# pangenome/seqrush

Measured on AMD Instinct MI355X. Metric: aligned pairs/sec all-vs-all 64x5kb, higher is better.
Workload: dtype i16; 1 GPU; C2: 64 x 5 kb synthetic (5% SNP, seed 2001), all-vs-all incl. self = 4096 ordered pairs, -k 0 -S 0,5,8,2,24,1 --orientation-scores 0,1,1,1, biWFA (Ultralow); pairs_total=4096, pairs_per_gpu=4096, parallelism=pair-shard x1

## Files before the change

### include/seqrush_amd.h

```cpp
#ifndef SEQRUSH_AMD_H
#define SEQRUSH_AMD_H
#include <stddef.h>
#include <stdint.h>

#ifdef __cplusplus
extern "C" {
#endif

#define SR_ABI_VERSION 2

typedef enum {
    SR_OK = 0,
    SR_ERR_INVALID = -1,
    SR_ERR_NO_DEVICE = -2,
    SR_ERR_HIP = -3,
    SR_ERR_ALPHABET = -4,
    SR_ERR_EMPTY_SEQ = -5,
    SR_ERR_UNSUPPORTED = -6,
    SR_ERR_DEVICE_FAULT = -7,
    SR_ERR_IO = -8,
    SR_ERR_NOMEM = -9
} sr_status;

typedef struct {
    uint32_t n;
    const uint8_t *bases;
    const uint64_t *offsets;
    const char *const *names;
} sr_seqset;

#define SR_MEM_HIGH 0
#define SR_MEM_ULTRALOW 3

#define SR_SPARSE_NONE 0
#define SR_SPARSE_AUTO 1
#define SR_SPARSE_RANDOM 2
#define SR_SPARSE_CONNECTIVITY 3
#define SR_SPARSE_TREE 4

typedef struct {
    int32_t match_score;
    int32_t mismatch_penalty;
    int32_t gap_open1, gap_ext1;
    int32_t gap_open2, gap_ext2;
    int32_t ori_match, ori_mismatch, ori_gap_open, ori_gap_ext;
    uint64_t min_match_len;
    double max_divergence;
    int32_t exclude_self;
    int32_t memory_mode;
    int32_t sparsify_kind;
    double sparsify_factor;
    uint64_t sparsify_seed;
    int32_t canonical_labels;
    int32_t device;
    uint32_t shard_rank, shard_count;
    uint32_t tree_k_nearest, tree_k_farthest;
    double tree_rand_frac;
    uint32_t tree_kmer;
} sr_params;

void sr_default_params(sr_params *p);
int sr_parse_scores(const char *s, sr_params *p);
int sr_parse_orientation_scores(const char *s, sr_params *p);
int sr_parse_sparsification(const char *s, sr_params *p);

int sr_pair_list(uint32_t n, const sr_params *p, uint32_t **q_out, uint32_t **t_out,
                 uint64_t *count);

typedef struct {
    uint64_t n;
    uint32_t *query_idx, *target_idx;
    uint8_t *is_reverse;
    int32_t *score;
    uint64_t *query_start, *query_end, *target_start, *target_end;
    uint64_t *cigar_off;
    uint32_t *cigar_ops;
} sr_alignments;

int sr_align_all(const sr_seqset *seqs, const sr_params *p, sr_alignments **out);
void sr_alignments_free(sr_alignments *a);
size_t sr_alignment_cigar(const sr_alignments *a, uint64_t i, char *buf, size_t cap);

int sr_align_and_unite(const sr_seqset *seqs, const sr_params *p, uint64_t *parent_out);

uint64_t sr_uf_find(const uint64_t *nodes, uint64_t n, uint64_t x);
int sr_uf_same(const uint64_t *nodes, uint64_t n, uint64_t x, uint64_t y);
int sr_uf_init_host(uint64_t *nodes, uint64_t n, uint64_t total_len);
int sr_uf_unite_host(uint64_t *nodes, uint64_t n, uint64_t x, uint64_t y);
int sr_uf_merge_labels_host(uint64_t *nodes, uint64_t n, const uint64_t *labels, uint32_t count);
int sr_uf_canonical_labels_host(const uint64_t *nodes, uint64_t n, uint64_t *labels_out);

int sr_write_paf(const sr_alignments *a, const sr_seqset *seqs, const char *path);

typedef struct sr_ctx sr_ctx;
int sr_ctx_create(int device, sr_ctx **out);
void sr_ctx_destroy(sr_ctx *c);
int sr_ctx_set_stream(sr_ctx *c, void *hip_stream);
int sr_ctx_load(sr_ctx *c, const sr_seqset *seqs, const sr_params *p);
int sr_ctx_load_pairs(sr_ctx *c, const sr_seqset *seqs, const sr_params *p, const uint32_t *query_idx,
                      const uint32_t *target_idx, uint64_t count);
int sr_ctx_pairs(const sr_ctx *c, uint32_t **q_out, uint32_t **t_out, uint64_t *count);
uint32_t sr_ctx_num_batches(const sr_ctx *c);
const char *sr_ctx_workspace_report(const sr_ctx *c);
int sr_ctx_reset_uf(sr_ctx *c);
int sr_ctx_align(sr_ctx *c);
int sr_ctx_unite(sr_ctx *c);
int sr_ctx_run(sr_ctx *c);
int sr_ctx_align_all(sr_ctx *c, int unite, sr_alignments **out);
int sr_ctx_pair_results(sr_ctx *c, int32_t *score, uint8_t *is_reverse, uint32_t *cigar_ops);
int sr_ctx_sync(sr_ctx *c);
int sr_ctx_alignments(sr_ctx *c, sr_alignments **out);
int sr_ctx_download_uf(sr_ctx *c, uint64_t *parent_out);
uint64_t sr_ctx_uf_size(const sr_ctx *c);
uint64_t sr_ctx_num_pairs(const sr_ctx *c);
uint64_t sr_ctx_dp_cells(const sr_ctx *c);
int sr_ctx_labels_device(sr_ctx *c, uint64_t *dev_labels);
int sr_ctx_merge_labels(sr_ctx *c, const uint64_t *dev_labels, uint32_t count);
int sr_ctx_labels_device_u32(sr_ctx *c, uint32_t *dev_labels);
int sr_ctx_merge_labels_u32(sr_ctx *c, const uint32_t *dev_labels, uint32_t count);
int sr_ctx_download_labels(sr_ctx *c, uint64_t *labels_out);
int sr_ctx_merge_labels_host(sr_ctx *c, const uint64_t *labels, uint32_t count);
int sr_ctx_load_paf(sr_ctx *c, const sr_seqset *seqs, const sr_params *p, const char *paf_path);
int sr_unite_paf(const sr_seqset *seqs, const sr_params *p, const char *paf_path, uint64_t *parent_out);
int sr_ctx_build_gfa(sr_ctx *c, const sr_seqset *seqs, char **gfa, uint64_t *n_nodes, uint64_t *n_edges);
int sr_ctx_kernel_ms(sr_ctx *c, int which, float *ms);
const char *sr_ctx_align_kernel(const sr_ctx *c);
int sr_ctx_counters(sr_ctx *c, uint64_t out[16]);
int sr_ctx_counters_ext(sr_ctx *c, uint64_t out[32]);
int sr_ctx_counters_all(sr_ctx *c, uint64_t *out, uint32_t cap);
const char *sr_knobs_doc(void);
int sr_ctx_tail_deferred(sr_ctx *c, uint64_t *out);
int sr_ctx_tail_timeline(sr_ctx *c, uint64_t *out, uint32_t cap_wg);
int sr_tail_shape(int impl, int block_levels, int wave_build, int off16, int ring_u16, int symbol_bits, int two_piece,
                  int main_threads, uint32_t max_words, int forced);

typedef struct {
    uint64_t tree_entries;
    uint64_t random_entries;
    uint64_t random_processed;
    uint64_t random_aligned;
    uint64_t checks;
    uint64_t windows;
    uint64_t post_tree;
    uint64_t final_components;
    int32_t stabilized;
    int32_t tree_defaulted;
    uint32_t tree_k_nearest, tree_k_farthest;
    double tree_rand_frac;
    uint32_t tree_kmer;
    uint32_t reserved;
} sr_iter_stats;
int sr_ctx_load_iterative(sr_ctx *c, const sr_seqset *seqs, const sr_params *p, int keep_alignments);
int sr_ctx_run_iterative(sr_ctx *c);
int sr_ctx_iterative_stats(sr_ctx *c, sr_iter_stats *out, uint64_t *check_counts, uint64_t cap);
int sr_ctx_iterative_alignments(sr_ctx *c, sr_alignments **out);
int sr_uf_count_components_host(const uint64_t *nodes, uint64_t n, uint64_t total_len, uint64_t *count);
int sr_iterative_stop_host(const uint64_t *counts, uint64_t nchecks, uint64_t post_tree, uint64_t *stop_check);
int sr_iterative_pair_lists(uint32_t n, const uint8_t *sel, const sr_params *p, uint32_t **tree_i, uint32_t **tree_j,
                            uint64_t *tree_count, uint32_t **rand_i, uint32_t **rand_j, uint64_t *rand_count);
int sr_base_cone_reach(int e1, int e2, int two, int levels_left);
int sr_mirror_map(const uint32_t *query_idx, const uint32_t *target_idx, uint64_t count, const uint32_t *batch_first,
                  uint32_t nbatch, uint32_t workgroups, uint32_t *mirror_out, uint64_t *partners_out);
int sr_ctx_orientation_scores(sr_ctx *c, int32_t *fwd, int32_t *rev);
int sr_mirror_bt_pick(const int *off, int transposed);
int sr_mirror_bt_rank_transposed(int tag);
int sr_mirror_bt_tie_host(const int *off);
int sr_mirror_bp_pick_host(const int *val, const int *dist, const int *comp, const int *diag, int n, int value_bias,
                           int *pick_out, int *pick_t_out);
int sr_replay_record_ints(void);
void sr_replay_transpose_host(const int *rec, int *out);
int sr_replay_match_host(const int *recs, int nrec, const int *segs, int nseg, int level, int *match_out);

typedef struct {
    uint64_t min_size;
    int32_t keep_alignments;
    uint32_t join_below;
} sr_inv_params;
typedef struct {
    uint64_t scanned;
    uint64_t sites;
    uint64_t candidates;
    uint64_t accepted;
    uint64_t rejected_score;
    uint64_t rejected_divergence;
    uint64_t united_bases;
    uint64_t patch_batches;
    double scan_ms, patch_align_ms;
} sr_inv_stats;
typedef struct {
    uint64_t pair;
    uint32_t query_idx, target_idx;
    uint64_t query_start, query_end;
    uint64_t target_start, target_end;
    int32_t main_score, patch_score;
    uint8_t is_reverse;
    uint8_t accepted;
    uint8_t reserved[2];
    int32_t site_cost;
} sr_inv_job;
int sr_ctx_enable_inversions(sr_ctx *c, const sr_inv_params *p);
int sr_ctx_inversion_stats(sr_ctx *c, sr_inv_stats *out);
int sr_ctx_inversion_join_stats(sr_ctx *c, uint64_t out[4]);
int sr_ctx_inversion_jobs(sr_ctx *c, sr_inv_job **jobs, uint64_t *count);
int sr_ctx_inversion_alignments(sr_ctx *c, sr_alignments **out);
int sr_append_paf_tagged(const sr_alignments *a, const sr_seqset *seqs, const char *path, const char *tag);
#define SR_INV_SITE_DIVERGENT 1
#define SR_INV_SITE_QUERY_ONLY 2
#define SR_INV_SITE_TARGET_ONLY 3
typedef struct {
    uint64_t query_start, query_end, target_start, target_end;
    int32_t kind;
    int32_t candidate;
} sr_inv_site;
int sr_inversion_sites_host(const uint32_t *ops, uint64_t n_ops, uint64_t min_size, sr_inv_site **sites, uint64_t *count);
int sr_inversion_candidate(uint64_t qgap, uint64_t tgap, uint64_t min_size);
int sr_inversion_accept(int32_t patch_score, int32_t main_score);
int sr_inversion_sites_host_join(const uint32_t *ops, uint64_t n_ops, uint64_t min_size, uint32_t join_below, const sr_params *pen,
                                 sr_inv_site **sites, int32_t **cost, uint64_t *count);
int sr_inversion_accept_site(int32_t patch_score, int32_t site_cost);
int sr_inversion_scan_device(int device, const uint32_t *ops, const uint64_t *cigar_off, uint64_t n, uint64_t min_size,
                             sr_inv_site **sites, uint64_t **owner, uint64_t *count);
int sr_inversion_scan_device_join(int device, const uint32_t *ops, const uint64_t *cigar_off, uint64_t n, uint64_t min_size,
                                  uint32_t join_below, const sr_params *pen, const int32_t *score, const int32_t *max_score,
                                  sr_inv_site **sites, uint64_t **owner, int32_t **cost, uint64_t *count, uint64_t stats[4]);
int sr_sketch_device(int device, const sr_seqset *seqs, uint32_t kmer, uint64_t **sketch, uint32_t **sketch_n,
                     uint32_t **shared, uint32_t **denom);
int sr_knn_select_device(int device, const uint32_t *shared, const uint32_t *denom, uint32_t n, uint32_t k_nearest,
                         uint32_t k_farthest, uint8_t **sel);

int sr_build_gfa(const sr_seqset *seqs, const uint64_t *labels, char **gfa,
                 uint64_t *n_nodes, uint64_t *n_edges);
int sr_build_gfa_opts(const sr_seqset *seqs, const uint64_t *labels, int compact, char **gfa,
                      uint64_t *n_nodes, uint64_t *n_edges);
int sr_build_gfa_from_nodes(const sr_seqset *seqs, const uint64_t *nodes, int compact, char **gfa,
                            uint64_t *n_nodes, uint64_t *n_edges);
int sr_ctx_build_gfa_opts(sr_ctx *c, const sr_seqset *seqs, int compact, char **gfa, uint64_t *n_nodes, uint64_t *n_edges);

#define SR_SORT_DEVICE_HOST_TWIN (-1)
#define SR_SORT_DEVICE_SEQUENTIAL (-2)
typedef struct {
    uint64_t seed;
    uint64_t iter_max;
    double theta;
    double eps;
    double eta_max;
    double cooling_start;
    uint64_t space;
    uint64_t space_max;
    uint64_t space_quant;
    uint64_t min_term_updates;
    uint64_t terms_per_round;
    int32_t skip_sgd, skip_groom, skip_topo;
    int32_t device;
} sr_sort_params;
void sr_sort_params_default(sr_sort_params *p);
int sr_ctx_build_gfa_sorted(sr_ctx *c, const sr_seqset *seqs, int compact, const sr_sort_params *p, char **gfa,
                            uint64_t *n_nodes, uint64_t *n_edges);
int sr_sort_gfa(const char *gfa_in, const sr_sort_params *p, char **gfa_out, uint64_t *n_nodes, uint64_t *n_edges);
int sr_sgd_layout(const char *gfa_in, const sr_sort_params *p, double *pos_out, uint64_t n);
int sr_sgd_tables(const char *gfa_in, const sr_sort_params *p, sr_sort_params *resolved, uint64_t sizes[4], double *etas,
                  double *zetas, double *prefix_theta, double *prefix_cool);
int sr_sort_stats(double *out, uint32_t cap);

#define SR_COMPACT_DEVICE_HOST (-1)
#define SR_COMPACT_DEVICE_TABLES_HOST (-2)
int sr_compact_gfa(const char *gfa_in, int device, char **gfa_out, uint64_t *n_nodes, uint64_t *n_edges, uint64_t stats[8]);
int sr_compact_stats(uint64_t stats[8]);

#define SR_STATS_DEVICE_HOST (-1)
typedef struct {
    uint64_t length, nodes, edges, paths, steps;
    uint64_t rev_steps, depth_bp;
    uint64_t self_loops, tips, components;
    uint32_t *depth, *paths_on;
    uint64_t *bp_by_paths, *nodes_by_paths;
    uint64_t *shared;
    uint64_t *path_pairs, *path_abs, *path_len;
    uint64_t *path_sq;
    uint64_t total_pairs, total_abs, total_len, total_sq[3];
    uint64_t stats_us;
    uint64_t kernel_us[5];
} sr_graph_stats;
int sr_graph_stats_gfa(const char *gfa_in, int device, sr_graph_stats **out);
void sr_graph_stats_free(sr_graph_stats *s);
int sr_graph_stats_report(const sr_graph_stats *s, const char *const *names, char **text);
// ... 115 lines not shown
```

### seqrush_amd/_lib.py

```python
import ctypes as C
import os

_HERE = os.path.dirname(os.path.abspath(__file__))
LIB_PATH = os.environ.get("SEQRUSH_AMD_LIB") or os.path.join(_HERE, "libseqrush_amd.so")

EXPORTS = [
    "sr_default_params", "sr_parse_scores", "sr_parse_orientation_scores",
    "sr_parse_sparsification", "sr_align_all", "sr_alignments_free", "sr_alignment_cigar",
    "sr_align_and_unite", "sr_uf_find", "sr_uf_same", "sr_write_paf", "sr_ctx_create",
    "sr_ctx_destroy", "sr_ctx_set_stream", "sr_ctx_load", "sr_ctx_reset_uf", "sr_ctx_align",
    "sr_ctx_unite", "sr_ctx_sync", "sr_ctx_alignments", "sr_ctx_download_uf", "sr_ctx_uf_size",
    "sr_ctx_num_pairs", "sr_ctx_dp_cells", "sr_ctx_labels_device", "sr_ctx_merge_labels",
    "sr_ctx_download_labels", "sr_ctx_kernel_ms", "sr_ctx_counters", "sr_build_gfa", "sr_free",
    "sr_last_error", "sr_abi_version", "sr_device_count", "sr_pair_list", "sr_ctx_align_kernel",
    "sr_ctx_load_paf", "sr_unite_paf", "sr_ctx_build_gfa", "sr_ctx_load_pairs", "sr_ctx_pairs",
    "sr_ctx_num_batches", "sr_ctx_workspace_report", "sr_ctx_run", "sr_ctx_align_all", "sr_ctx_pair_results",
    "sr_ctx_labels_device_u32", "sr_ctx_merge_labels_u32", "sr_ctx_counters_ext",
    "sr_build_gfa_opts", "sr_ctx_build_gfa_opts", "sr_ctx_merge_labels_host",
    "sr_uf_init_host", "sr_uf_unite_host", "sr_uf_merge_labels_host", "sr_uf_canonical_labels_host",
    "sr_build_gfa_from_nodes", "sr_ctx_counters_all", "sr_knobs_doc",
    "sr_sort_params_default", "sr_ctx_build_gfa_sorted", "sr_sort_gfa", "sr_sgd_layout", "sr_sgd_tables", "sr_sort_stats",
    "sr_ctx_load_iterative", "sr_ctx_run_iterative", "sr_ctx_iterative_stats", "sr_ctx_iterative_alignments",
    "sr_uf_count_components_host", "sr_iterative_stop_host", "sr_iterative_pair_lists", "sr_base_cone_reach",
    "sr_ctx_enable_inversions", "sr_ctx_inversion_stats", "sr_ctx_inversion_jobs", "sr_ctx_inversion_alignments",
    "sr_append_paf_tagged", "sr_inversion_sites_host", "sr_inversion_candidate", "sr_inversion_accept",
    "sr_inversion_scan_device",
    "sr_ctx_inversion_join_stats", "sr_inversion_sites_host_join", "sr_inversion_accept_site", "sr_inversion_scan_device_join",
    "sr_compact_gfa", "sr_compact_stats",
    "sr_sketch_device", "sr_knn_select_device",
    "sr_graph_stats_gfa", "sr_graph_stats_free", "sr_graph_stats_report", "sr_stats_sq_sums_host",
    "sr_mirror_map", "sr_mirror_bt_pick", "sr_mirror_bt_rank_transposed", "sr_mirror_bt_tie_host", "sr_mirror_bp_pick_host",
    "sr_ctx_orientation_scores",
    "sr_layout_params_default", "sr_layout_gfa", "sr_layout_tsv", "sr_layout_svg", "sr_layout_quality", "sr_layout_stats",
    "sr_layout_resolve", "sr_layout_select_host",
    "sr_path_bins_gfa", "sr_path_bins_free", "sr_path_bins_tsv", "sr_viz_params_default", "sr_path_bins_rgb", "sr_path_bins_png",
    "sr_growth_params_default", "sr_growth_gfa", "sr_growth_free", "sr_growth_groups", "sr_growth_expected", "sr_growth_fit",
    "sr_growth_report",
    "sr_variant_params_default", "sr_variants_gfa", "sr_variants_free", "sr_variants_vcf",
    "sr_ctx_tail_deferred", "sr_ctx_tail_timeline", "sr_tail_shape",
    "sr_replay_record_ints", "sr_replay_transpose_host", "sr_replay_match_host",
]


class SeqSetC(C.Structure):
    _fields_ = [("n", C.c_uint32), ("bases", C.c_char_p), ("offsets", C.POINTER(C.c_uint64)),
                ("names", C.POINTER(C.c_char_p))]


class ParamsC(C.Structure):
    _fields_ = [
        ("match_score", C.c_int32), ("mismatch_penalty", C.c_int32),
        ("gap_open1", C.c_int32), ("gap_ext1", C.c_int32),
        ("gap_open2", C.c_int32), ("gap_ext2", C.c_int32),
        ("ori_match", C.c_int32), ("ori_mismatch", C.c_int32),
        ("ori_gap_open", C.c_int32), ("ori_gap_ext", C.c_int32),
        ("min_match_len", C.c_uint64), ("max_divergence", C.c_double),
        ("exclude_self", C.c_int32), ("memory_mode", C.c_int32),
        ("sparsify_kind", C.c_int32), ("sparsify_factor", C.c_double),
        ("sparsify_seed", C.c_uint64), ("canonical_labels", C.c_int32), ("device", C.c_int32),
        ("shard_rank", C.c_uint32), ("shard_count", C.c_uint32),
        ("tree_k_nearest", C.c_uint32), ("tree_k_farthest", C.c_uint32), ("tree_rand_frac", C.c_double),
        ("tree_kmer", C.c_uint32),
    ]


class SortParamsC(C.Structure):
    _fields_ = [
        ("seed", C.c_uint64), ("iter_max", C.c_uint64), ("theta", C.c_double), ("eps", C.c_double),
        ("eta_max", C.c_double), ("cooling_start", C.c_double), ("space", C.c_uint64), ("space_max", C.c_uint64),
        ("space_quant", C.c_uint64), ("min_term_updates", C.c_uint64), ("terms_per_round", C.c_uint64),
        ("skip_sgd", C.c_int32), ("skip_groom", C.c_int32), ("skip_topo", C.c_int32), ("device", C.c_int32),
    ]


class LayoutParamsC(C.Structure):
    _fields_ = [
        ("seed", C.c_uint64), ("iter_max", C.c_uint64), ("theta", C.c_double), ("eps", C.c_double),
        ("eta_max", C.c_double), ("cooling_start", C.c_double), ("space", C.c_uint64), ("space_max", C.c_uint64),
        ("space_quant", C.c_uint64), ("min_term_updates", C.c_uint64), ("terms_per_round", C.c_uint64),
        ("device", C.c_int32), ("reserved", C.c_int32),
    ]


class IterStatsC(C.Structure):
    _fields_ = [
        ("tree_entries", C.c_uint64), ("random_entries", C.c_uint64), ("random_processed", C.c_uint64),
        ("random_aligned", C.c_uint64), ("checks", C.c_uint64), ("windows", C.c_uint64), ("post_tree", C.c_uint64),
        ("final_components", C.c_uint64), ("stabilized", C.c_int32), ("tree_defaulted", C.c_int32),
        ("tree_k_nearest", C.c_uint32), ("tree_k_farthest", C.c_uint32), ("tree_rand_frac", C.c_double),
        ("tree_kmer", C.c_uint32), ("reserved", C.c_uint32),
    ]


class InvParamsC(C.Structure):
    _fields_ = [("min_size", C.c_uint64), ("keep_alignments", C.c_int32), ("join_below", C.c_uint32)]


class InvStatsC(C.Structure):
    _fields_ = [("scanned", C.c_uint64), ("sites", C.c_uint64), ("candidates", C.c_uint64), ("accepted", C.c_uint64),
                ("rejected_score", C.c_uint64), ("rejected_divergence", C.c_uint64), ("united_bases", C.c_uint64),
                ("patch_batches", C.c_uint64), ("scan_ms", C.c_double), ("patch_align_ms", C.c_double)]


class InvJobC(C.Structure):
    _fields_ = [("pair", C.c_uint64), ("query_idx", C.c_uint32), ("target_idx", C.c_uint32),
                ("query_start", C.c_uint64), ("query_end", C.c_uint64), ("target_start", C.c_uint64),
                ("target_end", C.c_uint64), ("main_score", C.c_int32), ("patch_score", C.c_int32),
                ("is_reverse", C.c_uint8), ("accepted", C.c_uint8), ("reserved", C.c_uint8 * 2), ("site_cost", C.c_int32)]


class InvSiteC(C.Structure):
    _fields_ = [("query_start", C.c_uint64), ("query_end", C.c_uint64), ("target_start", C.c_uint64),
                ("target_end", C.c_uint64), ("kind", C.c_int32), ("candidate", C.c_int32)]


class GraphStatsC(C.Structure):
    _fields_ = [("length", C.c_uint64), ("nodes", C.c_uint64), ("edges", C.c_uint64), ("paths", C.c_uint64), ("steps", C.c_uint64),
                ("rev_steps", C.c_uint64), ("depth_bp", C.c_uint64),
                ("self_loops", C.c_uint64), ("tips", C.c_uint64), ("components", C.c_uint64),
                ("depth", C.POINTER(C.c_uint32)), ("paths_on", C.POINTER(C.c_uint32)),
                ("bp_by_paths", C.POINTER(C.c_uint64)), ("nodes_by_paths", C.POINTER(C.c_uint64)),
                ("shared", C.POINTER(C.c_uint64)),
                ("path_pairs", C.POINTER(C.c_uint64)), ("path_abs", C.POINTER(C.c_uint64)), ("path_len", C.POINTER(C.c_uint64)),
                ("path_sq", C.POINTER(C.c_uint64)),
                ("total_pairs", C.c_uint64), ("total_abs", C.c_uint64), ("total_len", C.c_uint64), ("total_sq", C.c_uint64 * 3),
                ("stats_us", C.c_uint64), ("kernel_us", C.c_uint64 * 5)]


class BinParamsC(C.Structure):
    _fields_ = [("bin_width", C.c_uint64), ("bins", C.c_uint64)]


class PathBinsC(C.Structure):
    _fields_ = [("length", C.c_uint64), ("paths", C.c_uint64), ("bins", C.c_uint64), ("bin_width", C.c_uint64),
                ("cov", C.POINTER(C.c_uint64)), ("inv", C.POINTER(C.c_uint64)),
                ("bin_us", C.c_uint64), ("kernel_us", C.c_uint64 * 3)]


class VizParamsC(C.Structure):
    _fields_ = [("mode", C.c_int), ("path_height", C.c_uint32), ("path_gap", C.c_uint32), ("depth_max", C.c_uint32)]


class GrowthParamsC(C.Structure):
    _fields_ = [("seed", C.c_uint64), ("permutations", C.c_uint64)]


class GrowthC(C.Structure):
    _fields_ = [("length", C.c_uint64), ("paths", C.c_uint64), ("groups", C.c_uint64), ("permutations", C.c_uint64),
                ("exhaustive", C.c_int32), ("variant", C.c_int32),
                ("pan", C.POINTER(C.c_uint64)), ("core", C.POINTER(C.c_uint64)), ("perm", C.POINTER(C.c_uint32)),
                ("bp_by_groups", C.POINTER(C.c_uint64)), ("growth_us", C.c_uint64), ("kernel_us", C.c_uint64 * 4),
                ("seed", C.c_uint64)]


class VariantParamsC(C.Structure):
    _fields_ = [("ref_name", C.c_char_p), ("max_allele_len", C.c_uint64), ("hash_mask", C.c_uint64), ("reserved", C.c_uint64)]


class VariantsC(C.Structure):
    _fields_ = [("ref_path", C.c_uint64), ("ref_len", C.c_uint64), ("paths", C.c_uint64), ("anchors", C.c_uint64),
                ("traversals", C.c_uint64), ("sites", C.c_uint64), ("hash_collision_sites", C.c_uint64),
                ("breaks", C.POINTER(C.c_uint64)), ("skipped", C.POINTER(C.c_uint64)),
                ("site_start", C.POINTER(C.c_uint64)), ("site_end", C.POINTER(C.c_uint64)), ("site_alleles", C.POINTER(C.c_uint32)),
                ("allele_off", C.POINTER(C.c_uint64)), ("alleles", C.POINTER(C.c_char)), ("gt", C.POINTER(C.c_int32)),
                ("ref_seq", C.POINTER(C.c_char)), ("variant", C.c_int32), ("reserved", C.c_int32),
                ("variants_us", C.c_uint64), ("kernel_us", C.c_uint64 * 6)]


class AlignmentsC(C.Structure):
    _fields_ = [
        ("n", C.c_uint64), ("query_idx", C.POINTER(C.c_uint32)), ("target_idx", C.POINTER(C.c_uint32)),
        ("is_reverse", C.POINTER(C.c_uint8)), ("score", C.POINTER(C.c_int32)),
        ("query_start", C.POINTER(C.c_uint64)), ("query_end", C.POINTER(C.c_uint64)),
        ("target_start", C.POINTER(C.c_uint64)), ("target_end", C.POINTER(C.c_uint64)),
        ("cigar_off", C.POINTER(C.c_uint64)), ("cigar_ops", C.POINTER(C.c_uint32)),
    ]


class SeqRushError(RuntimeError):
    def __init__(self, code, msg):
        super().__init__(f"seqrush_amd error {code}: {msg}")
        self.code = code


_lib = None


def load():
    global _lib
    if _lib is not None:
        return _lib
    if not os.path.exists(LIB_PATH):
        raise ImportError(
            f"{LIB_PATH} not found: build it with `python -c 'import __graft_entry__ as g; g.build()'` "
            "(seqrush_amd has no CPU fallback)")
    L = C.CDLL(LIB_PATH)
    vp, u64, i32 = C.c_void_p, C.c_uint64, C.c_int
    PP, PS = C.POINTER(ParamsC), C.POINTER(SeqSetC)
    L.sr_default_params.argtypes = [PP]; L.sr_default_params.restype = None
    L.sr_parse_scores.argtypes = [C.c_char_p, PP]
    L.sr_parse_orientation_scores.argtypes = [C.c_char_p, PP]
    L.sr_parse_sparsification.argtypes = [C.c_char_p, PP]
    L.sr_align_all.argtypes = [PS, PP, C.POINTER(C.POINTER(AlignmentsC))]
    L.sr_alignments_free.argtypes = [C.POINTER(AlignmentsC)]; L.sr_alignments_free.restype = None
    L.sr_alignment_cigar.argtypes = [C.POINTER(AlignmentsC), u64, C.c_char_p, C.c_size_t]
    L.sr_alignment_cigar.restype = C.c_size_t
    L.sr_align_and_unite.argtypes = [PS, PP, C.POINTER(u64)]
    L.sr_uf_find.argtypes = [C.POINTER(u64), u64, u64]; L.sr_uf_find.restype = u64
    L.sr_uf_same.argtypes = [C.POINTER(u64), u64, u64, u64]
    L.sr_write_paf.argtypes = [C.POINTER(AlignmentsC), PS, C.c_char_p]
    L.sr_ctx_create.argtypes = [i32, C.POINTER(vp)]
    L.sr_ctx_destroy.argtypes = [vp]; L.sr_ctx_destroy.restype = None
    L.sr_ctx_set_stream.argtypes = [vp, vp]
    L.sr_ctx_load.argtypes = [vp, PS, PP]
    for f in ("sr_ctx_reset_uf", "sr_ctx_align", "sr_ctx_unite", "sr_ctx_sync"):
        getattr(L, f).argtypes = [vp]
    L.sr_ctx_alignments.argtypes = [vp, C.POINTER(C.POINTER(AlignmentsC))]
    L.sr_ctx_download_uf.argtypes = [vp, C.POINTER(u64)]
    for f in ("sr_ctx_uf_size", "sr_ctx_num_pairs", "sr_ctx_dp_cells"):
        getattr(L, f).argtypes = [vp]; getattr(L, f).restype = u64
    L.sr_ctx_labels_device.argtypes = [vp, vp]
    L.sr_ctx_merge_labels.argtypes = [vp, vp, C.c_uint32]
    L.sr_ctx_download_labels.argtypes = [vp, C.POINTER(u64)]
    L.sr_ctx_merge_labels_host.argtypes = [vp, C.POINTER(u64), C.c_uint32]
    L.sr_ctx_kernel_ms.argtypes = [vp, i32, C.POINTER(C.c_float)]
    L.sr_ctx_align_kernel.argtypes = [vp]; L.sr_ctx_align_kernel.restype = C.c_char_p
    L.sr_ctx_load_paf.argtypes = [vp, PS, PP, C.c_char_p]
    L.sr_unite_paf.argtypes = [PS, PP, C.c_char_p, C.POINTER(u64)]
    L.sr_ctx_build_gfa.argtypes = [vp, PS, C.POINTER(vp), C.POINTER(u64), C.POINTER(u64)]
    L.sr_ctx_counters.argtypes = [vp, C.POINTER(u64)]
    L.sr_ctx_counters_ext.argtypes = [vp, C.POINTER(u64)]
    L.sr_ctx_counters_all.argtypes = [vp, C.POINTER(u64), C.c_uint32]
    L.sr_knobs_doc.restype = C.c_char_p
    L.sr_ctx_tail_deferred.argtypes = [vp, C.POINTER(u64)]
    L.sr_ctx_tail_timeline.argtypes = [vp, C.POINTER(u64), C.c_uint32]
    L.sr_tail_shape.argtypes = [i32] * 8 + [C.c_uint32, i32]
    L.sr_ctx_load_pairs.argtypes = [vp, PS, PP, C.POINTER(C.c_uint32), C.POINTER(C.c_uint32), u64]
    L.sr_ctx_pairs.argtypes = [vp, C.POINTER(C.POINTER(C.c_uint32)), C.POINTER(C.POINTER(C.c_uint32)), C.POINTER(u64)]
    L.sr_ctx_num_batches.argtypes = [vp]; L.sr_ctx_num_batches.restype = C.c_uint32
    L.sr_ctx_workspace_report.argtypes = [vp]; L.sr_ctx_workspace_report.restype = C.c_char_p
    L.sr_ctx_run.argtypes = [vp]
    L.sr_ctx_align_all.argtypes = [vp, i32, C.POINTER(C.POINTER(AlignmentsC))]
    L.sr_ctx_pair_results.argtypes = [vp, C.POINTER(C.c_int32), C.POINTER(C.c_uint8), C.POINTER(C.c_uint32)]
    L.sr_ctx_labels_device_u32.argtypes = [vp, vp]
    L.sr_ctx_merge_labels_u32.argtypes = [vp, vp, C.c_uint32]
    L.sr_build_gfa.argtypes = [PS, C.POINTER(u64), C.POINTER(vp), C.POINTER(u64), C.POINTER(u64)]
    L.sr_build_gfa_opts.argtypes = [PS, C.POINTER(u64), i32, C.POINTER(vp), C.POINTER(u64), C.POINTER(u64)]
    L.sr_ctx_build_gfa_opts.argtypes = [vp, PS, i32, C.POINTER(vp), C.POINTER(u64), C.POINTER(u64)]
    L.sr_uf_init_host.argtypes = [C.POINTER(u64), u64, u64]
    L.sr_uf_unite_host.argtypes = [C.POINTER(u64), u64, u64, u64]
    L.sr_uf_merge_labels_host.argtypes = [C.POINTER(u64), u64, C.POINTER(u64), C.c_uint32]
    L.sr_uf_canonical_labels_host.argtypes = [C.POINTER(u64), u64, C.POINTER(u64)]
    L.sr_build_gfa_from_nodes.argtypes = [PS, C.POINTER(u64), i32, C.POINTER(vp), C.POINTER(u64), C.POINTER(u64)]
    SP, PD = C.POINTER(SortParamsC), C.POINTER(C.c_double)
    L.sr_sort_params_default.argtypes = [SP]; L.sr_sort_params_default.restype = None
    L.sr_ctx_build_gfa_sorted.argtypes = [vp, PS, i32, SP, C.POINTER(vp), C.POINTER(u64), C.POINTER(u64)]
    L.sr_sort_gfa.argtypes = [C.c_char_p, SP, C.POINTER(vp), C.POINTER(u64), C.POINTER(u64)]
    L.sr_sgd_layout.argtypes = [C.c_char_p, SP, PD, u64]
    L.sr_sgd_tables.argtypes = [C.c_char_p, SP, SP, C.POINTER(u64), PD, PD, PD, PD]
    L.sr_sort_stats.argtypes = [PD, C.c_uint32]
    L.sr_pair_list.argtypes = [C.c_uint32, PP, C.POINTER(C.POINTER(C.c_uint32)),
                               C.POINTER(C.POINTER(C.c_uint32)), C.POINTER(u64)]
    L.sr_ctx_load_iterative.argtypes = [vp, PS, PP, i32]
    L.sr_ctx_run_iterative.argtypes = [vp]
    L.sr_ctx_iterative_stats.argtypes = [vp, C.POINTER(IterStatsC), C.POINTER(u64), u64]
    L.sr_ctx_iterative_alignments.argtypes = [vp, C.POINTER(C.POINTER(AlignmentsC))]
    L.sr_uf_count_components_host.argtypes = [C.POINTER(u64), u64, u64, C.POINTER(u64)]
    L.sr_iterative_stop_host.argtypes = [C.POINTER(u64), u64, u64, C.POINTER(u64)]
    L.sr_base_cone_reach.argtypes = [C.c_int, C.c_int, C.c_int, C.c_int]
    PU32 = C.POINTER(C.POINTER(C.c_uint32))
    L.sr_iterative_pair_lists.argtypes = [C.c_uint32, C.POINTER(C.c_uint8), PP, PU32, PU32, C.POINTER(u64), PU32, PU32,
                                          C.POINTER(u64)]
    L.sr_ctx_enable_inversions.argtypes = [vp, C.POINTER(InvParamsC)]
    L.sr_ctx_inversion_stats.argtypes = [vp, C.POINTER(InvStatsC)]
    L.sr_ctx_inversion_jobs.argtypes = [vp, C.POINTER(C.POINTER(InvJobC)), C.POINTER(u64)]
    L.sr_ctx_inversion_alignments.argtypes = [vp, C.POINTER(C.POINTER(AlignmentsC))]
    L.sr_append_paf_tagged.argtypes = [C.POINTER(AlignmentsC), PS, C.c_char_p, C.c_char_p]
    L.sr_inversion_sites_host.argtypes = [C.POINTER(C.c_uint32), u64, u64, C.POINTER(C.POINTER(InvSiteC)), C.POINTER(u64)]
    L.sr_inversion_candidate.argtypes = [u64, u64, u64]
    L.sr_inversion_accept.argtypes = [C.c_int32, C.c_int32]
    L.sr_inversion_scan_device.argtypes = [i32, C.POINTER(C.c_uint32), C.POINTER(u64), u64, u64,
                                           C.POINTER(C.POINTER(InvSiteC)), C.POINTER(C.POINTER(u64)), C.POINTER(u64)]
    PI32 = C.POINTER(C.c_int32)
    L.sr_ctx_inversion_join_stats.argtypes = [vp, C.POINTER(u64)]
    L.sr_inversion_sites_host_join.argtypes = [C.POINTER(C.c_uint32), u64, u64, C.c_uint32, PP, C.POINTER(C.POINTER(InvSiteC)),
                                               C.POINTER(PI32), C.POINTER(u64)]
    L.sr_inversion_accept_site.argtypes = [C.c_int32, C.c_int32]
    L.sr_inversion_scan_device_join.argtypes = [i32, C.POINTER(C.c_uint32), C.POINTER(u64), u64, u64, C.c_uint32, PP, PI32, PI32,
                                                C.POINTER(C.POINTER(InvSiteC)), C.POINTER(C.POINTER(u64)), C.POINTER(PI32),
                                                C.POINTER(u64), C.POINTER(u64)]
    PU32P = C.POINTER(C.POINTER(C.c_uint32))
    L.sr_sketch_device.argtypes = [i32, PS, C.c_uint32, C.POINTER(C.POINTER(u64)), PU32P, PU32P, PU32P]
    L.sr_knn_select_device.argtypes = [i32, C.POINTER(C.c_uint32), C.POINTER(C.c_uint32), C.c_uint32, C.c_uint32, C.c_uint32,
                                       C.POINTER(C.POINTER(C.c_uint8))]
    L.sr_compact_gfa.argtypes = [C.c_char_p, i32, C.POINTER(vp), C.POINTER(u64), C.POINTER(u64), C.POINTER(u64)]
    L.sr_compact_stats.argtypes = [C.POINTER(u64)]
    PGS = C.POINTER(GraphStatsC)
    L.sr_graph_stats_gfa.argtypes = [C.c_char_p, i32, C.POINTER(PGS)]
    L.sr_graph_stats_free.argtypes = [PGS]; L.sr_graph_stats_free.restype = None
    L.sr_graph_stats_report.argtypes = [PGS, C.POINTER(C.c_char_p), C.POINTER(vp)]
    L.sr_stats_sq_sums_host.argtypes = [C.POINTER(u64), u64, C.POINTER(u64)]
    LP = C.POINTER(LayoutParamsC)
    L.sr_layout_params_default.argtypes = [LP]; L.sr_layout_params_default.restype = None
    L.sr_layout_gfa.argtypes = [C.c_char_p, LP, PD, u64]
    L.sr_layout_tsv.argtypes = [PD, u64, C.POINTER(vp)]
    L.sr_layout_svg.argtypes = [C.c_char_p, PD, u64, C.POINTER(vp)]
    L.sr_layout_quality.argtypes = [C.c_char_p, PD, u64, u64, u64, PD]
    L.sr_layout_stats.argtypes = [PD, C.c_uint32]
    L.sr_layout_resolve.argtypes = [C.c_char_p, LP, LP]
    L.sr_layout_select_host.argtypes = [C.c_char_p, LP, u64, u64, u64, i32, C.POINTER(C.c_uint32), C.POINTER(C.c_uint32), PD]
    PPB, PVP = C.POINTER(PathBinsC), C.POINTER(VizParamsC)
    L.sr_path_bins_gfa.argtypes = [C.c_char_p, C.POINTER(BinParamsC), i32, C.POINTER(PPB)]
    L.sr_path_bins_free.argtypes = [PPB]; L.sr_path_bins_free.restype = None
    L.sr_path_bins_tsv.argtypes = [PPB, C.POINTER(C.c_char_p), C.POINTER(vp)]
    L.sr_viz_params_default.argtypes = [PVP]; L.sr_viz_params_default.restype = None
    L.sr_path_bins_rgb.argtypes = [PPB, C.POINTER(C.c_char_p), PVP, C.POINTER(vp), C.POINTER(C.c_uint32), C.POINTER(C.c_uint32)]
    L.sr_path_bins_png.argtypes = [PPB, C.POINTER(C.c_char_p), PVP, C.POINTER(vp), C.POINTER(u64)]
    PG, PU32 = C.POINTER(GrowthC), C.POINTER(C.c_uint32)
    L.sr_growth_params_default.argtypes = [C.POINTER(GrowthParamsC)]; L.sr_growth_params_default.restype = None
    L.sr_growth_gfa.argtypes = [C.c_char_p, PU32, C.c_uint32, C.POINTER(GrowthParamsC), i32, C.POINTER(PG)]
    L.sr_growth_free.argtypes = [PG]; L.sr_growth_free.restype = None
    L.sr_growth_groups.argtypes = [C.POINTER(C.c_char_p), u64, i32, PU32, PU32, C.POINTER(C.POINTER(C.c_char_p))]
    L.sr_growth_expected.argtypes = [C.POINTER(u64), C.c_uint32, PD, PD]
    L.sr_growth_fit.argtypes = [PD, C.c_uint32, PD, PD, PU32]
    L.sr_growth_report.argtypes = [PG, C.POINTER(vp)]
    PV = C.POINTER(VariantsC)
    L.sr_variant_params_default.argtypes = [C.POINTER(VariantParamsC)]; L.sr_variant_params_default.restype = None
    L.sr_variants_gfa.argtypes = [C.c_char_p, C.POINTER(VariantParamsC), i32, C.POINTER(PV)]
    L.sr_variants_free.argtypes = [PV]; L.sr_variants_free.restype = None
    L.sr_variants_vcf.argtypes = [PV, C.POINTER(C.c_char_p), C.POINTER(vp)]
    PI = C.POINTER(C.c_int)
    L.sr_mirror_map.argtypes = [C.POINTER(C.c_uint32), C.POINTER(C.c_uint32), u64, C.POINTER(C.c_uint32), C.c_uint32, C.c_uint32,
                                C.POINTER(C.c_uint32), C.POINTER(u64)]
    L.sr_ctx_orientation_scores.argtypes = [vp, C.POINTER(C.c_int32), C.POINTER(C.c_int32)]
    L.sr_mirror_bt_pick.argtypes = [PI, i32]
    L.sr_mirror_bt_rank_transposed.argtypes = [i32]
    L.sr_mirror_bt_tie_host.argtypes = [PI]
    L.sr_mirror_bp_pick_host.argtypes = [PI, PI, PI, PI, i32, i32, PI, PI]
    L.sr_replay_record_ints.argtypes = []
    L.sr_replay_transpose_host.argtypes = [PI, PI]; L.sr_replay_transpose_host.restype = None
    L.sr_replay_match_host.argtypes = [PI, i32, PI, i32, i32, PI]
    L.sr_free.argtypes = [vp]; L.sr_free.restype = None
    L.sr_last_error.restype = C.c_char_p
    L.sr_abi_version.restype = i32
    L.sr_device_count.restype = i32
    _lib = L
    return L


def check(rc):
    if rc != 0:
        raise SeqRushError(rc, load().sr_last_error().decode(errors="replace"))
```

### seqrush_amd/csrc/sr_align_blk.inc

```
#include "sr_blk_rows.inc"
#include "sr_blk_tile.inc"
#include "sr_blk_pass.inc"
#include "sr_blk_phase2.inc"
#include "sr_blk_orient.inc"

#define K_SHIFT0 29
#define K_WIDTH0 64
struct KSeqs { int poff_f, poff_r, toff_f, toff_r, plen_all, tlen_all; };
__device__ __forceinline__ void kjob_set(int jid, int base, int pb, int pe, int tb, int te, int rev, int begin, int chk,
                                         int seg, const KSeqs &q) {
    bjob_set(jid, base, pb, pe, tb, te, 0, begin, chk, seg, rev ? q.poff_r : q.poff_f);
    BJob &b = b_sh.job[jid];
    b.shift = (pe - pb) + K_SHIFT0;
    b.pad0 = rev ? q.toff_r : q.toff_f;
    b.pad2 = 1;
    if (rev) { b.p0 = q.plen_all - pe; b.t0 = q.tlen_all - te; }
}
__device__ __forceinline__ int kjob_width(int plen, int tlen) { return (plen + tlen + K_WIDTH0) & ~3; }

#define SR_BLK_MIN_WAVES 4
template <typename OT, int NT, bool TWO, int B, int E1, int E2, bool PROF = false, int X = 0, int OE1 = 0, typename RT = OT>
__global__ void __launch_bounds__(NT, SR_BLK_MIN_WAVES) sr_align_blk_kernel(SrAlignArgs a) {
    const int tid = threadIdx.x;
    if (a.tail_mode == SR_TAIL_RUN && *a.tail_count == 0u) return;
    GP<RT> bring = (GP<RT>)(RT *)a.bring + (size_t)blockIdx.x * a.bring_wg_stride;
    GP<OT> bhist = (GP<OT>)(OT *)a.bhist + (size_t)blockIdx.x * a.bhist_wg_stride;
    GP<int> lists = (GP<int>)a.bseg + (size_t)blockIdx.x * 2 * SR_BFS_MAXSEG * SR_BFS_SEGREC;
    GP<uint32_t> btbuf = (GP<uint32_t>)a.bbt + (size_t)blockIdx.x * a.bbase_jobs * SR_BFS_BTCAP;
    GP<uint32_t> clist = (GP<uint32_t>)a.bcl + (size_t)blockIdx.x * a.bcl_wg_stride;
    GP<int> gmak = (GP<int>)a.bmak + (size_t)blockIdx.x * (BJ_MAX * BFS_MAK_SLOTS);
    unsigned long long t_ori = 0, t_bp = 0, t_base = 0, t_all = 0, tb_bt = 0, tb_emit = 0;
    unsigned long long tq_pass = 0, tq_bar = 0, tq_ctl = 0, tq_ph2 = 0, tq_tail = 0, tq_rec = 0;
    unsigned row_ld = 0, row_st = 0;
    unsigned long long tl_first = 0, tl_last = 0, tl_n = 0, tl_mir = 0;
    const int depth = a.kdepth;
    const int depth2 = a.kdepth2;
    const unsigned nrows = (unsigned)depth + 4u * (unsigned)depth2 + (unsigned)SR_NULL_ROWS + 2u;
    KRows<OT, RT> RR;
    KRows<OT, OT> RH;
    RR.base = bring; RR.cM = (unsigned)depth * 256u; RR.cst2 = (unsigned)depth2 * 256u; RR.sstr = 256u; RR.chs = nrows * 256u;
    RR.depth = depth; RR.depth2 = depth2; RR.perjob = false; RR.extent = (unsigned)a.bring_wg_stride;
    RR.nuloff = ((unsigned)depth + 4u * (unsigned)depth2) * 256u; RR.urow = RR.nuloff + (unsigned)SR_NULL_ROWS * 256u; RR.trash = RR.urow + 256u;
    const unsigned urow = RR.urow;
    const unsigned hw = a.hist_nul_w;
    RH.base = bhist; RH.cM = 0; RH.cst2 = 0; RH.sstr = 0; RH.chs = 256u; RH.depth = 0x3fff; RH.depth2 = 0x3fff; RH.urow = 0; RH.perjob = true; RH.extent = (unsigned)a.bhist_wg_stride;
    RH.nuloff = (unsigned)a.hist_cap; RH.trash = RH.nuloff + hw;
    if (tid < 64) k_sh.cells_l[tid] = 0ull;
    if (tid < 64) k_sh.row_w[tid >> 4][tid & 15] = 0ull;
    {
        for (int r = 0; r < SR_NULL_ROWS; r++)
            for (int i = tid; i < a.brow; i += NT) rput(RR, RR.nuloff + (unsigned)r * 256u, (unsigned)i, NULLV);
        for (int i = tid; i < (int)hw; i += NT) RH.base[RH.nuloff + (unsigned)i] = (OT)NULLV;
        if (tid == 0) {
            b_sh.pen[0] = a.pen; b_sh.pen[1] = a.ori; b_sh.cells = 0; k_sh.t_setup = 0; k_sh.t_p2a = k_sh.t_p2f = k_sh.t_p2e = k_sh.t_p2w = 0; k_sh.t_c1 = k_sh.t_c2 = 0;
            k_sh.dg_f = k_sh.dg_c = k_sh.dg_e = k_sh.dg_r = 0; k_sh.dg_redo = 0;
#ifdef SR_BOUNDS
            k_sh.bnd_flag = 0; k_sh.bnd_off = k_sh.bnd_ext = k_sh.bnd_what = 0; k_sh.lds_seq_bytes = 16u * a.max_words + 16u;
#endif
            k_sh.dg_steps = k_sh.dg_nbase = k_sh.dg_nbp = k_sh.dg_npass = 0; k_sh.base_tiles = k_sh.base_cells = 0;
            k_sh.mir_next = -1; k_sh.mir_pairs = k_sh.mir_ties = 0;
            k_sh.rp_record = k_sh.rp_on = k_sh.rp_ready = 0; k_sh.rp_nrec = 0;
            k_sh.rp_replays = k_sh.rp_cached = k_sh.rp_tie_top = k_sh.rp_tie_base = 0;
            b_sh.geom.brow = a.brow; b_sh.geom.ring_scope = a.ring_scope; b_sh.geom.ring_hot = a.ring_hot;
            b_sh.geom.bbase_jobs = a.bbase_jobs; b_sh.geom.hist_w = a.hist_w; b_sh.geom.hist_levels = a.hist_levels;
            b_sh.geom.urow = urow;
        }
        __syncthreads();
    }
    const SrPen pen = a.pen;
    const SrPen ori = a.ori;
    constexpr bool KTIGHT = KTIGHT_OF(OT, RT, B, X);
    const int scope = pen.scope;
    const int gap_opening = TWO ? max(pen.o1, pen.o2) : pen.o1;
    for (;;) {
        if (tid < 64) {
            unsigned long long cl = k_sh.cells_l[tid];
            k_sh.cells_l[tid] = 0ull;
            for (int o = 32; o > 0; o >>= 1) cl += __shfl_xor(cl, o, 64);
            if (tid == 0) b_sh.cells += cl;
        }
        if (tid == 0) {
            int pr = k_sh.mir_next;
            k_sh.mir_next = -1;
            const bool from_mir = pr >= 0;
            if (a.tail_mode == SR_TAIL_RUN) {
                const uint32_t i = atomicAdd(a.tail_head, 1u);
                pr = i < *a.tail_count ? (int)a.tail_list[i] : (int)a.npairs;
            } else while (pr < 0) {
                pr = (int)atomicAdd(a.queue_head, 1u);
                if (pr >= (int)a.npairs) { pr = (int)a.npairs; break; }
                if (a.order) pr = (int)a.order[pr];
                if (a.mirror && a.mirror[pr] != SR_MIRROR_NONE && (a.mirror[pr] & SR_MIRROR_SECONDARY)) pr = -1;
            }
            if (PROF) {
                const unsigned long long now = KTICK();
                if (tl_n == 0) tl_first = now;
                if (pr < (int)a.npairs) { tl_last = now; tl_n++; tl_mir = from_mir ? 1ull : 0ull; }
            }
            k_sh.rp_on = (from_mir && k_sh.rp_ready) ? 1 : 0;
            k_sh.rp_ready = 0; k_sh.rp_record = 0;
            if (a.brec && !from_mir && a.tail_mode != SR_TAIL_RUN && a.mirror && pr < (int)a.npairs) {
                const uint32_t m = a.mirror[pr];
                if (m != SR_MIRROR_NONE && !(m & SR_MIRROR_SECONDARY)) { k_sh.rp_record = 1; k_sh.rp_nrec = 0; }
            }
            k_sh.rp_level = 0; k_sh.rp_rd = 0; k_sh.rp_top_tie = 0; k_sh.rp_seg_tie = 0;
            b_sh.pair = pr;
            b_sh.err = 0; b_sh.cig_cnt = 0; b_sh.score_acc = 0; k_sh.pend_op = -1; k_sh.pend_len = 0;
            k_sh.mir_tie = 0;
            k_sh.mir_snap[0] = b_sh.cells; k_sh.mir_snap[1] = k_sh.dg_steps; k_sh.mir_snap[2] = k_sh.dg_nbase; k_sh.mir_snap[3] = k_sh.dg_nbp;
        }
        __syncthreads();
        const int pair = RFL(b_sh.pair);
        if (pair >= (int)a.npairs) break;
        const uint32_t q = a.pair_q[pair], t = a.pair_t[pair];
        const int plen = (int)a.seqlen[q], tlen = (int)a.seqlen[t];
        const int pw = SR_SEQ_WORDS(plen), tw = SR_SEQ_WORDS(tlen);
        load_seq_lds<NT>(lds_seq, (GP<const uint32_t>)a.seqwords + a.word_off_fwd[q] - 1, pw);
        load_seq_lds<NT>(lds_seq + a.max_words, (GP<const uint32_t>)a.seqwords + a.word_off_rc[q] - 1, pw);
        load_seq_lds<NT>(lds_seq + 2 * (size_t)a.max_words, (GP<const uint32_t>)a.seqwords + a.word_off_fwd[t] - 1, tw);
        load_seq_lds<NT>(lds_seq + 3 * (size_t)a.max_words, (GP<const uint32_t>)a.seqwords + a.word_off_rev[t] - 1, tw);
        const int oPf = 1, oPr = (int)a.max_words + 1, oTf = 2 * (int)a.max_words + 1, oTr = 3 * (int)a.max_words + 1;
        GP<uint32_t> ops = (GP<uint32_t>)a.cigar_ops + a.cigar_base[pair];
        const uint32_t cap = (uint32_t)(a.cigar_base[pair + 1] - a.cigar_base[pair]);
        const unsigned long long tk0 = KTICK();
        int fwd = -1, rev = INT_MAX, is_rev = 0;
        if (a.pre_oriented) {
            is_rev = a.is_reverse[pair] != 0; fwd = a.ori_fwd[pair]; rev = a.ori_rev[pair];
        } else {
        if (tid == 0) {
            const int w = kjob_width(plen, tlen);
            const KSeqs k0 = {oPf, oPr, oTf, oTr, plen, tlen}, k1 = {oPr, oPf, oTf, oTr, plen, tlen};
            kjob_set(0, 0, 0, plen, 0, tlen, 0, SR_C_M, SR_C_M, 0, k0);
            kjob_set(1, w, 0, plen, 0, tlen, 0, SR_C_M, SR_C_M, 0, k1);
            b_sh.njobs = 2;
        }
        __syncthreads();
        const long long smax = (long long)ori.o1 * 2 + (long long)ori.e1 * (plen + tlen) + 64;
        if (!ori.two && ori.x == 1 && ori.o1 == 1 && ori.e1 == 1 && !a.ori_levels) {
            if (tid == 0) {
                b_sh.job[0].shift = plen + 24; b_sh.job[1].shift = plen + 24;
                b_sh.job[1].base = (plen + tlen + 64) & ~3;
            }
            __syncthreads();
            for (int s0 = 0;; s0 += ORI_B) {
                ori_pass8<OT, NT>(RR, s0, ori, row_ld, row_st);
                __syncthreads();
                int hit = -1, who = 0;
#pragma unroll
                for (int j = ORI_B - 1; j >= 0; j--) {
                    const bool rf = RFL(k_sh.jreach[j][0]) != 0, rr = RFL(k_sh.jreach[j][1]) != 0;
                    if (rf || rr) { hit = j; who = rf ? 0 : 1; }
                }
                __syncthreads();
                const int used = hit >= 0 ? hit + 1 : ORI_B;
                if (tid == 0) k_sh.dg_steps += 2ull * (unsigned long long)used;
                if (hit >= 0) {
                    if (tid == 0) {
                        long long sur = 0;
                        for (int l = s0 + hit + 1; l < s0 + ORI_B; l++) {
                            const int Rw = reach(ori, l, SR_C_M);
                            sur += 2LL * (long long)(min(tlen, Rw) - max(-plen, -Rw) + 1);
                        }
                        b_sh.cells -= (unsigned long long)sur;
                    }
                    if (who == 0) fwd = s0 + hit; else { rev = s0 + hit; is_rev = 1; }
                    break;
                }
                if (s0 + ORI_B - 1 > smax) { if (tid == 0) b_sh.err |= SR_DEV_ERR_SCORE_BOUND; break; }
            }
        } else {
            for (int s = 0;; s++) {
                blk_pass<OT, false, NT, 1, 1, 1, PROF>(RR, s, ori, 2, row_ld, row_st);
                __syncthreads();
                if (tid == 0) k_sh.dg_steps += 2ull;
                const bool rf = RFL(k_sh.jreach[0][0]) != 0, rr = RFL(k_sh.jreach[0][1]) != 0;
                __syncthreads();
                if (rf) { fwd = s; break; }
                if (rr) { rev = s; is_rev = 1; break; }
                if (s > smax) { if (tid == 0) b_sh.err |= SR_DEV_ERR_SCORE_BOUND; break; }
            }
        }
        }
        if (a.word_off_rev != a.word_off_rc) {
            __syncthreads();
            load_seq_lds<NT>(lds_seq + (is_rev ? 0 : (size_t)a.max_words),
                             (GP<const uint32_t>)a.seqwords + (is_rev ? a.word_off_cmp[q] : a.word_off_rev[q]) - 1, pw);
            __syncthreads();
        }
        const KSeqs ks = {is_rev ? oPr : oPf, is_rev ? oPf : oPr, oTf, oTr, plen, tlen};
        const unsigned long long tk1 = KTICK();
        t_ori += tk1 - tk0;
        GP<int> cur = lists, nxt = lists + (size_t)SR_BFS_MAXSEG * SR_BFS_SEGREC;
        if (tid == 0) {
            cur[SL_PB] = 0; cur[SL_PE] = plen; cur[SL_TB] = 0; cur[SL_TE] = tlen; cur[SL_CB] = SR_C_M; cur[SL_CE] = SR_C_M;
            const int rem = (a.mem_mode == 3) ? INT_MAX : -1;
            cur[SL_REM] = rem; cur[SL_KIND] = seg_kind(plen, tlen, rem);
            b_sh.list_n = 1;
            if (is_rev) k_sh.rp_on = 0;
            if (k_sh.rp_on) k_sh.rp_replays += 1ull;
        }
        __syncthreads();
        for (;;) {
            const int n_cur = RFL(b_sh.list_n);
            bool any_bp = false;
            int pos = 0;
            if (RFL(k_sh.rp_on) != 0 && tid == 0) {
                GP<int> recs = (GP<int>)a.brec + (size_t)blockIdx.x * (SR_BPREC_MAX * SR_BPREC_INTS);
                const int nrec = min(k_sh.rp_nrec, SR_BPREC_MAX), lvl = k_sh.rp_level;
                int rd = k_sh.rp_rd;
                unsigned long long cells = 0ull, cached = 0ull;
                while (rd < nrec && recs[rd * SR_BPREC_INTS + SR_BR_LEVEL] < lvl) rd++;
                for (int p = 0; p < n_cur; p++) {
                    GP<int> e = cur + (size_t)p * SR_BFS_SEGREC;
                    if (e[SL_KIND] != SK_BP) continue;
                    int solved = 0;
                    while (rd < nrec) {
                        GP<int> r = recs + rd * SR_BPREC_INTS;
                        if (r[SR_BR_LEVEL] != lvl) break;
                        const int c = sr_replay_cmp(r, e);
                        if (c > 0) break;
                        rd++;
                        if (c < 0) continue;
                        if (r[SR_BR_TIE] == 0 && sr_replay_same(r, e)) {
                            e[SL_BV] = sr_bprec_t(r, SR_BR_BV); e[SL_BH] = sr_bprec_t(r, SR_BR_BH); e[SL_BCOMP] = sr_bprec_t(r, SR_BR_BCOMP);
                            e[SL_BSF] = r[SR_BR_BSF]; e[SL_BSR] = r[SR_BR_BSR]; e[SL_PASSES] = r[SR_BR_PASSES];
                            cells += ((unsigned long long)(unsigned)r[SR_BR_CELLS_HI] << 32) | (unsigned long long)(unsigned)r[SR_BR_CELLS_LO];
                            cached += 1ull; solved = 1;
                        }
                        break;
                    }
                    e[SL_SOLVED] = solved;
                }
                k_sh.rp_rd = rd; b_sh.cells += cells; k_sh.rp_cached += cached;
            }
            while (pos < n_cur && RFL(b_sh.err) == 0) {
                __syncthreads();
                if (tid == 0) {
                    int na = 0, p = pos, base = 0, ntot = 0, maxp = 0;
                    const bool rp_on = k_sh.rp_on != 0, rp_rec = k_sh.rp_record != 0;
                    for (; p < n_cur && ntot < SR_BFS_MAXACT; p++) {
                        GP<int> e = cur + (size_t)p * SR_BFS_SEGREC;
                        if (e[SL_KIND] != SK_BP) continue;
                        ntot++;
                        if (rp_on && e[SL_SOLVED] != 0) { maxp = max(maxp, e[SL_PASSES]); continue; }
                        k_sh.sg_tie[na] = 0; k_sh.sg_sur[na] = 0; k_sh.sg_done[na] = 0;
                        if (rp_rec) {
                            b_sh.cells += k_sh.cells_l[2 * na] + k_sh.cells_l[2 * na + 1];
                            k_sh.cells_l[2 * na] = 0ull; k_sh.cells_l[2 * na + 1] = 0ull;
                        }
// ... 296 lines not shown
                            if (st == 0) EMIT(SR_OP_D, sp);
                            else EMIT(SR_OP_I, st);
                        } else if (kind == SK_BASE) {
                            GP<uint32_t> b = btbuf + (size_t)bj * SR_BFS_BTCAP;
                            const int nbt = RFL(b_sh.bt_n[bj]);
                            for (int i = nbt - 1; i >= 0; i -= 64) {
                                const uint32_t v = (i - lane >= 0) ? b[i - lane] : 0u;
                                const int m = min(64, i + 1);
                                for (int u = 0; u < m; u++) {
                                    const uint32_t x = (uint32_t)__builtin_amdgcn_readlane((int)v, u);
                                    EMIT((int)(x & 15u), (int)(x >> 4));
                                }
                            }
                            bj++;
                        } else err |= SR_DEV_ERR_BACKTRACE;
                    }
#undef EMIT
                    if (lane == 0) {
                        b_sh.cig_cnt = cnt; b_sh.emit_pos = pos; k_sh.pend_op = pop; k_sh.pend_len = plen_;
                        if (err) b_sh.err |= err;
                    }
                    KPRIO_LO();
                }
                __syncthreads();
                tb_emit += KTICK() - tem0;
            }
            if (tid == 0 && b_sh.err == 0 && k_sh.pend_op >= 0) {
                uint32_t cnt = b_sh.cig_cnt;
                if (cnt >= cap) b_sh.err |= SR_DEV_ERR_CIGAR_OVERFLOW;
                else { ops[cnt++] = ((uint32_t)k_sh.pend_len << 4) | (uint32_t)k_sh.pend_op; b_sh.cig_cnt = cnt; }
            }
            __syncthreads();
        }
        t_base += KTICK() - tc0;
        __syncthreads();
        const uint32_t cnt = RFL(b_sh.cig_cnt);
        int part = 0;
        for (uint32_t i = tid; i < cnt; i += NT) {
            const uint32_t op = ops[i] & 15u; const int len = (int)(ops[i] >> 4);
            if (op == SR_OP_X) part += len * pen.x;
            else if (op == SR_OP_I || op == SR_OP_D) {
                int g = pen.o1 + pen.e1 * len;
                if (TWO) g = min(g, pen.o2 + pen.e2 * len);
                part += g;
            }
        }
        if (part) atomicAdd(&b_sh.score_acc, part);
        __syncthreads();
        const int p_err = RFL(b_sh.err), p_score = RFL(b_sh.score_acc), p_tie = RFL(k_sh.mir_tie);
        if (tid == 0) {
            a.is_reverse[pair] = is_rev ? 1 : 0;
            a.score[pair] = b_sh.err ? -1 : b_sh.score_acc;
            a.ori_fwd[pair] = fwd; a.ori_rev[pair] = rev;
            a.cigar_cnt[pair] = b_sh.err ? 0u : cnt;
            if (b_sh.err) atomicOr(a.error_flag, b_sh.err);
#ifdef SR_BOUNDS
            if (k_sh.bnd_flag == 1) {
                k_sh.bnd_flag = 2;
                if (atomicCAS(&a.counters[40], 0ull, (unsigned long long)pair + 1ull) == 0ull) {
                    a.counters[41] = k_sh.bnd_what; a.counters[42] = k_sh.bnd_off; a.counters[43] = k_sh.bnd_ext;
                }
            }
#endif
        }
        __syncthreads();
        const uint32_t mir = a.mirror ? a.mirror[pair] : SR_MIRROR_NONE;
        bool mir_emit = false;
        if (mir != SR_MIRROR_NONE && !(mir & SR_MIRROR_SECONDARY)) {
            mir_emit = p_err == 0 && !is_rev && p_tie == 0 && !(a.pre_oriented && a.is_reverse[mir] != 0);
            if (mir_emit) {
                GP<uint32_t> ops2 = (GP<uint32_t>)a.cigar_ops + a.cigar_base[mir];
                for (uint32_t i = tid; i < cnt; i += NT) { const uint32_t v = ops[i]; ops2[i] = v ^ ((v & 2u) >> 1); }
                if (tid < 64) {
                    unsigned long long cl = k_sh.cells_l[tid];
                    k_sh.cells_l[tid] = 0ull;
                    for (int o = 32; o > 0; o >>= 1) cl += __shfl_xor(cl, o, 64);
                    if (tid == 0) {
                        b_sh.cells += cl;
                        b_sh.cells += b_sh.cells - k_sh.mir_snap[0]; k_sh.dg_steps += k_sh.dg_steps - k_sh.mir_snap[1];
                        k_sh.dg_nbase += k_sh.dg_nbase - k_sh.mir_snap[2]; k_sh.dg_nbp += k_sh.dg_nbp - k_sh.mir_snap[3];
                        k_sh.mir_pairs += 1ull;
                        a.score[mir] = p_score; a.cigar_cnt[mir] = cnt;
                        if (!a.pre_oriented) { a.is_reverse[mir] = 0; a.ori_fwd[mir] = fwd; a.ori_rev[mir] = rev; }
                    }
                }
            } else if (tid == 0) {
                k_sh.mir_ties += 1ull;
                if (p_tie != 0) {
                    if (k_sh.rp_top_tie != 0) k_sh.rp_tie_top += 1ull;
                    else if (k_sh.rp_seg_tie == 0) k_sh.rp_tie_base += 1ull;
                }
                const bool replay = k_sh.rp_record != 0 && p_err == 0 && !is_rev && k_sh.rp_top_tie == 0 &&
                                    !(a.pre_oriented && a.is_reverse[mir] != 0) && a.tail_mode != SR_TAIL_DEFER_ALL;
                bool defer = false;
                if (!replay && a.tail_list && a.tail_mode != SR_TAIL_RUN)
                    defer = a.tail_mode == SR_TAIL_DEFER_ALL ||
                            __hip_atomic_load(a.queue_head, __ATOMIC_RELAXED, __HIP_MEMORY_SCOPE_AGENT) >= a.npairs;
                if (defer) { a.tail_list[atomicAdd(a.tail_count, 1u)] = mir; atomicAdd(a.tail_deferred, 1u); }
                else { k_sh.mir_next = (int)mir; k_sh.rp_ready = replay ? 1 : 0; }
            }
        }
        if (a.fuse_unite) {
            const int sc = p_err ? -1 : p_score;
            if (sc >= 0 && sc <= a.max_score[pair]) {
                unsigned long long united = 0, runs = 0;
                int uerr = 0;
                uf_unite_cigar<NT>((const uint32_t *)a.cigar_ops + a.cigar_base[pair], cnt, a.seq_goff[q], a.seq_goff[t],
                                   (unsigned long long)plen, is_rev != 0, 0ull, 0ull, a.min_match_len, a.uf_nodes, united, runs, uerr);
                for (int o = 32; o > 0; o >>= 1) { united += __shfl_xor(united, o, 64); runs += __shfl_xor(runs, o, 64); }
                if ((tid & 63) == 0) {
                    if (united) atomicAdd(&a.counters[4], mir_emit ? 2ull * united : united);
                    if (runs) atomicAdd(&a.counters[5], mir_emit ? 2ull * runs : runs);
                }
                if (uerr) atomicOr(a.error_flag, uerr);
            }
        }
        t_all += KTICK() - tk0;
        if ((tid & 63) == 0) {
            k_sh.row_w[0][(tid >> 6) & 15] += row_ld; k_sh.row_w[1][(tid >> 6) & 15] += row_st;
            k_sh.row_w[2][(tid >> 6) & 15] += row_ld; k_sh.row_w[3][(tid >> 6) & 15] += row_st;
        }
        row_ld = 0; row_st = 0;
    }
    if (tid < 64 && k_sh.cells_l[tid]) atomicAdd(&a.counters[0], k_sh.cells_l[tid]);
    if ((tid & 63) == 0) {
        const unsigned long long lane_bytes = 8ull;
        const unsigned long long row_ld_acc = k_sh.row_w[0][(tid >> 6) & 15], row_st_acc = k_sh.row_w[1][(tid >> 6) & 15];
        if (row_ld_acc) atomicAdd(&a.counters[16], row_ld_acc * lane_bytes);
        if (row_st_acc) atomicAdd(&a.counters[17], row_st_acc * lane_bytes);
        const unsigned long long hist_ld_acc = k_sh.row_w[2][(tid >> 6) & 15], hist_st_acc = k_sh.row_w[3][(tid >> 6) & 15];
        if (hist_ld_acc) atomicAdd(&a.counters[44], hist_ld_acc * lane_bytes);
        if (hist_st_acc) atomicAdd(&a.counters[45], hist_st_acc * lane_bytes);
    }
    if (tid == 0) {
        atomicAdd(&a.counters[0], b_sh.cells);
        atomicAdd(&a.counters[1], k_sh.dg_steps);
        atomicAdd(&a.counters[2], k_sh.dg_nbase);
        atomicAdd(&a.counters[3], k_sh.dg_nbp);
        atomicAdd(&a.counters[9], k_sh.dg_npass);
        atomicAdd(&a.counters[19], k_sh.dg_f); atomicAdd(&a.counters[20], k_sh.dg_c);
        atomicAdd(&a.counters[21], k_sh.dg_e); atomicAdd(&a.counters[22], k_sh.dg_r);
        if (k_sh.dg_redo) atomicAdd(&a.counters[37], k_sh.dg_redo);
        if (k_sh.mir_pairs) atomicAdd(&a.counters[38], k_sh.mir_pairs);
        if (k_sh.mir_ties) atomicAdd(&a.counters[39], k_sh.mir_ties);
        if (k_sh.rp_tie_top) atomicAdd(&a.counters[48], k_sh.rp_tie_top);
        if (k_sh.rp_tie_base) atomicAdd(&a.counters[49], k_sh.rp_tie_base);
        if (k_sh.rp_replays) atomicAdd(&a.counters[50], k_sh.rp_replays);
        if (k_sh.rp_cached) atomicAdd(&a.counters[51], k_sh.rp_cached);
        atomicAdd(&a.counters[46], k_sh.base_tiles); atomicAdd(&a.counters[47], k_sh.base_cells);
        if (PROF && a.timeline) {
            unsigned long long *tl = a.timeline + 4ull * blockIdx.x;
            tl[0] = tl_first; tl[1] = tl_last; tl[2] = KTICK(); tl[3] = tl_n | (tl_mir << 32);
        }
        if (PROF) {
            if (!a.pre_oriented) atomicAdd(&a.counters[6], t_ori);
            atomicAdd(&a.counters[7], t_bp);
            atomicAdd(&a.counters[8], t_base);
            atomicAdd(&a.counters[10], t_all);
            atomicAdd(&a.counters[11], tq_pass);
            atomicAdd(&a.counters[12], tq_bar);
            atomicAdd(&a.counters[13], k_sh.t_setup);
            atomicAdd(&a.counters[25], tq_ctl); atomicAdd(&a.counters[26], k_sh.t_c1); atomicAdd(&a.counters[27], k_sh.t_c2);
            atomicAdd(&a.counters[28], k_sh.t_p2a); atomicAdd(&a.counters[29], k_sh.t_p2f); atomicAdd(&a.counters[30], k_sh.t_p2e); atomicAdd(&a.counters[31], k_sh.t_p2w);
            atomicAdd(&a.counters[14], tq_ph2);
            atomicAdd(&a.counters[18], tq_rec);
            atomicAdd(&a.counters[23], tb_bt); atomicAdd(&a.counters[24], tb_emit);
            atomicAdd(&a.counters[15], tq_tail);
        }
    }
#undef KTICK
}
```

### seqrush_amd/csrc/sr_blk_pass.inc

```
#include "sr_base_cone.h"
template <bool TWO, int E1, int E2>
__device__ __forceinline__ int kreach(const SrPen &p, int s, int begin) {
    int r;
    if (begin == SR_C_M) {
        r = (s >= p.o1 + E1) ? (s - p.o1) / E1 : 0;
        if (TWO && s >= p.o2 + E2) r = max(r, (s - p.o2) / E2);
    } else {
        r = s / E1;
        if (TWO) r = max(r, s / E2);
    }
    return r;
}

template <bool TWO, int B, int E1, int E2, bool TIGHT>
__device__ __forceinline__ void kwindow(const SrPen &pen, const BJob &b, int s0, int &glo, int &ghi) {
    const int Rw = kreach<TWO, E1, E2>(pen, s0 + B - 1, b.begin);
    const int mg = TIGHT ? 1 : pen.scope + 1;
    const int wlo = max(-b.plen - 1, -Rw - mg), whi = min(b.tlen + 1, Rw + mg);
    glo = (wlo + b.shift) >> 2; ghi = (whi + b.shift) >> 2;
}

#define KTICK() (PROF ? __builtin_amdgcn_s_memrealtime() : 0ull)
#define KPRIO_HI() __builtin_amdgcn_s_setprio(3)
#define KPRIO_LO() __builtin_amdgcn_s_setprio(0)
#ifndef SR_BASE_CONE
#define SR_BASE_CONE 1
#endif
template <bool TWO, int NT, int B, int E1, int E2, bool TIGHT = false, bool BASE = false>
__device__ __forceinline__ void blk_setup(int s0, const SrPen &pen, int njobs) {
    const int tid = threadIdx.x;
    constexpr bool CONE = BASE && SR_BASE_CONE;
    int nt = 0, glo = 0, ghi = -1, cells = 0, ccells = 0;
    const bool act = tid < njobs && b_sh.job[tid].active;
    const int pglo = (tid < BJ_MAX) ? k_sh.jglo[tid] : 0, pghi = (tid < BJ_MAX) ? k_sh.jghi[tid] : -1;
    if (act) {
        const BJob &b = b_sh.job[tid];
        int Rw = 0, clo0 = 0, chi0 = 0;
#pragma unroll
        for (int j = 0; j < B; j++) {
            Rw = kreach<TWO, E1, E2>(pen, s0 + j, b.begin);
            int klo = max(-b.plen, -Rw), khi = min(b.tlen, Rw);
            cells += (khi >= klo) ? khi - klo + 1 : 0;
            if (CONE) {
                const int rb = sr_cone_reach(E1, E2, TWO, b.pad1 - 1 - (s0 + j));
                klo = max(klo, b.kend - rb); khi = min(khi, b.kend + rb);
                if (j == 0) { clo0 = b.kend - rb; chi0 = b.kend + rb; }
            }
            k_sh.jklo[j][tid] = klo; k_sh.jkhi[j][tid] = khi;
            ccells += (khi >= klo) ? khi - klo + 1 : 0;
        }
        (void)Rw;
        kwindow<TWO, B, E1, E2, TIGHT>(pen, b, s0, glo, ghi);
        if (CONE) {
            const int mg = TIGHT ? 1 : pen.scope + 1;
            const int wlo = max(max(-b.plen - 1, -Rw - mg), clo0 - 1), whi = min(min(b.tlen + 1, Rw + mg), chi0 + 1);
            glo = (wlo + b.shift) >> 2; ghi = (whi >= wlo) ? (whi + b.shift) >> 2 : glo - 1;
        }
        nt = max(0, (ghi - glo + KGeo<B>::OWN) / KGeo<B>::OWN);
        if (BASE && ccells) atomicAdd(&k_sh.base_cells, (unsigned long long)ccells);
    }
    int incl = nt, hincl = 0;
#pragma unroll
    for (int o = 1; o < 64; o <<= 1) {
        const int v = __shfl_up(incl, o, 64), h = __shfl_up(hincl, o, 64);
        if (tid >= o) { incl += v; hincl += h; }
    }
    if (tid < BJ_MAX) {
        k_sh.jglo[tid] = glo; k_sh.jghi[tid] = ghi;
        k_sh.jgplo[tid] = pglo; k_sh.jgphi[tid] = pghi;
        k_sh.jtstart[tid + 1] = incl;
        k_sh.jmerge[tid] = 0;
        k_sh.jband[tid] = INT_MAX / 2;
#pragma unroll
        for (int j = 0; j < B; j++) { k_sh.jak[j][tid] = 0; k_sh.jreach[j][tid] = 0; }
    }
    if (tid == 0) k_sh.jtstart[0] = 0;
    if (tid == 63) { k_sh.nband = hincl; k_sh.total_tiles = incl + hincl; k_sh.next_tile = NT / 64; if (BASE) k_sh.base_tiles += (unsigned long long)incl; }
    k_sh.cells_l[tid] += (unsigned long long)cells;
}

template <typename OT, bool TWO, int NT, int B, int E1, int E2, bool PROF, int X = 0, int OE1 = 0, typename ST = OT, bool RING = false, bool BASE = false>
__device__ __forceinline__ void blk_pass(const KRows<OT, ST> &R, int s0, const SrPen &pen, int njobs,
                                         unsigned &row_ld, unsigned &row_st, const bool setup = true) {
    const int tid = threadIdx.x;
    if (setup) {
        const unsigned long long tsu0 = KTICK();
        if (tid < 64) blk_setup<TWO, NT, B, E1, E2, RING && KTIGHT_OF(OT, ST, B, X), BASE>(s0, pen, njobs);
        __syncthreads();
        if (PROF && threadIdx.x == 0) k_sh.t_setup += KTICK() - tsu0;
    }
    const int total = RFL(k_sh.total_tiles);
    const int slot0 = kslots(R, s0);
    const int nband = RFL(k_sh.nband);
    for (int t = (tid >> 6); t < total;) {
        int lo, ti;
        if (t < nband) { lo = RFL(k_sh.jbandown[t]); ti = RFL(k_sh.jband[lo]); }
        else {
            const int r = t - nband;
            int hi = njobs; lo = 0;
            while (hi - lo > 1) { const int mid = (lo + hi) >> 1; if (RFL(k_sh.jtstart[mid]) <= r) lo = mid; else hi = mid; }
            ti = r - RFL(k_sh.jtstart[lo]);
            ti += (ti >= RFL(k_sh.jband[lo])) ? 1 : 0;
        }
        blk_tile_any<OT, TWO, B, E1, E2, false, X, OE1, ST, RING>(R, s0, slot0, pen, lo, ti, lo, row_ld, row_st);
        int nx = 0;
        if ((tid & 63) == 0) nx = atomicAdd(&k_sh.next_tile, 1);
        t = RFL(nx);
    }
}

template <typename OT, bool TWO, int NT, int B, int E1, int E2, int X = 0, int OE1 = 0, typename ST = OT>
__device__ __forceinline__ void blk_recompute(const KRows<OT, ST> &R, const SrPen &pen, int sa, int entry_level, int s0_now,
                                              unsigned &row_ld, unsigned &row_st) {
    const int tid = threadIdx.x;
    const int wlo = max(0, entry_level - pen.scope);
    for (int blk = (wlo / B) * B; blk <= s0_now; blk += B) {
        __syncthreads();
        if (tid < 2) {
            const BJob &b = b_sh.job[2 * sa + tid];
            int Rw = 0;
#pragma unroll
            for (int j = 0; j < B; j++) {
                Rw = kreach<TWO, E1, E2>(pen, blk + j, b.begin);
                k_sh.jklo[j][BJ_MAX + tid] = max(-b.plen, -Rw); k_sh.jkhi[j][BJ_MAX + tid] = min(b.tlen, Rw);
            }
            (void)Rw;
            int glo, ghi;
            kwindow<TWO, B, E1, E2, KTIGHT_OF(OT, ST, B, X)>(pen, b, blk, glo, ghi);
            const bool first = blk == (wlo / B) * B;
            k_sh.jgplo[BJ_MAX + tid] = first ? 1 : k_sh.jglo[BJ_MAX + tid];
            k_sh.jgphi[BJ_MAX + tid] = first ? 0 : k_sh.jghi[BJ_MAX + tid];
            k_sh.jglo[BJ_MAX + tid] = glo; k_sh.jghi[BJ_MAX + tid] = ghi;
            const int nt = (ghi - glo + KGeo<B>::OWN) / KGeo<B>::OWN;
            const int n0 = __shfl(nt, 0, 64), n1 = __shfl(nt, 1, 64);
            if (tid == 0) { k_sh.rt_n0 = n0; k_sh.rt_total = n0 + n1; }
        }
        __syncthreads();
        const int n0 = RFL(k_sh.rt_n0), total = RFL(k_sh.rt_total);
        const int slot0 = kslots(R, blk);
        for (int t = (tid >> 6); t < total; t += NT / 64) {
            const int side = (t >= n0) ? 1 : 0;
            blk_tile_any<OT, TWO, B, E1, E2, true, X, OE1, ST, true>(R, blk, slot0, pen, 2 * sa + side, t - (side ? n0 : 0), BJ_MAX + side, row_ld, row_st);
        }
    }
    __syncthreads();
    if (tid < 2) b_sh.job[2 * sa + tid].pad2 = 1;
}

__device__ __forceinline__ long long blk_surplus(const SrPen &pen, int jid, int l0, int l1) {
    const BJob &b = b_sh.job[jid];
    long long c = 0;
    for (int l = l0 + 1; l <= l1; l++) {
        const int Rw = reach(pen, l, b.begin);
        const int klo = max(-b.plen, -Rw), khi = min(b.tlen, Rw);
        c += (khi >= klo) ? khi - klo + 1 : 0;
    }
    return c;
}
```

### seqrush_amd/csrc/sr_blk_rows.inc

```
#define SR_ORI_B 16
#define SR_KB_MAX 10
#define KB_LV (SR_ORI_B > SR_KB_MAX ? SR_ORI_B : SR_KB_MAX)
#define KB_MAX SR_KB_MAX
#define KPK_U16_OF(OT, ST, B, X) (sizeof(OT) == 4 && sizeof(ST) == 2 && (X) > 0 && (B) % 10 == 0)
#define KTIGHT_OF(OT, ST, B, X) ((X) > 0 && (B) % 10 == 0 && (sizeof(OT) == 2 || KPK_U16_OF(OT, ST, B, X)))

struct KShared {
    int jklo[KB_LV][BJ_MAX + 2], jkhi[KB_LV][BJ_MAX + 2];
    int jak[KB_MAX][BJ_MAX], jreach[KB_LV][BJ_MAX];
    int jtstart[BJ_MAX + 1], jglo[BJ_MAX + 2], jghi[BJ_MAX + 2];
    int jmerge[BJ_MAX];
    int jband[BJ_MAX], jbandown[BJ_MAX], nband;
    unsigned newmask;
    int rt_n0, rt_total;
    int jgplo[BJ_MAX + 2], jgphi[BJ_MAX + 2];
    int total_tiles;
    int next_tile;
    int p2n, p2seg[K_P2];
    unsigned p2mask_lo, p2mask_hi;
    int pc_n[K_P2], pc_s1[K_P2][2 * KB_MAX];
    unsigned char pc_side[K_P2][2 * KB_MAX];
    signed char pc_idx[K_P2][2][KB_MAX];
    unsigned long long pc_best[K_P2][2 * KB_MAX];
    unsigned long long pc_best_t[K_P2][2 * KB_MAX];
    int pu_start[2 * K_P2 + 1], pu_glo[2 * K_P2];
    int pu_kmin[2 * K_P2], pu_kmax[2 * K_P2];
    int cl_n;
#ifdef SR_BOUNDS
    unsigned lds_seq_bytes;
    int bnd_flag; unsigned bnd_off, bnd_ext, bnd_what;
#endif
    int mir_tie, mir_next;
    unsigned long long mir_snap[4];
    unsigned long long mir_pairs, mir_ties;
    int sg_tie[SR_BFS_MAXACT], sg_sur[SR_BFS_MAXACT], sg_done[SR_BFS_MAXACT];
    int rp_record, rp_on, rp_ready;
    int rp_level, rp_nrec, rp_rd;
    int rp_top_tie, rp_seg_tie;
    int rp_ntot, rp_maxp;
    unsigned long long rp_npass0;
    unsigned long long rp_replays, rp_cached, rp_tie_top, rp_tie_base;
    int redo_from;
    int pend_op, pend_len;
    unsigned long long row_w[4][16];
    unsigned long long base_tiles, base_cells;
    unsigned long long cells_l[64];
    unsigned long long t_c1, t_c2;
    unsigned long long t_setup, t_p2a, t_p2f, t_p2e, t_p2w;
    unsigned long long dg_steps, dg_nbase, dg_nbp, dg_npass;
    unsigned long long dg_f, dg_c, dg_e, dg_r;
    unsigned long long dg_redo;
};
__shared__ KShared k_sh;

template <typename OT, typename ST = OT>
struct KRows {
    GP<ST> base;
    unsigned cM, cst2, sstr, chs;
    unsigned urow, nuloff, trash;
    int depth, depth2;
    bool perjob;
    unsigned extent;
};
#ifdef SR_BOUNDS
__device__ __forceinline__ void kbnd_fail(unsigned what, unsigned off, unsigned ext) {
    atomicOr(&b_sh.err, SR_DEV_ERR_ADDRESS);
    if (atomicCAS(&k_sh.bnd_flag, 0, 1) == 0) { k_sh.bnd_off = off; k_sh.bnd_ext = ext; k_sh.bnd_what = what; }
}
#define SR_BND_OK(R, CELL, WHAT) (((CELL) + 3u < (R).extent) ? true : (kbnd_fail((WHAT), (CELL), (R).extent), false))
#else
#define SR_BND_OK(R, CELL, WHAT) true
#endif
struct KAdr { unsigned hb, cM, cst2, sst; int slotM, slotD, depth, depth2; };
template <typename OT, typename ST>
__device__ __forceinline__ KAdr kadr(const KRows<OT, ST> &R, const BJob &jb, int slots) {
    KAdr A;
    if (R.perjob) { const unsigned hw = RFL(jb.hw); A.hb = RFL(jb.hbase); A.cM = hw; A.cst2 = hw; A.sst = 5u * hw; }
    else { A.hb = 0u; A.cM = R.cM; A.cst2 = R.cst2; A.sst = R.sstr; }
    A.slotM = slots & 0xffff; A.slotD = (int)((unsigned)slots >> 16); A.depth = R.depth; A.depth2 = R.depth2;
    return A;
}
template <typename OT, typename ST>
__device__ __forceinline__ int kslots(const KRows<OT, ST> &R, int s) { return (s % R.depth) | ((s % R.depth2) << 16); }
#define SR_RING_BIAS 24576
typedef short __attribute__((ext_vector_type(4))) S4;
template <typename OT, typename ST> __device__ __forceinline__ V4<OT> kcvt_in(V4<ST> v) {
    if constexpr (sizeof(ST) == sizeof(OT)) return v;
    else { const V4<OT> b = {SR_RING_BIAS, SR_RING_BIAS, SR_RING_BIAS, SR_RING_BIAS}; return __builtin_convertvector((S4)v, V4<OT>) + b; }
}
template <typename OT, typename ST> __device__ __forceinline__ V4<ST> kcvt_out(V4<OT> v) {
    if constexpr (sizeof(ST) == sizeof(OT)) return v;
    else { const V4<OT> b = {SR_RING_BIAS, SR_RING_BIAS, SR_RING_BIAS, SR_RING_BIAS}; return (V4<ST>)__builtin_convertvector(v - b, S4); }
}

__device__ __forceinline__ unsigned kslot(int slot0, int d, int depth) {
    int t = slot0 + d;
    t += (t < 0) ? depth : 0;
    t -= (t >= depth) ? depth : 0;
    return (unsigned)t;
}
template <typename OT, typename ST>
__device__ __forceinline__ unsigned klane(const KRows<OT, ST> &R, unsigned idx) { return (idx >> 8) * R.chs + (idx & 255u); }
template <typename OT, typename ST>
__device__ __forceinline__ unsigned krow_rel(const KRows<OT, ST> &R, const KAdr &A, int s0, int lvl, int c) {
    if (lvl < 0) return R.nuloff;
    if (c == SR_C_M) return A.hb + kslot(A.slotM, lvl - s0, A.depth) * A.sst;
    return A.hb + A.cM + (unsigned)(c - 1) * A.cst2 + kslot(A.slotD, lvl - s0, A.depth2) * A.sst;
}
template <typename OT, typename ST>
__device__ __forceinline__ unsigned krow_abs(const KRows<OT, ST> &R, int lvl, int c) {
    if (c == SR_C_M) return (unsigned)(lvl % R.depth) * R.sstr;
    return R.cM + (unsigned)(c - 1) * R.cst2 + (unsigned)(lvl % R.depth2) * R.sstr;
}
template <typename OT, typename ST>
__device__ __forceinline__ unsigned krow_fix(const KRows<OT, ST> &R, int c, int slot) {
    return (c == SR_C_M ? 0u : R.cM + (unsigned)(c - 1) * R.cst2) + (unsigned)slot * R.sstr;
}
#define SR_ROWPTR(R, OFF, LI) ((V4<ST> __attribute__((address_space(1))) *)((char __attribute__((address_space(1))) *)(R).base + (((OFF) + (LI)) * (unsigned)sizeof(ST))))
#define SR_BND_WHAT(R) ((R).perjob ? 2u : 1u)
template <typename OT> __device__ __forceinline__ V4<OT> knull4() { const V4<OT> n = {(OT)NULLV, (OT)NULLV, (OT)NULLV, (OT)NULLV}; return n; }
template <typename OT, typename ST> __device__ __forceinline__ V4<OT> rld(const KRows<OT, ST> &R, unsigned off, unsigned li) {
    if (!SR_BND_OK(R, off + li, SR_BND_WHAT(R))) return knull4<OT>();
    return kcvt_in<OT, ST>(*SR_ROWPTR(R, off, li));
}
template <typename OT, typename ST> __device__ __forceinline__ V4<OT> rld_nt(const KRows<OT, ST> &R, unsigned off, unsigned li) {
    if (!SR_BND_OK(R, off + li, SR_BND_WHAT(R))) return knull4<OT>();
    return kcvt_in<OT, ST>(__builtin_nontemporal_load(SR_ROWPTR(R, off, li)));
}
template <typename OT, typename ST> __device__ __forceinline__ void rst(const KRows<OT, ST> &R, unsigned off, unsigned li, V4<OT> v) {
    if (!SR_BND_OK(R, off + li, SR_BND_WHAT(R))) return;
    *SR_ROWPTR(R, off, li) = kcvt_out<OT, ST>(v);
}
template <typename OT, typename ST> __device__ __forceinline__ void rst_nt(const KRows<OT, ST> &R, unsigned off, unsigned li, V4<OT> v) {
    if (!SR_BND_OK(R, off + li, SR_BND_WHAT(R))) return;
    __builtin_nontemporal_store(kcvt_out<OT, ST>(v), SR_ROWPTR(R, off, li));
}
template <typename OT, typename ST> __device__ __forceinline__ int rcell(const KRows<OT, ST> &R, unsigned off, int idx) {
    if (!SR_BND_OK(R, off + klane(R, (unsigned)idx), SR_BND_WHAT(R))) return NULLV;
    const int v = (int)R.base[off + klane(R, (unsigned)idx)];
    return sizeof(ST) == sizeof(OT) ? v : (int)(short)v + SR_RING_BIAS;
}
template <typename OT, typename ST> __device__ __forceinline__ void rput(const KRows<OT, ST> &R, unsigned off, unsigned idx, int val) {
    if (!SR_BND_OK(R, off + klane(R, idx), SR_BND_WHAT(R))) return;
    R.base[off + klane(R, idx)] = (ST)(sizeof(ST) == sizeof(OT) ? val : val - SR_RING_BIAS);
}

typedef char __attribute__((address_space(1))) *GPB;
#define KBLK_C 4
template <typename OT, typename ST>
__device__ __forceinline__ GPB kbase(const KRows<OT, ST> &R, unsigned off_cells) { return (GPB)R.base + (size_t)off_cells * sizeof(ST); }
#define SR_IMMPTR(B, LANE_B, IMM) ((V4<ST> __attribute__((address_space(1))) *)((B) + (LANE_B) + (IMM) * (256 * (int)sizeof(ST))))
__device__ __forceinline__ unsigned kopaque_v(unsigned l) { asm volatile("" : "+v"(l)); return l; }
__device__ __forceinline__ int kopaque_s(int x) { asm volatile("" : "+s"(x)); return x; }
#define SR_IMMCELL(R, B, LANE_B, IMM) ((unsigned)(((B) - (GPB)(R).base) / (long)sizeof(ST)) + (LANE_B) / (unsigned)sizeof(ST) + (unsigned)((IMM) * 256))
template <typename OT, typename ST, typename KR> __device__ __forceinline__ V4<OT> ild(const KR &R, GPB b, unsigned lane_b, int imm) {
    if (!SR_BND_OK(R, SR_IMMCELL(R, b, lane_b, imm), 1u)) return knull4<OT>();
    return kcvt_in<OT, ST>(*SR_IMMPTR(b, lane_b, imm));
}
template <typename OT, typename ST, typename KR> __device__ __forceinline__ V4<OT> ild_nt(const KR &R, GPB b, unsigned lane_b, int imm) {
    if (!SR_BND_OK(R, SR_IMMCELL(R, b, lane_b, imm), 1u)) return knull4<OT>();
    return kcvt_in<OT, ST>(__builtin_nontemporal_load(SR_IMMPTR(b, lane_b, imm)));
}
template <typename OT, typename ST, typename KR> __device__ __forceinline__ void ist(const KR &R, GPB b, unsigned lane_b, int imm, V4<OT> v) {
    if (!SR_BND_OK(R, SR_IMMCELL(R, b, lane_b, imm), 1u)) return;
    *SR_IMMPTR(b, lane_b, imm) = kcvt_out<OT, ST>(v);
}
template <typename OT, typename ST, typename KR> __device__ __forceinline__ void ist_nt(const KR &R, GPB b, unsigned lane_b, int imm, V4<OT> v) {
    if (!SR_BND_OK(R, SR_IMMCELL(R, b, lane_b, imm), 1u)) return;
    __builtin_nontemporal_store(kcvt_out<OT, ST>(v), SR_IMMPTR(b, lane_b, imm));
}
// ... 34 lines not shown
```

### seqrush_amd/csrc/sr_host.cpp

```cpp
#include <hip/hip_runtime_api.h>
#include <algorithm>
#include <chrono>
#include <climits>
#include <functional>
#include <queue>
#include <cmath>
#include <cstdio>
#include <cstdlib>
#include <cstring>
#include <string>
#include <unordered_map>
#include <unordered_set>
#include <vector>
#include "../../include/seqrush_amd.h"
#include "sr_internal.h"
#include "sr_graph.h"
#include "sr_sort.h"
#include "sr_compact.h"
#include "sr_iter_rule.h"
#include "sr_inv_rule.h"
#include "sr_base_cone.h"
#include "sr_mirror_rule.h"

static thread_local std::string g_err;
static int fail(int code, const std::string &msg) { g_err = msg; return code; }
int sr_fail(int code, const std::string &msg) { return fail(code, msg); }
extern "C" const char *sr_last_error(void) { return g_err.c_str(); }

struct SrKnob { const char *name, *unset, *doc; };
static const SrKnob SR_KNOBS[] = {
    {"SR_ALIGN_IMPL", "2 when the penalties have a blocked instance", "1 = level-per-pass kernel (sr_align_bfs_kernel), 2 = score-blocked kernel"},
    {"SR_BLK_LEVELS", "10 for x=5, o1+e1=10", "5 = generic 5-level blocked instance instead of the exact 10-level one"},
    {"SR_ALIGN_THREADS", "by pairs per CU", "threads per workgroup: 64 | 128 | 256 | 512 | 1024"},
    {"SR_WG_PER_CU", "4", "workgroups per CU the launch is sized for"},
    {"SR_NWG", "CUs x workgroups per CU", "cap on workgroups (several pairs per workgroup on small inputs)"},
    {"SR_RING_U16", "1 below 57 k", "0 = 32-bit searches keep 32-bit ring rows"},
    {"SR_LAZY_ID", "1", "0 = searches store their I/D rows from the first level (no recompute pass)"},
    {"SR_HIST_JOBS", "4", "worst-case base cases the per-workgroup history holds (1..16)"},
    {"SR_BFS_BASE_JOBS", "16 (lean builds 4 / 8)", "base cases per batch"},
    {"SR_CIGAR_ARENA_OPS", "25 % of free memory", "CIGAR arena in ops (tests: force batches)"},
    {"SR_POISON_ROWS", "off", "fill the row workspaces with this offset before the run (stale-row tests)"},
    {"SR_PREORIENT", "by pairs per CU and LDS", "1 / 0 = orientation as its own kernel / inside the alignment kernel"},
    {"SR_NO_REORDER", "off", "keep list order instead of the cost-sorted dequeue order"},
    {"SR_ORIENT_LEVELS", "off", "orientation level by level even for the default penalties"},
    {"SR_NO_KBITS", "off", "no q-gram bound in the orientation kernel"},
    {"SR_NO_MIRROR", "off", "1 = no pair has a mirror partner: (q, t) and (t, q) are both aligned (A/B runs, tests)"},
    {"SR_MIRROR_REPLAY", "on", "0 = a tied secondary is aligned in full: its primary keeps no breakpoint records and none is matched (A/B runs, tests)"},
    {"SR_NO_FUSED_UNITE", "off", "sr_ctx_run launches sr_unite_kernel per batch instead of uniting inside the blocked alignment kernel"},
    {"SR_PROFILE_TICKS", "0", "1 = launch the instrumented instance (100 MHz tick counters, per-workgroup timeline)"},
    {"SR_TAIL", "on", "0 = no tail launch: a tied secondary is always aligned by its primary's workgroup (A/B runs); all = every such secondary is deferred to the tail launch (tests)"},
    {"SR_TAIL_THREADS", "widest instance wider than the main launch", "threads per workgroup of the tail launch among the existing instances: 256 | 512 | 1024 (tests)"},
    {"SR_TAIL_ROUNDS", "8", "a batch defers only when its alignments are at most this many times the launch's workgroups"},
    {"SR_FORCE_INT32", "off", "tests: 32-bit offsets (and the 16-bit ring of 32-bit searches) whatever the sequence length"},
    {"SR_TEST_BASE_LEVELS", "off", "tests: cap on the levels a base case is given at first (forces the re-queue path)"},
    {"SR_BOUNDS_DETAIL", "off", "1 = (bounds-checked build) keep the first offending access in counters[40..43]"},
};
static const char *knob(const char *name) {
    for (const SrKnob &k : SR_KNOBS)
        if (!strcmp(k.name, name)) return getenv(name);
    fprintf(stderr, "seqrush_amd: internal error: environment knob %s is not in SR_KNOBS\n", name);
    abort();
}
static std::string knobs_json() {
    std::string out = "{";
    for (const SrKnob &k : SR_KNOBS)
        if (const char *v = getenv(k.name)) {
            if (out.size() > 1) out += ", ";
            out += std::string("\"") + k.name + "\": \"";
            for (const char *q = v; *q; q++) if (*q != '"' && *q != '\\' && (unsigned char)*q >= 32) out += *q;
            out += "\"";
        }
    return out + "}";
}
extern "C" const char *sr_knobs_doc(void) {
    static std::string doc;
    if (doc.empty())
        for (const SrKnob &k : SR_KNOBS) doc += std::string(k.name) + "\t" + k.unset + "\t" + k.doc + "\n";
    return doc.c_str();
}
extern "C" int sr_abi_version(void) { return SR_ABI_VERSION; }
extern "C" void sr_free(void *p) { free(p); }
extern "C" int sr_device_count(void) {
    int n = 0;
    if (hipGetDeviceCount(&n) != hipSuccess) return 0;
    return n;
}

#define HIPCHK(expr)                                                                     \
    do {                                                                                 \
        hipError_t _e = (expr);                                                          \
        if (_e != hipSuccess)                                                            \
            return fail(SR_ERR_HIP, std::string(#expr) + ": " + hipGetErrorString(_e));  \
    } while (0)

extern "C" void sr_default_params(sr_params *p) {
    memset(p, 0, sizeof(*p));
    p->match_score = 0; p->mismatch_penalty = 5; p->gap_open1 = 8; p->gap_ext1 = 2;
    p->gap_open2 = 24; p->gap_ext2 = 1;
    p->ori_match = 0; p->ori_mismatch = 1; p->ori_gap_open = 1; p->ori_gap_ext = 1;
    p->min_match_len = 0; p->max_divergence = -1.0; p->exclude_self = 0;
    p->memory_mode = SR_MEM_ULTRALOW; p->sparsify_kind = SR_SPARSE_NONE; p->sparsify_factor = 1.0;
    p->sparsify_seed = 42; p->canonical_labels = 0; p->device = 0;
    p->shard_rank = 0; p->shard_count = 1;
    p->tree_k_nearest = 0; p->tree_k_farthest = 0; p->tree_rand_frac = 0.0; p->tree_kmer = 16;
}

static bool parse_i32(const std::string &s, int32_t *out) {
    if (s.empty() || s.size() > 15) return false;
    size_t i = (s[0] == '+' || s[0] == '-') ? 1 : 0;
    if (i == s.size()) return false;
    for (size_t j = i; j < s.size(); j++) if (s[j] < '0' || s[j] > '9') return false;
    long long v = atoll(s.c_str());
    if (v > INT32_MAX || v < INT32_MIN) return false;
    *out = (int32_t)v;
    return true;
}
static std::vector<std::string> split(const std::string &s, char c) {
    std::vector<std::string> out;
    size_t st = 0;
    for (;;) {
        size_t p = s.find(c, st);
        if (p == std::string::npos) { out.push_back(s.substr(st)); break; }
        out.push_back(s.substr(st, p - st));
        st = p + 1;
    }
    return out;
}

extern "C" int sr_parse_scores(const char *s, sr_params *p) {
    auto parts = split(s, ',');
    if (parts.size() < 4)
        return fail(SR_ERR_INVALID, "Scores must have at least 4 values: match,mismatch,gap1_open,gap1_extend");
    if (parts.size() > 6) return fail(SR_ERR_INVALID, "Too many score values provided (max 6)");
    int32_t v[6] = {0, 0, 0, 0, -1, -1};
    static const char *nm[6] = {"match score", "mismatch penalty", "gap1_open penalty",
                                "gap1_extend penalty", "gap2_open penalty", "gap2_extend penalty"};
    for (int i = 0; i < 4; i++)
        if (!parse_i32(parts[i], &v[i])) return fail(SR_ERR_INVALID, std::string("Invalid ") + nm[i] + ": " + parts[i]);
    if (parts.size() >= 6)
        for (int i = 4; i < 6; i++)
            if (!parse_i32(parts[i], &v[i])) return fail(SR_ERR_INVALID, std::string("Invalid ") + nm[i] + ": " + parts[i]);
    p->match_score = v[0]; p->mismatch_penalty = v[1]; p->gap_open1 = v[2]; p->gap_ext1 = v[3];
    p->gap_open2 = v[4]; p->gap_ext2 = v[5];
    return SR_OK;
}

extern "C" int sr_parse_orientation_scores(const char *s, sr_params *p) {
    auto parts = split(s, ',');
    if (parts.size() != 4)
        return fail(SR_ERR_INVALID, "Orientation scores must have exactly 4 values: match,mismatch,gap_open,gap_extend");
    int32_t v[4];
    for (int i = 0; i < 4; i++)
        if (!parse_i32(parts[i], &v[i])) return fail(SR_ERR_INVALID, "Invalid orientation score: " + parts[i]);
    p->ori_match = v[0]; p->ori_mismatch = v[1]; p->ori_gap_open = v[2]; p->ori_gap_ext = v[3];
    return SR_OK;
}

static bool parse_f64(const std::string &s, double *out) {
    if (s.empty() || isspace((unsigned char)s[0])) return false;
    for (char ch : s) if (ch == 'x' || ch == 'X') return false;
    char *end;
    double v = strtod(s.c_str(), &end);
    if (*end != 0) return false;
    *out = v;
    return true;
}

extern "C" int sr_parse_sparsification(const char *cs, sr_params *p) {
    std::string s(cs);
    if (s == "none" || s == "1.0") { p->sparsify_kind = SR_SPARSE_NONE; return SR_OK; }
    if (s == "auto") { p->sparsify_kind = SR_SPARSE_AUTO; return SR_OK; }
    double f;
    if (s.rfind("random:", 0) == 0) {
        if (!parse_f64(s.substr(7), &f)) return fail(SR_ERR_INVALID, "Invalid random factor: " + s);
        if (f > 0.0 && f <= 1.0) { p->sparsify_kind = SR_SPARSE_RANDOM; p->sparsify_factor = f; return SR_OK; }
        return fail(SR_ERR_INVALID, "Random factor must be in (0.0, 1.0]");
    }
    if (s.rfind("connectivity:", 0) == 0) {
        if (!parse_f64(s.substr(13), &f)) return fail(SR_ERR_INVALID, "Invalid connectivity probability: " + s);
        if (f > 0.0 && f <= 1.0) { p->sparsify_kind = SR_SPARSE_CONNECTIVITY; p->sparsify_factor = f; return SR_OK; }
        return fail(SR_ERR_INVALID, "Connectivity probability must be in (0.0, 1.0]");
    }
    if (s.rfind("tree:", 0) == 0) {
        auto parts = split(s.substr(5), ',');
        if (parts.empty() || parts.size() > 4)
            return fail(SR_ERR_INVALID, "Tree sampling requires 1-4 values: tree:neighbor[,stranger[,random[,k-mer]]], got " + s);
        auto parse_usize = [](const std::string &t, uint64_t *v) {
            size_t i = (!t.empty() && t[0] == '+') ? 1 : 0;
            if (i >= t.size()) return false;
            *v = 0;
            for (; i < t.size(); i++) {
                if (t[i] < '0' || t[i] > '9') return false;
                const uint64_t dgt = (uint64_t)(t[i] - '0');
                if (*v > (0xffffffffffffffffULL - dgt) / 10) return false;
                *v = *v * 10 + dgt;
            }
            return true;
        };
        uint64_t kn = 0, kf = 0, km = 16;
        double rf = 0.0;
        if (!parse_usize(parts[0], &kn)) return fail(SR_ERR_INVALID, "Invalid neighbor count: " + parts[0]);
        if (parts.size() >= 2 && !parse_usize(parts[1], &kf)) return fail(SR_ERR_INVALID, "Invalid stranger count: " + parts[1]);
        if (parts.size() >= 3) {
            if (!parse_f64(parts[2], &rf)) return fail(SR_ERR_INVALID, "Invalid random fraction: " + parts[2]);
            if (rf < 0.0 || rf > 1.0) return fail(SR_ERR_INVALID, "Random fraction must be in [0.0, 1.0], got " + parts[2]);
        }
        if (parts.size() >= 4) {
            if (!parse_usize(parts[3], &km)) return fail(SR_ERR_INVALID, "Invalid k-mer size: " + parts[3]);
            if (km == 0) return fail(SR_ERR_INVALID, "K-mer size must be > 0");
        }
        p->sparsify_kind = SR_SPARSE_TREE;
        p->tree_k_nearest = (uint32_t)std::min<uint64_t>(kn, 0xffffffffULL);
        p->tree_k_farthest = (uint32_t)std::min<uint64_t>(kf, 0xffffffffULL);
        p->tree_rand_frac = rf; p->tree_kmer = (uint32_t)std::min<uint64_t>(km, 0xffffffffULL);
        return SR_OK;
    }
    if (parse_f64(s, &f) && f > 0.0 && f <= 1.0) { p->sparsify_kind = SR_SPARSE_RANDOM; p->sparsify_factor = f; return SR_OK; }
    return fail(SR_ERR_INVALID, "Invalid sparsification: '" + s + "'");
}

static int32_t max_score_for_divergence(const sr_params &p, uint64_t seq_len, double d) {
    int32_t max_mismatches = (int32_t)std::ceil((double)seq_len * d);
    int32_t max_gaps = (int32_t)std::ceil((double)seq_len * d * 0.5);
    int32_t mismatch_score = max_mismatches * p.mismatch_penalty;
    int32_t gap_score = max_gaps > 0 ? p.gap_open1 + (max_gaps - 1) * p.gap_ext1 : 0;
    return std::max(mismatch_score + gap_score, p.mismatch_penalty * 2);
}

#define SR_TAIL_ROUNDS_DEFAULT 8

struct sr_ctx {
    int device = 0;
    hipStream_t stream = nullptr;
    bool own_stream = false;
    sr_params prm;
    uint32_t n = 0;
    std::vector<uint32_t> len;
    std::vector<uint64_t> goff;
    uint64_t total_len = 0, uf_size = 0;
    std::vector<uint32_t> pair_q, pair_t;
    std::vector<uint64_t> cigar_base;
    std::vector<uint32_t> batch_first;
    uint64_t total_pairs_all_ranks = 0;
    uint64_t dp_cells = 0;
    int off16 = 1, nwg = 0, nthreads = 256, symbits = 2;
    size_t lds_bytes = 0;
    SrAlignArgs aa{};
    SrUniteArgs ua{};
    std::vector<void *> dev_allocs;
    unsigned long long *d_nodes = nullptr, *d_minarr = nullptr, *d_labels = nullptr;
    unsigned long long *d_counters = nullptr;
    int *d_error = nullptr;
    uint32_t *d_queue = nullptr, *d_oqueue = nullptr, *d_order = nullptr;
    uint64_t *d_okeys = nullptr, *d_okeys2 = nullptr;
    uint32_t *d_ovals = nullptr; void *d_otemp = nullptr; size_t otemp_bytes = 0;
    uint64_t *d_cbase = nullptr;
    uint8_t *d_bases = nullptr;
    int onwg = 0;
    size_t olds_bytes = 0;
    int32_t *d_max_score = nullptr;
    uint32_t *d_mirror = nullptr;
    uint64_t mirror_partners = 0;
    int tail_threads = 0, tail_wg_per_cu = 1, tail_rounds = SR_TAIL_ROUNDS_DEFAULT, tail_cus = 0;
    bool tail_all = false;
    std::vector<uint32_t> batch_partners;
    uint32_t *d_tail_list = nullptr, *d_tail_deferred = nullptr;
    unsigned long long *d_timeline = nullptr;
    std::vector<std::pair<hipEvent_t, hipEvent_t>> ev[5];
    int ev_used[5] = {0, 0, 0, 0, 0};
    bool loaded = false;
    bool fuse_unite = false;
    bool from_paf = false;
    bool aligned_batch_valid = false;
    std::string workspace_report;
    bool iter_loaded = false, iter_keep = false, iter_ran = false;
    uint64_t iter_tree_pairs = 0;
    uint32_t iter_tree_batches = 0, iter_max_chunks = 0;
    sr_iter_stats iter_stats{};
    std::vector<uint64_t> iter_counts;
    SrIterState *d_iter_state = nullptr;
    unsigned long long *d_iter_counts = nullptr;
    sr_alignments *iter_al = nullptr;
    bool inv_on = false, inv_keep = false;
    uint64_t inv_m = 0;
    uint32_t *d_inv_count = nullptr, *d_inv_off = nullptr;
    unsigned long long *d_inv_stats = nullptr;
    SrInvJob *d_inv_jobs = nullptr;
    uint64_t inv_job_cap = 0;
    std::vector<SrInvJob> inv_raw;
    std::vector<sr_inv_job> inv_jobs;
    sr_inv_stats inv_stats{};
    sr_alignments *inv_al = nullptr;
    std::vector<std::pair<hipEvent_t, hipEvent_t>> inv_ev;
    uint32_t inv_join = 0;
    SrInvJobJ *d_inv_jobs_j = nullptr;
    uint64_t inv_job_cap_j = 0;
    std::vector<SrInvJobJ> inv_raw_j;
    uint64_t inv_join_stats[4] = {0, 0, 0, 0};
    std::chrono::steady_clock::time_point t_first_kernel;
    int inv_ev_used = 0;
};

static int dev_alloc(sr_ctx *c, void **p, size_t bytes) {
    hipError_t e = hipMalloc(p, bytes ? bytes : 16);
    if (e != hipSuccess) {
        char buf[160];
        snprintf(buf, sizeof(buf), "hipMalloc of %zu bytes failed: %s", bytes, hipGetErrorString(e));
        return fail(e == hipErrorOutOfMemory ? SR_ERR_NOMEM : SR_ERR_HIP, buf);
    }
    c->dev_allocs.push_back(*p);
    return SR_OK;
}
static void free_dev(sr_ctx *c) {
    for (void *p : c->dev_allocs) (void)hipFree(p);
    c->dev_allocs.clear();
    c->d_nodes = c->d_minarr = c->d_labels = c->d_counters = nullptr;
    c->d_error = nullptr; c->d_queue = nullptr; c->d_oqueue = nullptr; c->d_order = nullptr; c->d_cbase = nullptr;
    c->d_bases = nullptr; c->d_max_score = nullptr; c->d_mirror = nullptr; c->mirror_partners = 0; c->onwg = 0;
    c->tail_threads = 0; c->tail_all = false; c->batch_partners.clear(); c->d_tail_list = c->d_tail_deferred = nullptr; c->d_timeline = nullptr;
    c->d_okeys = c->d_okeys2 = nullptr; c->d_ovals = nullptr; c->d_otemp = nullptr; c->otemp_bytes = 0;
    c->loaded = false; c->from_paf = false; c->aligned_batch_valid = false;
    for (int k = 0; k < 5; k++) c->ev_used[k] = 0;
    c->iter_loaded = c->iter_keep = c->iter_ran = false; c->iter_tree_pairs = 0; c->iter_tree_batches = c->iter_max_chunks = 0;
    c->iter_counts.clear(); c->d_iter_state = nullptr; c->d_iter_counts = nullptr; c->iter_stats = sr_iter_stats{};
    if (c->iter_al) { sr_alignments_free(c->iter_al); c->iter_al = nullptr; }
    c->inv_on = c->inv_keep = false; c->inv_m = 0; c->d_inv_count = c->d_inv_off = nullptr; c->d_inv_stats = nullptr;
    c->d_inv_jobs = nullptr; c->inv_job_cap = 0; c->inv_raw.clear(); c->inv_jobs.clear(); c->inv_stats = sr_inv_stats{};
    c->inv_join = 0; c->d_inv_jobs_j = nullptr; c->inv_job_cap_j = 0; c->inv_raw_j.clear();
    for (uint64_t &v : c->inv_join_stats) v = 0;
    c->inv_ev_used = 0;
    if (c->inv_al) { sr_alignments_free(c->inv_al); c->inv_al = nullptr; }
}

static int ev_get(sr_ctx *c, int kind, int idx, hipEvent_t **a, hipEvent_t **b) {
    while ((int)c->ev[kind].size() <= idx) {
        hipEvent_t x = nullptr, y = nullptr;
        HIPCHK(hipEventCreate(&x)); HIPCHK(hipEventCreate(&y));
        c->ev[kind].push_back({x, y});
    }
    *a = &c->ev[kind][idx].first; *b = &c->ev[kind][idx].second;
    return SR_OK;
}

extern "C" int sr_ctx_create(int device, sr_ctx **out) {
    int n = 0;
    if (hipGetDeviceCount(&n) != hipSuccess || n == 0)
        return fail(SR_ERR_NO_DEVICE, "no HIP device available (seqrush_amd has no CPU fallback)");
    if (device < 0 || device >= n) return fail(SR_ERR_INVALID, "device ordinal out of range");
    HIPCHK(hipSetDevice(device));
    sr_ctx *c = new sr_ctx();
    c->device = device;
    if (hipStreamCreate(&c->stream) != hipSuccess) { delete c; return fail(SR_ERR_HIP, "hipStreamCreate failed"); }
    c->own_stream = true;
    *out = c;
    return SR_OK;
}

extern "C" void sr_ctx_destroy(sr_ctx *c) {
    if (!c) return;
    (void)hipSetDevice(c->device);
    (void)hipStreamSynchronize(c->stream);
    free_dev(c);
    for (int k = 0; k < 5; k++)
        for (auto &e : c->ev[k]) { (void)hipEventDestroy(e.first); (void)hipEventDestroy(e.second); }
    for (auto &e : c->inv_ev) { (void)hipEventDestroy(e.first); (void)hipEventDestroy(e.second); }
    if (c->own_stream && c->stream) (void)hipStreamDestroy(c->stream);
    delete c;
}

extern "C" int sr_ctx_set_stream(sr_ctx *c, void *hip_stream) {
    if (!c) return fail(SR_ERR_INVALID, "null ctx");
    if (c->own_stream && c->stream) { (void)hipStreamSynchronize(c->stream); (void)hipStreamDestroy(c->stream); }
    c->stream = (hipStream_t)hip_stream;
    c->own_stream = false;
    return SR_OK;
}

static inline uint8_t comp_base(uint8_t b) {
    switch (b) {
    case 'A': case 'a': return 'T'; case 'T': case 't': return 'A';
    case 'C': case 'c': return 'G'; case 'G': case 'g': return 'C';
    default: return b;
    }
}

static uint64_t splitmix64(uint64_t x) {
    x += 0x9e3779b97f4a7c15ULL;
    x = (x ^ (x >> 30)) * 0xbf58476d1ce4e5b9ULL;
    x = (x ^ (x >> 27)) * 0x94d049bb133111ebULL;
    return x ^ (x >> 31);
}
static inline double unit53(uint64_t h) { return (double)(h >> 11) * (1.0 / 9007199254740992.0); }

static double connectivity_fraction(uint32_t n, double P) {
    if (n <= 2 || P >= 1.0) return 1.0;
    const double c = -std::log(-std::log(P));
    const double f = (std::log((double)n) + c) / (double)n;
    return f >= 1.0 ? 1.0 : (f <= 0.0 ? 0.0 : f);
}

static void enumerate_pairs(uint32_t n, const sr_params &p, const uint8_t *sel, std::vector<uint32_t> &pq, std::vector<uint32_t> &pt) {
    pq.clear(); pt.clear();
    int kind = p.sparsify_kind;
    double frac = p.sparsify_factor;
    if (kind == SR_SPARSE_AUTO) { if (n < 10) kind = SR_SPARSE_NONE; else { kind = SR_SPARSE_CONNECTIVITY; frac = 0.99; } }
    const double conn_f = (kind == SR_SPARSE_CONNECTIVITY) ? connectivity_fraction(n, frac) : 1.0;
    for (uint32_t q = 0; q < n; q++)
        for (uint32_t t = 0; t < n; t++) {
            if (q == t) { if (p.exclude_self) continue; pq.push_back(q); pt.push_back(t); continue; }
            const uint32_t i = std::min(q, t), j = std::max(q, t);
            bool keep = true;
            if (kind == SR_SPARSE_RANDOM)
                keep = unit53(splitmix64(p.sparsify_seed ^ ((uint64_t)q * n + t))) < frac;
            else if (kind == SR_SPARSE_CONNECTIVITY)
                keep = unit53(splitmix64(p.sparsify_seed ^ ((uint64_t)i * n + j))) < conn_f;
            else if (kind == SR_SPARSE_TREE)
                keep = (sel && (sel[(uint64_t)i * n + j] || sel[(uint64_t)j * n + i])) ||
                       unit53(splitmix64(p.sparsify_seed ^ ((uint64_t)i * n + j))) < p.tree_rand_frac;
            if (keep) { pq.push_back(q); pt.push_back(t); }
        }
}

static void iterative_lists(uint32_t n, const uint8_t *sel, uint64_t seed, double rf, std::vector<uint32_t> &ti,
                            std::vector<uint32_t> &tj, std::vector<uint32_t> &ri, std::vector<uint32_t> &rj) {
    ti.clear(); tj.clear(); ri.clear(); rj.clear();
    struct R { uint64_t h; uint32_t i, j; };
    std::vector<R> rnd;
    for (uint32_t i = 0; i < n; i++)
        for (uint32_t j = i + 1; j < n; j++) {
            if (sel && (sel[(uint64_t)i * n + j] || sel[(uint64_t)j * n + i])) { ti.push_back(i); tj.push_back(j); continue; }
            const uint64_t h = splitmix64(seed ^ ((uint64_t)i * n + j));
            if (unit53(h) < rf) rnd.push_back({h, i, j});
        }
    std::sort(rnd.begin(), rnd.end(), [](const R &a, const R &b) {
        return a.h != b.h ? a.h < b.h : (a.i != b.i ? a.i < b.i : a.j < b.j); });
    for (const R &e : rnd) { ri.push_back(e.i); rj.push_back(e.j); }
}

static uint32_t *copy_out_u32(const std::vector<uint32_t> &v) {
    uint32_t *o = (uint32_t *)malloc((v.empty() ? 1 : v.size()) * 4);
    if (o) memcpy(o, v.data(), v.size() * 4);
    return o;
}

extern "C" int sr_iterative_pair_lists(uint32_t n, const uint8_t *sel, const sr_params *p, uint32_t **tree_i, uint32_t **tree_j,
                                       uint64_t *tree_count, uint32_t **rand_i, uint32_t **rand_j, uint64_t *rand_count) {
    if (!p || !tree_i || !tree_j || !tree_count || !rand_i || !rand_j || !rand_count) return fail(SR_ERR_INVALID, "null argument");
    std::vector<uint32_t> ti, tj, ri, rj;
    iterative_lists(n, sel, p->sparsify_seed, p->tree_rand_frac, ti, tj, ri, rj);
    *tree_i = copy_out_u32(ti); *tree_j = copy_out_u32(tj); *rand_i = copy_out_u32(ri); *rand_j = copy_out_u32(rj);
    *tree_count = ti.size(); *rand_count = ri.size();
    return SR_OK;
}

static void shard_pairs(const std::vector<uint32_t> &len, uint32_t rank, uint32_t count, std::vector<uint32_t> &pq,
                        std::vector<uint32_t> &pt) {
    if (count <= 1) return;
    const size_t m = pq.size();
    std::vector<uint64_t> cost(m);
    for (size_t i = 0; i < m; i++)
        cost[i] = pq[i] == pt[i] ? (uint64_t)len[pq[i]] : (uint64_t)len[pq[i]] * (uint64_t)len[pt[i]];
    std::vector<uint32_t> idx(m);
    for (size_t i = 0; i < m; i++) idx[i] = (uint32_t)i;
    std::stable_sort(idx.begin(), idx.end(), [&](uint32_t a, uint32_t b) { return cost[a] > cost[b]; });
    typedef std::pair<uint64_t, uint32_t> LR;
    std::priority_queue<LR, std::vector<LR>, std::greater<LR>> heap;
    for (uint32_t r = 0; r < count; r++) heap.push({0, r});
    std::vector<uint8_t> mine(m, 0);
    for (uint32_t i : idx) {
        LR top = heap.top(); heap.pop();
        if (top.second == rank) mine[i] = 1;
        top.first += cost[i] ? cost[i] : 1;
// ... 454 lines not shown
    pl.hist_w = (2 * (rmax + pen.scope + 2) + 1 + 8 + 64 + 7) & ~7;
    pl.brow = (int)((4 * maxlen + 32 * 72 + 64 + 512 + 7) & ~7ULL);
    pl.kdepth = std::max(pen.scope + std::max(kblock, 1), ori.scope + 1) + 1;
    const char *lz = knob("SR_LAZY_ID");
    pl.lazy_id = (impl == 2 && !(lz && atoi(lz) == 0) && 2 * pen.scope + 2 * kblock + 2 <= SR_BLK_MAK_SLOTS) ? 1 : 0;
    pl.kdepth2 = pl.kdepth;
    if (pl.lazy_id) {
        pl.kdepth2 = std::max(pl.kdepth, pen.scope + 2 * kblock + 2);
        pl.kdepth = std::max(pl.kdepth, 2 * pen.scope + 2 * kblock + 2);
    }
    if (impl == 2 && kblock == 10) {
        pl.kdepth = (pl.kdepth + 9) / 10 * 10; pl.kdepth2 = (pl.kdepth2 + 9) / 10 * 10;
    }
    pl.bring_wg = ((uint64_t)(pl.ring_scope + 1) + 4ULL * pl.ring_hot + 4ULL * (pl.ring_scope + 1) + 2ULL) * (uint64_t)pl.brow;
    if (impl == 2) pl.bring_wg = ((uint64_t)pl.brow / 256 + 2ULL) * ((uint64_t)pl.kdepth + 4ULL * pl.kdepth2 + (uint64_t)SR_NULL_ROWS + 2ULL) * 256ULL + 1024;
    if (impl == 2 && pl.bring_wg * pl.rsz >= (1ULL << 32)) return fail(SR_ERR_UNSUPPORTED, "sequences too long for the device row workspace (4 GB per workgroup)");
    const uint64_t hist_worst = (uint64_t)pl.hist_levels * 5 * (uint64_t)pl.hist_w;
    pl.hist_cap = hist_worst * 4;
    if (const char *e = knob("SR_HIST_JOBS")) pl.hist_cap = hist_worst * (uint64_t)std::max(1, std::min(16, atoi(e)));
    pl.hist_nul_w = impl == 2 ? (uint64_t)pl.hist_w + 256 : (uint64_t)pl.bbase_jobs * (uint64_t)pl.hist_w;
    pl.bhist_wg = impl == 2 ? ((pl.hist_cap + pl.hist_nul_w + 256 + 1024 + 7) & ~7ULL)
                            : ((uint64_t)pl.hist_levels * 5 + 1) * pl.hist_nul_w + 1024;
    pl.bseg_wg = 2ULL * SR_BFS_MAXSEG * SR_BFS_SEGREC * 4;
    pl.bbt_wg = (uint64_t)pl.bbase_jobs * SR_BFS_BTCAP * 4;
    pl.brec_wg = impl == 2 ? (uint64_t)SR_BPREC_MAX * SR_BPREC_INTS * 4 : 0;
    pl.bcl_wg = 0;
    pl.per_wg_bytes = pl.bring_wg * pl.rsz + pl.bhist_wg * pl.osz + pl.bseg_wg + pl.bbt_wg + pl.bcl_wg * 4 + (impl == 2 ? 32 * SR_BLK_MAK_SLOTS * 4 : 0) +
                      pl.brec_wg;
    (void)c;
    return SR_OK;
}

static int plan_memory(sr_ctx *c, uint32_t np, Plan &pl, bool iterative = false) {
    size_t total_b = 0;
    HIPCHK(hipMemGetInfo(&pl.free_b, &total_b));
    const uint64_t fixed = 3ULL * c->uf_size * 8 + (uint64_t)np * 40 + (1ULL << 20);
    if (fixed + (64ULL << 20) > pl.free_b) return fail(SR_ERR_NOMEM, "not enough device memory for the union-find arrays");
    const uint64_t avail = pl.free_b - fixed;
    pl.arena_ops = c->cigar_base[np] + 1;
    {
        uint64_t cap = std::max<uint64_t>((uint64_t)(avail * 0.25) / 4, pl.max_reserve + 1);
        if (const char *e = knob("SR_CIGAR_ARENA_OPS")) cap = std::max<uint64_t>((uint64_t)atoll(e), pl.max_reserve + 1);
        if (iterative)
            for (uint64_t f = c->iter_tree_pairs; f < np; f += 4 * SR_ITER_CHECK_INTERVAL)
                cap = std::max<uint64_t>(cap, c->cigar_base[std::min<uint64_t>(np, f + 4 * SR_ITER_CHECK_INTERVAL)] - c->cigar_base[f] + 1);
        pl.arena_ops = std::min(pl.arena_ops, cap);
    }
    if (pl.arena_ops * 4 > avail / 2) return fail(SR_ERR_NOMEM, "not enough device memory for one pair's CIGAR");
    c->batch_first.assign(1, 0);
    const uint32_t tp = iterative ? (uint32_t)c->iter_tree_pairs : np;
    for (uint32_t i = 0; i < tp; i++)
        if (c->cigar_base[i + 1] - c->cigar_base[c->batch_first.back()] + 1 > pl.arena_ops) c->batch_first.push_back(i);
    if (iterative) {
        if (tp > 0 && tp < np) c->batch_first.push_back(tp);
        c->iter_tree_batches = tp == 0 ? 0 : (tp < np ? (uint32_t)c->batch_first.size() - 1 : (uint32_t)c->batch_first.size());
        const uint32_t CH = 4 * SR_ITER_CHECK_INTERVAL;
        uint64_t target = SR_ITER_STABILITY_THRESHOLD;
        c->iter_max_chunks = 0;
        for (uint32_t f = tp; f < np;) {
            uint32_t l = f, chunks = 0;
            while (l < np && (chunks == 0 || chunks < target)) {
                const uint32_t e = std::min(np, l + CH);
                if (chunks > 0 && c->cigar_base[e] - c->cigar_base[f] + 1 > pl.arena_ops) break;
                l = e; chunks++;
            }
            c->iter_max_chunks = std::max(c->iter_max_chunks, chunks);
            if (l < np) c->batch_first.push_back(l);
            f = l;
            target = std::min<uint64_t>(2 * target, 1ULL << 32);
        }
    } else {
        c->iter_tree_batches = 0;
    }
    c->batch_first.push_back(np);
    pl.nbatch = (uint32_t)c->batch_first.size() - 1;
    pl.max_batch_pairs = 0;
    for (uint32_t b = 0; b < pl.nbatch; b++) pl.max_batch_pairs = std::max(pl.max_batch_pairs, c->batch_first[b + 1] - c->batch_first[b]);
    pl.left = avail - pl.arena_ops * 4;
    const uint64_t budget = (uint64_t)(pl.left * 0.7);
    int nwg = pl.cus * pl.wg_per_cu;
    if (const char *e = knob("SR_NWG")) nwg = std::max(1, std::min(nwg, atoi(e)));
    if ((uint64_t)nwg > pl.max_batch_pairs) nwg = (int)pl.max_batch_pairs;
    if (nwg < 1) nwg = 1;
    while (nwg > 1 && (uint64_t)nwg * pl.per_wg_bytes > budget) nwg--;
    if ((uint64_t)nwg * pl.per_wg_bytes > budget) return fail(SR_ERR_NOMEM, "not enough device memory for one workgroup's wavefront ring");
    pl.nwg = c->nwg = nwg;
    return SR_OK;
}

static int alloc_workspace(sr_ctx *c, const sr_params *p, const PackedSeqs &pk, const SeqDev &sd, const SrPen &pen, const SrPen &ori,
                           uint64_t maxlen, const std::vector<int32_t> &max_score, Plan &pl, bool forced_strand = false) {
    int r;
    void *d;
    const uint32_t np = (uint32_t)c->pair_q.size(), nbatch = pl.nbatch;
    const int impl = pl.impl, nwg = pl.nwg;
    const size_t osz = pl.osz, rsz = pl.rsz;
    SrAlignArgs &a = c->aa;
    memset(&a, 0, sizeof(a));
    uint32_t *d_pq, *d_pt;
    std::vector<uint32_t> pq = c->pair_q, pt = c->pair_t;
    if (pq.empty()) { pq.push_back(0); pt.push_back(0); }
    DEV_UPLOAD(d_pq, uint32_t, pq);
    DEV_UPLOAD(d_pt, uint32_t, pt);
    std::vector<uint64_t> cb((size_t)np + nbatch, 0);
    for (uint32_t b = 0; b < nbatch; b++) {
        const uint32_t f = c->batch_first[b], l = c->batch_first[b + 1];
        for (uint32_t i = f; i <= l; i++) cb[(size_t)i + b] = c->cigar_base[i] - c->cigar_base[f];
    }
    DEV_UPLOAD(c->d_cbase, uint64_t, cb);
    std::vector<uint32_t> order(std::max<uint32_t>(np, 1), 0);
    for (uint32_t b = 0; b < nbatch; b++) {
        const uint32_t f = c->batch_first[b], l = c->batch_first[b + 1];
        std::vector<uint32_t> idx(l - f);
        for (uint32_t i = 0; i < l - f; i++) idx[i] = i;
        auto cost = [&](uint32_t i) { const uint32_t q = c->pair_q[f + i], t = c->pair_t[f + i];
                                      return q == t ? (uint64_t)c->len[q] : (uint64_t)c->len[q] * c->len[t]; };
        std::stable_sort(idx.begin(), idx.end(), [&](uint32_t x, uint32_t y) { return cost(x) > cost(y); });
        for (uint32_t i = 0; i < l - f; i++) order[f + i] = idx[i];
    }
    DEV_UPLOAD(c->d_order, uint32_t, order);
    DEV_UPLOAD(c->d_max_score, int32_t, max_score);
    std::vector<uint32_t> mirror;
    c->mirror_partners = 0;
    if (impl == 2 && pk.sm.bits == 2 && !forced_strand && np > 0) {
        mirror.assign(np, SR_MIRROR_NONE);
        if (!knob("SR_NO_MIRROR")) c->mirror_partners = mirror_map(c->pair_q.data(), c->pair_t.data(), c->batch_first.data(), nbatch, (uint32_t)nwg, mirror.data());
        DEV_UPLOAD(c->d_mirror, uint32_t, mirror);
    }
    c->batch_partners.assign(nbatch, 0);
    uint32_t max_partners = 0;
    for (uint32_t b = 0; b < nbatch && !mirror.empty(); b++) {
        for (uint32_t i = c->batch_first[b]; i < c->batch_first[b + 1]; i++)
            if (mirror[i] != SR_MIRROR_NONE && !(mirror[i] & SR_MIRROR_SECONDARY)) c->batch_partners[b]++;
        max_partners = std::max(max_partners, c->batch_partners[b]);
    }
    HIPCHK(hipStreamSynchronize(c->stream));
    if ((r = dev_alloc(c, &d, 4 * sizeof(uint32_t)))) return r; c->d_queue = (uint32_t *)d;
    c->tail_threads = c->mirror_partners > 0 ? pl.tail_threads : 0;
    pl.tail_threads = c->tail_threads;
    if (c->tail_threads) {
        c->tail_wg_per_cu = (int)std::max<size_t>(1, std::min<size_t>((size_t)1024 / c->tail_threads,
                                                                      (160 * 1024) / (c->lds_bytes + align_static_lds(false, 2, c->tail_threads))));
        const char *tl = knob("SR_TAIL"), *tr = knob("SR_TAIL_ROUNDS");
        c->tail_all = tl && !strcmp(tl, "all");
        c->tail_rounds = tr ? std::max(0, atoi(tr)) : SR_TAIL_ROUNDS_DEFAULT;
        c->tail_cus = pl.cus;
        if ((r = dev_alloc(c, &d, (size_t)max_partners * 4))) return r; c->d_tail_list = (uint32_t *)d;
        if ((r = dev_alloc(c, &d, sizeof(uint32_t)))) return r; c->d_tail_deferred = (uint32_t *)d;
        HIPCHK(hipMemsetAsync(c->d_tail_deferred, 0, sizeof(uint32_t), c->stream));
    }
    if (impl == 2 && knob("SR_PROFILE_TICKS") && atoi(knob("SR_PROFILE_TICKS")) != 0) {
        if ((r = dev_alloc(c, &d, (size_t)nwg * 4 * 8))) return r; c->d_timeline = (unsigned long long *)d;
        HIPCHK(hipMemsetAsync(c->d_timeline, 0, (size_t)nwg * 4 * 8, c->stream));
    }
    if ((r = dev_alloc(c, &d, (uint64_t)nwg * pl.bring_wg * rsz))) return r; a.bring = d;
    if ((r = dev_alloc(c, &d, (uint64_t)nwg * pl.bhist_wg * osz))) return r; a.bhist = d;
    if (const char *e = knob("SR_POISON_ROWS")) {
        const int v = atoi(e);
        if (rsz == 2) HIPCHK(hipMemsetD16Async((hipDeviceptr_t)a.bring, (unsigned short)(pl.ring_u16 ? v - 24576 : v), (size_t)nwg * pl.bring_wg, c->stream));
        else HIPCHK(hipMemsetD32Async((hipDeviceptr_t)a.bring, v, (size_t)nwg * pl.bring_wg, c->stream));
        if (osz == 2) HIPCHK(hipMemsetD16Async((hipDeviceptr_t)a.bhist, (unsigned short)v, (size_t)nwg * pl.bhist_wg, c->stream));
        else HIPCHK(hipMemsetD32Async((hipDeviceptr_t)a.bhist, v, (size_t)nwg * pl.bhist_wg, c->stream));
    }
    if ((r = dev_alloc(c, &d, (uint64_t)nwg * pl.bseg_wg))) return r; a.bseg = (int *)d;
    if ((r = dev_alloc(c, &d, (uint64_t)nwg * pl.bbt_wg))) return r; a.bbt = (uint32_t *)d;
    {
        const char *rpk = knob("SR_MIRROR_REPLAY");
        pl.brec_bytes = 0;
        if (impl == 2 && c->mirror_partners > 0 && pl.brec_wg && !(rpk && atoi(rpk) == 0)) {
            pl.brec_bytes = (uint64_t)nwg * pl.brec_wg;
            if ((r = dev_alloc(c, &d, pl.brec_bytes))) return r; a.brec = (int *)d;
        }
    }
    if (pl.bcl_wg) { if ((r = dev_alloc(c, &d, (uint64_t)nwg * pl.bcl_wg * 4))) return r; a.bcl = (uint32_t *)d; a.bcl_wg_stride = pl.bcl_wg; }
    if (impl == 2) { if ((r = dev_alloc(c, &d, (uint64_t)nwg * 32 * SR_BLK_MAK_SLOTS * 4))) return r; a.bmak = (int *)d; }
    const char *po = knob("SR_PREORIENT");
    const bool pre_auto = (uint64_t)np >= 4ULL * (uint64_t)pl.cus && (size_t)pl.max_words * 12 <= 20 * 1024;
    if (!forced_strand && impl == 2 && (po ? atoi(po) != 0 : pre_auto) && (size_t)pl.max_words * 12 <= 60 * 1024) {
        const int orow = (int)((2 * ((2 * maxlen + 32) & ~3ULL) + 512 + 7) & ~7ULL);
        const uint64_t oring_wg = ((uint64_t)(ori.scope + 1) * 3 + 1) * (uint64_t)orow + 256;
        int onwg = (int)std::min<uint64_t>(pl.max_batch_pairs, (uint64_t)pl.cus * 16);
        while (onwg > 1 && (uint64_t)onwg * oring_wg * osz > (uint64_t)(pl.left * 0.2)) onwg--;
        if (onwg >= 1 && np > 0) {
            pl.oring_bytes = (uint64_t)onwg * oring_wg * osz;
            if ((r = dev_alloc(c, &d, pl.oring_bytes))) return r; a.oring = d;
            if ((r = dev_alloc(c, &d, sizeof(uint32_t)))) return r; c->d_oqueue = (uint32_t *)d;
            a.oring_wg_stride = oring_wg; a.orow = orow; a.oqueue = c->d_oqueue; a.pre_oriented = 1;
            if (!knob("SR_NO_REORDER")) {
                c->otemp_bytes = srk_order_temp_bytes(pl.max_batch_pairs);
                if ((r = dev_alloc(c, &d, (uint64_t)pl.max_batch_pairs * 8))) return r; c->d_okeys = (uint64_t *)d;
                if ((r = dev_alloc(c, &d, (uint64_t)pl.max_batch_pairs * 8))) return r; c->d_okeys2 = (uint64_t *)d;
                if ((r = dev_alloc(c, &d, (uint64_t)pl.max_batch_pairs * 4))) return r; c->d_ovals = (uint32_t *)d;
                if ((r = dev_alloc(c, &d, std::max<size_t>(c->otemp_bytes, 16)))) return r; c->d_otemp = d;
            }
            c->onwg = onwg; c->olds_bytes = (size_t)pl.max_words * 3 * 4;
        }
    }
    if ((r = dev_alloc(c, &d, (size_t)np + 1))) return r; a.is_reverse = (uint8_t *)d;
    if ((r = dev_alloc(c, &d, ((size_t)np + 1) * 4))) return r; a.score = (int32_t *)d;
    if ((r = dev_alloc(c, &d, ((size_t)np + 1) * 4))) return r; a.ori_fwd = (int32_t *)d;
    if ((r = dev_alloc(c, &d, ((size_t)np + 1) * 4))) return r; a.ori_rev = (int32_t *)d;
    if ((r = dev_alloc(c, &d, ((size_t)np + 1) * 4))) return r; a.cigar_cnt = (uint32_t *)d;
    if ((r = dev_alloc(c, &d, (pl.arena_ops + 1) * 4))) return r; a.cigar_ops = (uint32_t *)d;
    if ((r = dev_alloc(c, &d, SR_NCOUNTERS * sizeof(unsigned long long)))) return r; c->d_counters = (unsigned long long *)d;
    if ((r = dev_alloc(c, &d, sizeof(int)))) return r; c->d_error = (int *)d;
    if ((r = dev_alloc(c, &d, c->uf_size * 8))) return r; c->d_nodes = (unsigned long long *)d;
    if ((r = dev_alloc(c, &d, c->uf_size * 8))) return r; c->d_minarr = (unsigned long long *)d;
    if ((r = dev_alloc(c, &d, c->uf_size * 8))) return r; c->d_labels = (unsigned long long *)d;
    HIPCHK(hipMemsetAsync(c->d_counters, 0, SR_NCOUNTERS * sizeof(unsigned long long), c->stream));
    HIPCHK(hipMemsetAsync(c->d_error, 0, sizeof(int), c->stream));
    HIPCHK(hipMemsetAsync(a.cigar_cnt, 0, ((size_t)np + 1) * 4, c->stream));
    HIPCHK(hipMemsetAsync(a.score, 0xff, ((size_t)np + 1) * 4, c->stream));
    if (forced_strand) {
        HIPCHK(hipMemsetAsync(a.is_reverse, 0, (size_t)np + 1, c->stream));
        HIPCHK(hipMemsetAsync(a.ori_fwd, 0, ((size_t)np + 1) * 4, c->stream));
        HIPCHK(hipMemsetAsync(a.ori_rev, 0, ((size_t)np + 1) * 4, c->stream));
    }
    a.seqwords = sd.words; a.word_off_fwd = sd.woff[0]; a.word_off_rc = sd.woff[1]; a.word_off_rev = sd.woff[2]; a.word_off_cmp = sd.woff[3];
    if (forced_strand) { if (impl == 2) a.pre_oriented = 1; else a.word_off_rc = a.word_off_fwd; }
    a.symbits = pk.sm.bits; a.order = c->d_order; a.seqlen = sd.len;
    a.max_words = pl.max_words; a.pair_q = d_pq; a.pair_t = d_pt; a.npairs = np;
    a.queue_head = c->d_queue; a.pen = pen; a.ori = ori; a.mem_mode = p->memory_mode;
    a.ring_scope = pl.ring_scope; a.ring_hot = pl.ring_hot;
    a.hist_w = pl.hist_w; a.hist_levels = pl.hist_levels;
    { const char *pt_ = knob("SR_PROFILE_TICKS"); a.profile_ticks = (pt_ && atoi(pt_) != 0) ? 1 : 0; }
    a.impl = impl; a.kdepth = pl.kdepth; a.kdepth2 = pl.kdepth2; a.kblock = pl.kblock; a.lazy_id = pl.lazy_id; a.ring_u16 = pl.ring_u16;
    a.ori_levels = knob("SR_ORIENT_LEVELS") ? 1 : 0;
    { const char *tb = knob("SR_TEST_BASE_LEVELS"); a.test_base_levels = tb ? std::max(0, atoi(tb)) : 0; }
    a.bring_wg_stride = pl.bring_wg; a.brow = pl.brow; a.bhist_wg_stride = pl.bhist_wg; a.bbase_jobs = pl.bbase_jobs;
    a.hist_cap = pl.hist_cap; a.hist_nul_w = (uint32_t)pl.hist_nul_w; a.hist_stride = (uint32_t)((uint64_t)pl.bbase_jobs * (uint64_t)pl.hist_w);
    a.cigar_base = c->d_cbase; a.counters = c->d_counters; a.error_flag = c->d_error;
    if (a.pre_oriented && pk.sm.bits == 2 && !ori.two && ori.x == 1 && ori.o1 == 1 && ori.e1 == 1 && !knob("SR_NO_KBITS") && !knob("SR_ORIENT_LEVELS")) {
        const uint64_t kb = (uint64_t)c->len.size() * 8192ull;
        if (kb > 0 && kb <= (256ull << 20) && kb <= (uint64_t)(pl.left * 0.05)) {
            if ((r = dev_alloc(c, &d, kb))) return r;
            if ((r = srk_kmer_bits(&a, (uint32_t)c->len.size(), (uint32_t *)d, c->stream))) return fail(SR_ERR_DEVICE_FAULT, "k-mer set kernel failed to launch");
            a.kbits = (const uint32_t *)d;
        }
    }
    SrUniteArgs &u = c->ua;
    memset(&u, 0, sizeof(u));
    u.pair_q = d_pq; u.pair_t = d_pt; u.npairs = np; u.seqlen = sd.len; u.seq_goff = sd.goff;
    a.fuse_unite = 0; a.uf_nodes = c->d_nodes; a.seq_goff = sd.goff; a.max_score = c->d_max_score; a.min_match_len = p->min_match_len;
    a.mirror = c->d_mirror;
    a.tail_count = c->d_queue + 1; a.tail_head = c->d_queue + 2; a.tail_deferred = c->d_tail_deferred; a.timeline = c->d_timeline;
    c->fuse_unite = impl == 2 && !knob("SR_NO_FUSED_UNITE");
    u.is_reverse = a.is_reverse; u.score = a.score; u.max_score = c->d_max_score;
    u.cigar_ops = a.cigar_ops; u.cigar_base = c->d_cbase; u.cigar_cnt = a.cigar_cnt;
    u.min_match_len = p->min_match_len; u.nodes = c->d_nodes; u.uf_size = c->uf_size;
    u.counters = c->d_counters; u.error_flag = c->d_error;
    return SR_OK;
}

static void write_report(sr_ctx *c, const PackedSeqs &pk, const SrPen &pen, const Plan &pl) {
    const uint32_t np = (uint32_t)c->pair_q.size();
    char buf[2048];
    const SrPen &ori = c->aa.ori;
    const char *oroute = c->onwg == 0 ? "in-kernel"
                         : (!ori.two && ori.x == 1 && ori.o1 == 1 && ori.e1 == 1 && !knob("SR_ORIENT_LEVELS")) ? "orient-blk" : "orient-levels";
    snprintf(buf, sizeof(buf),
             "{\"pairs\": %u, \"batches\": %u, \"symbol_bits\": %d, \"offset_bytes\": %zu, \"ring_cell_bytes\": %zu, \"kernel_impl\": %d, "
             "\"block_levels\": %d, \"two_piece\": %d, \"lazy_id_rows\": %d, \"workgroups\": %d, "
             "\"threads_per_workgroup\": %d, \"workgroups_per_cu\": %d, \"lds_dynamic_bytes\": %zu, \"ring_bytes_per_workgroup\": %llu, "
             "\"base_history_bytes_per_workgroup\": %llu, \"workspace_bytes\": %llu, \"cigar_arena_bytes\": %llu, "
             "\"orientation_ring_bytes\": %llu, \"union_find_bytes\": %llu, \"device_free_bytes_at_load\": %zu, \"kernel_build\": \"%s\", "
             "\"ring_depth_m\": %d, \"ring_depth_id\": %d, \"fused_unite\": %d, \"wave_build\": %d, \"level_kernel_wide\": %d, "
             "\"profile_ticks\": %d, \"orientation_route\": \"%s\", \"source_digest\": \"%s\", \"mirror_partners\": %llu, \"tail_threads\": %d, \"mirror_replay\": %d, \"replay_record_bytes\": %llu, \"knobs\": ",
             np, pl.nbatch, pk.sm.bits, pl.osz, pl.impl == 2 ? pl.rsz : pl.osz, pl.impl, pl.impl == 2 ? pl.kblock : 1, pen.two ? 1 : 0, pl.lazy_id,
             pl.nwg, c->nthreads, pl.wg_per_cu, c->lds_bytes,
             (unsigned long long)(pl.bring_wg * pl.rsz), (unsigned long long)(pl.bhist_wg * pl.osz),
             (unsigned long long)((uint64_t)pl.nwg * pl.per_wg_bytes), (unsigned long long)(pl.arena_ops * 4), (unsigned long long)pl.oring_bytes,
             (unsigned long long)(3ULL * c->uf_size * 8), pl.free_b, srk_align_blk_build_tag(), pl.kdepth, pl.kdepth2, c->fuse_unite ? 1 : 0,
             pl.wave_wg ? 1 : 0, (pl.impl == 1 && pl.ring_scope + 1 > 32) ? 1 : 0, c->aa.profile_ticks, oroute, srk_source_digest(),
             (unsigned long long)c->mirror_partners, c->tail_threads, pl.brec_bytes ? 1 : 0, (unsigned long long)pl.brec_bytes);
    c->workspace_report = std::string(buf) + knobs_json() + "}";
}

static int load_impl(sr_ctx *c, const sr_seqset *seqs, const sr_params *p, const uint32_t *eq, const uint32_t *et,
                     uint64_t ecount, bool explicit_pairs, bool iterative = false, bool forced_strand = false) {
    if (!c || !seqs || !p) return fail(SR_ERR_INVALID, "null argument");
    if (seqs->n == 0) return fail(SR_ERR_INVALID, "no sequences");
    HIPCHK(hipSetDevice(c->device));
    HIPCHK(hipStreamSynchronize(c->stream));
    free_dev(c);
    int r;
    SrPen pen, ori;
    uint64_t maxlen = 0;
    if ((r = load_index(c, seqs, p, explicit_pairs, &pen, &ori, &maxlen))) return r;
    PackedSeqs pk;
    pack_sequences(c, seqs, pk);
    c->symbits = pk.sm.bits;
    SeqDev sd;
    if ((r = upload_sequences(c, seqs, pk, sd))) return r;
    Plan pl;
    std::vector<int32_t> max_score;
    if ((r = build_pair_list(c, p, sd, eq, et, ecount, explicit_pairs, max_score, &pl.max_reserve, iterative))) return r;
    const uint32_t np = (uint32_t)c->pair_q.size();
    if ((r = plan_kernel(c, pk, pen, ori, maxlen, np, pl))) return r;
    if ((r = plan_workspace(c, pen, ori, maxlen, pl))) return r;
    if ((r = plan_memory(c, np, pl, iterative))) return r;
    if ((r = alloc_workspace(c, p, pk, sd, pen, ori, maxlen, max_score, pl, forced_strand))) return r;
    write_report(c, pk, pen, pl);
    c->t_first_kernel = std::chrono::steady_clock::now();
    if (srk_uf_init(c->d_nodes, c->total_len, c->uf_size, c->stream)) return fail(SR_ERR_HIP, "uf init launch failed");
    HIPCHK(hipStreamSynchronize(c->stream));
    c->loaded = true;
    return SR_OK;
}
#undef DEV_UPLOAD

extern "C" int sr_ctx_load(sr_ctx *c, const sr_seqset *seqs, const sr_params *p) {
    return load_impl(c, seqs, p, nullptr, nullptr, 0, false);
}
extern "C" int sr_ctx_load_pairs(sr_ctx *c, const sr_seqset *seqs, const sr_params *p, const uint32_t *query_idx,
                                 const uint32_t *target_idx, uint64_t count) {
    if (count && (!query_idx || !target_idx)) return fail(SR_ERR_INVALID, "null pair list");
    return load_impl(c, seqs, p, query_idx, target_idx, count, true);
}

extern "C" int sr_ctx_pairs(const sr_ctx *c, uint32_t **q_out, uint32_t **t_out, uint64_t *count) {
    if (!c || !c->loaded || !q_out || !t_out || !count) return fail(SR_ERR_INVALID, "context not loaded");
    const size_t m = c->pair_q.size();
    *count = m;
    *q_out = (uint32_t *)malloc((m ? m : 1) * 4);
    *t_out = (uint32_t *)malloc((m ? m : 1) * 4);
    memcpy(*q_out, c->pair_q.data(), m * 4);
    memcpy(*t_out, c->pair_t.data(), m * 4);
    return SR_OK;
}
extern "C" int sr_ctx_orientation_scores(sr_ctx *c, int32_t *fwd, int32_t *rev) {
    if (!c || !c->loaded || c->from_paf || !c->aa.ori_fwd) return fail(SR_ERR_INVALID, "context has no alignment stage");
    const size_t np = c->pair_q.size();
    HIPCHK(hipSetDevice(c->device));
    HIPCHK(hipStreamSynchronize(c->stream));
    if (fwd && np) HIPCHK(hipMemcpy(fwd, c->aa.ori_fwd, np * 4, hipMemcpyDeviceToHost));
    if (rev && np) HIPCHK(hipMemcpy(rev, c->aa.ori_rev, np * 4, hipMemcpyDeviceToHost));
    return SR_OK;
}
extern "C" uint32_t sr_ctx_num_batches(const sr_ctx *c) { return (c && c->loaded) ? (uint32_t)c->batch_first.size() - 1 : 0; }
extern "C" const char *sr_ctx_workspace_report(const sr_ctx *c) { return c ? c->workspace_report.c_str() : ""; }

extern "C" int sr_ctx_reset_uf(sr_ctx *c) {
    if (!c || !c->loaded) return fail(SR_ERR_INVALID, "context not loaded");
    HIPCHK(hipSetDevice(c->device));
    if (srk_uf_init(c->d_nodes, c->total_len, c->uf_size, c->stream)) return fail(SR_ERR_HIP, "uf init launch failed");
    return SR_OK;
}

static void batch_args(const sr_ctx *c, uint32_t b, SrAlignArgs *a, SrUniteArgs *u) {
    const uint32_t f = c->batch_first[b], cnt = c->batch_first[b + 1] - f;
    if (a) {
        *a = c->aa;
        a->pair_q += f; a->pair_t += f; a->npairs = cnt; if (a->order) a->order += f;
        a->is_reverse += f; a->score += f; a->ori_fwd += f; a->ori_rev += f; a->cigar_cnt += f;
        if (a->max_score) a->max_score += f;
        if (a->mirror) a->mirror += f;
        a->cigar_base = c->d_cbase + f + b;
    }
    if (u) {
        *u = c->ua;
        u->pair_q += f; u->pair_t += f; u->npairs = cnt; u->is_reverse += f; u->score += f; u->max_score += f;
        u->cigar_cnt += f; u->cigar_base = c->d_cbase + f + b;
        if (u->q_start) { u->q_start += f; u->t_start += f; }
    }
}

static int enqueue_align_batch(sr_ctx *c, uint32_t b, bool fuse_unite = false) {
    SrAlignArgs a;
    batch_args(c, b, &a, nullptr);
    a.fuse_unite = fuse_unite ? 1 : 0;
    const int main_wg = std::min<int>(c->nwg, (int)a.npairs);
    const uint32_t partners = c->tail_threads && b < c->batch_partners.size() ? c->batch_partners[b] : 0;
    const bool defer = partners > 0 && (c->tail_all || (uint64_t)(a.npairs - partners) <= (uint64_t)c->tail_rounds * (uint64_t)main_wg);
    a.tail_list = defer ? c->d_tail_list : nullptr;
    a.tail_mode = defer && c->tail_all ? SR_TAIL_DEFER_ALL : SR_TAIL_MAIN;
    HIPCHK(hipMemsetAsync(c->d_queue, 0, (c->tail_threads ? 3 : 1) * sizeof(uint32_t), c->stream));
    hipEvent_t *e0, *e1;
    int r;
    if (c->onwg > 0 && a.npairs > 0) {
        HIPCHK(hipMemsetAsync(c->d_oqueue, 0, sizeof(uint32_t), c->stream));
        if ((r = ev_get(c, 4, c->ev_used[4], &e0, &e1))) return r;
        HIPCHK(hipEventRecord(*e0, c->stream));
        r = srk_orient(&a, std::min<int>(c->onwg, (int)a.npairs), c->olds_bytes, c->off16, c->stream);
        if (r) return fail(SR_ERR_HIP, std::string("orientation kernel launch failed: ") + hipGetErrorString((hipError_t)r));
        if (c->d_okeys && a.order) {
            r = srk_order(&a, c->d_okeys, c->d_okeys2, c->d_ovals, c->d_otemp, c->otemp_bytes, (uint32_t *)a.order, c->stream);
            if (r) return fail(SR_ERR_HIP, std::string("dequeue-order sort failed: ") + hipGetErrorString((hipError_t)r));
        }
        HIPCHK(hipEventRecord(*e1, c->stream));
        c->ev_used[4]++;
    }
    if ((r = ev_get(c, 0, c->ev_used[0], &e0, &e1))) return r;
    HIPCHK(hipEventRecord(*e0, c->stream));
    if (a.npairs > 0) {
        r = srk_align(&a, main_wg, c->lds_bytes, c->off16, c->nthreads, c->stream);
        if (r) return fail(SR_ERR_HIP, std::string("align kernel launch failed: ") + hipGetErrorString((hipError_t)r));
        if (defer) {
            const int grid = (int)std::min<uint64_t>({(uint64_t)c->tail_cus * (uint64_t)c->tail_wg_per_cu, (uint64_t)c->nwg, (uint64_t)partners});
            a.tail_mode = SR_TAIL_RUN; a.timeline = nullptr;
            r = srk_align(&a, grid, c->lds_bytes, c->off16, c->tail_threads, c->stream);
            if (r) return fail(SR_ERR_HIP, std::string("align kernel tail launch failed: ") + hipGetErrorString((hipError_t)r));
        }
    }
    HIPCHK(hipEventRecord(*e1, c->stream));
    c->ev_used[0]++;
    return SR_OK;
}

static int enqueue_unite_batch(sr_ctx *c, uint32_t b, bool fused = false) {
    SrUniteArgs u;
    batch_args(c, b, nullptr, &u);
    hipEvent_t *e0, *e1;
    int r;
    if ((r = ev_get(c, 1, c->ev_used[1], &e0, &e1))) return r;
    HIPCHK(hipEventRecord(*e0, c->stream));
    if (u.npairs > 0 && !fused) {
        int nwg = (int)std::min<uint64_t>(u.npairs, 4096);
        r = srk_unite(&u, nwg, c->stream);
        if (r) return fail(SR_ERR_HIP, std::string("unite kernel launch failed: ") + hipGetErrorString((hipError_t)r));
    }
    HIPCHK(hipEventRecord(*e1, c->stream));
    c->ev_used[1]++;
    return SR_OK;
}

static int begin_pass(sr_ctx *c, bool reset_counters) {
    HIPCHK(hipSetDevice(c->device));
    if (reset_counters) {
        HIPCHK(hipMemsetAsync(c->d_counters, 0, SR_NCOUNTERS * sizeof(unsigned long long), c->stream));
        if (c->d_tail_deferred) HIPCHK(hipMemsetAsync(c->d_tail_deferred, 0, sizeof(uint32_t), c->stream));
        c->ev_used[0] = c->ev_used[4] = 0;
    }
    return SR_OK;
}

extern "C" int sr_ctx_align(sr_ctx *c) {
    if (!c || !c->loaded) return fail(SR_ERR_INVALID, "context not loaded");
    if (c->from_paf) return fail(SR_ERR_INVALID, "context was loaded from a PAF file: there is no alignment stage");
    if (c->batch_first.size() > 2)
        return fail(SR_ERR_UNSUPPORTED, "the pair list runs in several batches that share one CIGAR arena: use sr_ctx_run "
                                        "(align + unite per batch) or sr_align_all");
    int r = begin_pass(c, true);
    if (r) return r;
    if ((r = enqueue_align_batch(c, 0))) return r;
    c->aligned_batch_valid = true;
    return SR_OK;
}

extern "C" int sr_ctx_unite(sr_ctx *c) {
    if (!c || !c->loaded) return fail(SR_ERR_INVALID, "context not loaded");
    if (c->batch_first.size() > 2) return fail(SR_ERR_UNSUPPORTED, "several batches: use sr_ctx_run");
    HIPCHK(hipSetDevice(c->device));
    c->ev_used[1] = 0;
    return enqueue_unite_batch(c, 0);
}

static int inv_begin_run(sr_ctx *c);
static int inv_scan_batch(sr_ctx *c, uint32_t b);
static int inv_patch_pass(sr_ctx *c);

extern "C" int sr_ctx_run(sr_ctx *c) {
    if (!c || !c->loaded) return fail(SR_ERR_INVALID, "context not loaded");
    int r = begin_pass(c, !c->from_paf);
    if (r) return r;
    c->ev_used[1] = 0;
    const uint32_t nbatch = (uint32_t)c->batch_first.size() - 1;
    const bool fuse = c->fuse_unite && !c->from_paf;
    if (c->inv_on && (r = inv_begin_run(c))) return r;
    for (uint32_t b = 0; b < nbatch; b++) {
        if (!c->from_paf && (r = enqueue_align_batch(c, b, fuse))) return r;
        if ((r = enqueue_unite_batch(c, b, fuse))) return r;
        if (c->inv_on && (r = inv_scan_batch(c, b))) return r;
    }
    c->aligned_batch_valid = nbatch == 1 && !c->from_paf;
    if (c->inv_on && (r = inv_patch_pass(c))) return r;
    return SR_OK;
}

extern "C" int sr_ctx_sync(sr_ctx *c) {
    if (!c) return fail(SR_ERR_INVALID, "null ctx");
    HIPCHK(hipSetDevice(c->device));
    HIPCHK(hipStreamSynchronize(c->stream));
    if (c->loaded) {
        int err = 0;
        HIPCHK(hipMemcpy(&err, c->d_error, sizeof(int), hipMemcpyDeviceToHost));
        if (err) {
            static const char *names[9] = {"score bound exceeded", "base-case history overflow", "backtrace found no predecessor",
                                           "recursion stack / segment list overflow", "CIGAR buffer overflow", "union-find retry bound",
                                           "breakpoint outside its segment", "graph induction",
                                           "row / LDS address outside the workgroup's extent (bounds-checked build)"};
            std::string msg = "device reported internal fault bits";
            char buf[32];
            snprintf(buf, sizeof(buf), " 0x%x:", err);
            msg += buf;
            for (int b = 0; b < 9; b++) if (err & (1 << b)) { msg += " ["; msg += names[b]; msg += "]"; }
            if (err & SR_DEV_ERR_ADDRESS) {
                uint64_t d[4] = {0, 0, 0, 0};
                if (hipMemcpy(d, c->d_counters + 40, sizeof(d), hipMemcpyDeviceToHost) == hipSuccess && d[0]) {
                    char b2[160];
                    snprintf(b2, sizeof(b2), " first: pair #%llu, %s, offset %llu, extent %llu", (unsigned long long)(d[0] - 1),
                             d[1] == 1 ? "ring row" : d[1] == 2 ? "history row" : "LDS window", (unsigned long long)d[2], (unsigned long long)d[3]);
                    msg += b2;
                }
            }
            if (!c->from_paf && c->aa.score) {
                const size_t np = c->pair_q.size();
                std::vector<int32_t> sc(np);
                if (np && hipMemcpy(sc.data(), c->aa.score, np * 4, hipMemcpyDeviceToHost) == hipSuccess) {
                    int shown = 0;
                    for (size_t i = 0; i < np && shown < 4; i++)
                        if (sc[i] < 0) { snprintf(buf, sizeof(buf), " pair(%u,%u)", c->pair_q[i], c->pair_t[i]); msg += buf; shown++; }
                }
            }
            return fail(SR_ERR_DEVICE_FAULT, msg);
        }
    }
    return SR_OK;
}

extern "C" uint64_t sr_ctx_uf_size(const sr_ctx *c) { return c ? c->uf_size : 0; }
extern "C" uint64_t sr_ctx_num_pairs(const sr_ctx *c) { return c ? c->pair_q.size() : 0; }
extern "C" uint64_t sr_ctx_dp_cells(const sr_ctx *c) { return c ? c->dp_cells : 0; }

extern "C" const char *sr_ctx_align_kernel(const sr_ctx *c) {
    if (!c || !c->loaded || c->from_paf) return nullptr;
    return c->aa.impl == 2 ? "sr_align_blk_kernel" : "sr_align_bfs_kernel";
}

extern "C" int sr_ctx_kernel_ms(sr_ctx *c, int which, float *ms) {
    if (!c || which < 0 || which > 4 || c->ev_used[which] == 0) return fail(SR_ERR_INVALID, "no timing recorded");
    float tot = 0;
    for (int i = 0; i < c->ev_used[which]; i++) {
        float t = 0;
        HIPCHK(hipEventSynchronize(c->ev[which][i].second));
        HIPCHK(hipEventElapsedTime(&t, c->ev[which][i].first, c->ev[which][i].second));
        tot += t;
    }
    *ms = tot;
    return SR_OK;
}

extern "C" int sr_ctx_counters(sr_ctx *c, uint64_t out[16]) {
    if (!c || !c->loaded) return fail(SR_ERR_INVALID, "context not loaded");
    HIPCHK(hipSetDevice(c->device));
    HIPCHK(hipStreamSynchronize(c->stream));
    HIPCHK(hipMemcpy(out, c->d_counters, 16 * sizeof(uint64_t), hipMemcpyDeviceToHost));
    return SR_OK;
}

extern "C" int sr_ctx_counters_ext(sr_ctx *c, uint64_t out[32]) {
    if (!c || !c->loaded) return fail(SR_ERR_INVALID, "context not loaded");
    HIPCHK(hipSetDevice(c->device));
    HIPCHK(hipStreamSynchronize(c->stream));
    HIPCHK(hipMemcpy(out, c->d_counters, 32 * sizeof(uint64_t), hipMemcpyDeviceToHost));
    return SR_OK;
}
extern "C" int sr_ctx_counters_all(sr_ctx *c, uint64_t *out, uint32_t cap) {
    if (!c || !c->loaded || !out) return fail(SR_ERR_INVALID, "context not loaded");
    HIPCHK(hipSetDevice(c->device));
    HIPCHK(hipStreamSynchronize(c->stream));
    const uint32_t n = std::min<uint32_t>(cap, SR_NCOUNTERS);
    HIPCHK(hipMemcpy(out, c->d_counters, n * sizeof(uint64_t), hipMemcpyDeviceToHost));
    return (int)n;
}

extern "C" int sr_ctx_tail_deferred(sr_ctx *c, uint64_t *out) {
    if (!c || !c->loaded || !out) return fail(SR_ERR_INVALID, "context not loaded");
    *out = 0;
    if (!c->d_tail_deferred) return SR_OK;
    HIPCHK(hipSetDevice(c->device));
    HIPCHK(hipStreamSynchronize(c->stream));
    uint32_t v = 0;
    HIPCHK(hipMemcpy(&v, c->d_tail_deferred, sizeof(v), hipMemcpyDeviceToHost));
    *out = v;
    return SR_OK;
}
extern "C" int sr_ctx_tail_timeline(sr_ctx *c, uint64_t *out, uint32_t cap_wg) {
    if (!c || !c->loaded || !out) return fail(SR_ERR_INVALID, "context not loaded");
    if (!c->d_timeline) return 0;
    HIPCHK(hipSetDevice(c->device));
    HIPCHK(hipStreamSynchronize(c->stream));
    const uint32_t n = std::min<uint32_t>(cap_wg, (uint32_t)c->nwg);
    HIPCHK(hipMemcpy(out, c->d_timeline, (size_t)n * 4 * sizeof(uint64_t), hipMemcpyDeviceToHost));
    return (int)n;
}

extern "C" int sr_ctx_download_uf(sr_ctx *c, uint64_t *parent_out) {
    if (!c || !c->loaded) return fail(SR_ERR_INVALID, "context not loaded");
    HIPCHK(hipSetDevice(c->device));
    HIPCHK(hipStreamSynchronize(c->stream));
    HIPCHK(hipMemcpy(parent_out, c->d_nodes, c->uf_size * 8, hipMemcpyDeviceToHost));
    return SR_OK;
}

static int labels_timed(sr_ctx *c, uint64_t *dev_labels64, uint32_t *dev_labels32) {
    hipEvent_t *e0, *e1;
    int r;
    if ((r = ev_get(c, 2, 0, &e0, &e1))) return r;
    HIPCHK(hipEventRecord(*e0, c->stream));
    if (dev_labels64) {
        if (srk_labels(c->d_nodes, c->uf_size, c->d_minarr, (unsigned long long *)dev_labels64, c->d_error, c->stream))
            return fail(SR_ERR_HIP, "label kernel launch failed");
    } else {
        if (srk_labels32(c->d_nodes, c->uf_size, c->d_minarr, dev_labels32, c->d_error, c->stream))
            return fail(SR_ERR_HIP, "label kernel launch failed");
    }
    HIPCHK(hipEventRecord(*e1, c->stream));
    c->ev_used[2] = 1;
    return SR_OK;
}

extern "C" int sr_ctx_labels_device(sr_ctx *c, uint64_t *dev_labels) {
    if (!c || !c->loaded) return fail(SR_ERR_INVALID, "context not loaded");
    HIPCHK(hipSetDevice(c->device));
    return labels_timed(c, dev_labels, nullptr);
}
extern "C" int sr_ctx_labels_device_u32(sr_ctx *c, uint32_t *dev_labels) {
    if (!c || !c->loaded) return fail(SR_ERR_INVALID, "context not loaded");
    if (c->uf_size > 0xffffffffULL) return fail(SR_ERR_UNSUPPORTED, "2N+2 >= 2^32: use the 64-bit label exchange");
    HIPCHK(hipSetDevice(c->device));
    return labels_timed(c, nullptr, dev_labels);
}

extern "C" int sr_ctx_merge_labels(sr_ctx *c, const uint64_t *dev_labels, uint32_t count) {
    if (!c || !c->loaded) return fail(SR_ERR_INVALID, "context not loaded");
    HIPCHK(hipSetDevice(c->device));
    if (srk_merge(c->d_nodes, c->uf_size, (const unsigned long long *)dev_labels, count, c->d_error, c->stream))
        return fail(SR_ERR_HIP, "merge kernel launch failed");
    return SR_OK;
}
extern "C" int sr_ctx_merge_labels_u32(sr_ctx *c, const uint32_t *dev_labels, uint32_t count) {
    if (!c || !c->loaded) return fail(SR_ERR_INVALID, "context not loaded");
    if (c->uf_size > 0xffffffffULL) return fail(SR_ERR_UNSUPPORTED, "2N+2 >= 2^32: use the 64-bit label exchange");
    HIPCHK(hipSetDevice(c->device));
    if (srk_merge32(c->d_nodes, c->uf_size, dev_labels, count, c->d_error, c->stream))
        return fail(SR_ERR_HIP, "merge kernel launch failed");
    return SR_OK;
}

extern "C" int sr_ctx_merge_labels_host(sr_ctx *c, const uint64_t *labels, uint32_t count) {
    if (!c || !c->loaded || !labels) return fail(SR_ERR_INVALID, "context not loaded");
    HIPCHK(hipSetDevice(c->device));
    for (uint32_t i = 0; i < count; i++) {
        HIPCHK(hipMemcpyAsync(c->d_labels, labels + (uint64_t)i * c->uf_size, c->uf_size * 8, hipMemcpyHostToDevice, c->stream));
        if (srk_merge(c->d_nodes, c->uf_size, c->d_labels, 1, c->d_error, c->stream)) return fail(SR_ERR_HIP, "merge kernel launch failed");
    }
    return SR_OK;
}

extern "C" int sr_ctx_download_labels(sr_ctx *c, uint64_t *labels_out) {
    int r = sr_ctx_labels_device(c, (uint64_t *)c->d_labels);
    if (r) return r;
    HIPCHK(hipStreamSynchronize(c->stream));
    HIPCHK(hipMemcpy(labels_out, c->d_labels, c->uf_size * 8, hipMemcpyDeviceToHost));
    return SR_OK;
}

extern "C" void sr_alignments_free(sr_alignments *a) {
    if (!a) return;
    free(a->query_idx); free(a->target_idx); free(a->is_reverse); free(a->score);
    free(a->query_start); free(a->query_end); free(a->target_start); free(a->target_end);
    free(a->cigar_off); free(a->cigar_ops);
    free(a);
}

struct AlnAcc { std::vector<uint32_t> cnt, ops; std::vector<int32_t> score; std::vector<uint8_t> isrev; };
static int collect_batch(sr_ctx *c, uint32_t b, AlnAcc &acc) {
    const uint32_t f = c->batch_first[b], l = c->batch_first[b + 1], cntp = l - f;
    if (cntp == 0) return SR_OK;
    std::vector<uint32_t> cnt(cntp);
    HIPCHK(hipMemcpy(cnt.data(), c->aa.cigar_cnt + f, (size_t)cntp * 4, hipMemcpyDeviceToHost));
    HIPCHK(hipMemcpy(acc.score.data() + f, c->aa.score + f, (size_t)cntp * 4, hipMemcpyDeviceToHost));
    HIPCHK(hipMemcpy(acc.isrev.data() + f, c->aa.is_reverse + f, (size_t)cntp, hipMemcpyDeviceToHost));
    const uint64_t arena_used = c->cigar_base[l] - c->cigar_base[f];
    std::vector<uint32_t> raw(arena_used + 1);
    HIPCHK(hipMemcpy(raw.data(), c->aa.cigar_ops, (arena_used + 1) * 4, hipMemcpyDeviceToHost));
    for (uint32_t i = 0; i < cntp; i++) {
        acc.cnt[f + i] = cnt[i];
        const uint32_t *src = raw.data() + (c->cigar_base[f + i] - c->cigar_base[f]);
        for (uint32_t j = 0; j < cnt[i]; j++) {
            const uint32_t op = src[j] & 15u, len = src[j] >> 4;
            const uint32_t o2 = op == SR_OP_M ? 0u : op == SR_OP_X ? 1u : op == SR_OP_I ? 3u : 2u;
            acc.ops.push_back((len << 4) | o2);
        }
    }
    return SR_OK;
}

static sr_alignments *make_alignments_of(const std::vector<uint32_t> &pair_q, const std::vector<uint32_t> &pair_t,
                                         const std::vector<uint32_t> &len, const AlnAcc &acc, size_t count = SIZE_MAX);
static sr_alignments *make_alignments(const sr_ctx *c, const AlnAcc &acc, size_t count = SIZE_MAX) {
    return make_alignments_of(c->pair_q, c->pair_t, c->len, acc, count);
}
static sr_alignments *make_alignments_of(const std::vector<uint32_t> &pair_q, const std::vector<uint32_t> &pair_t,
                                         const std::vector<uint32_t> &len, const AlnAcc &acc, size_t count) {
    const size_t np = std::min(count, pair_q.size());
    sr_alignments *a = (sr_alignments *)calloc(1, sizeof(sr_alignments));
    a->n = np;
    const size_t m = np ? np : 1;
    a->query_idx = (uint32_t *)malloc(m * 4); a->target_idx = (uint32_t *)malloc(m * 4);
    a->is_reverse = (uint8_t *)malloc(m); a->score = (int32_t *)malloc(m * 4);
    a->query_start = (uint64_t *)malloc(m * 8); a->query_end = (uint64_t *)malloc(m * 8);
    a->target_start = (uint64_t *)malloc(m * 8); a->target_end = (uint64_t *)malloc(m * 8);
    a->cigar_off = (uint64_t *)malloc((np + 1) * 8);
    a->cigar_ops = (uint32_t *)malloc((acc.ops.size() ? acc.ops.size() : 1) * 4);
    memcpy(a->cigar_ops, acc.ops.data(), acc.ops.size() * 4);
    uint64_t w = 0;
    for (size_t i = 0; i < np; i++) {
        a->query_idx[i] = pair_q[i]; a->target_idx[i] = pair_t[i];
        a->is_reverse[i] = acc.isrev[i]; a->score[i] = acc.score[i];
        a->query_start[i] = 0; a->query_end[i] = len[pair_q[i]];
        a->target_start[i] = 0; a->target_end[i] = len[pair_t[i]];
        a->cigar_off[i] = w;
        w += acc.cnt[i];
    }
    a->cigar_off[np] = w;
    return a;
}

extern "C" int sr_ctx_alignments(sr_ctx *c, sr_alignments **out) {
    if (!c || !c->loaded) return fail(SR_ERR_INVALID, "context not loaded");
    if (c->from_paf) return fail(SR_ERR_INVALID, "context was loaded from a PAF file: it holds no device alignments");
    if (c->batch_first.size() > 2 || !c->aligned_batch_valid)
        return fail(SR_ERR_UNSUPPORTED, "the CIGARs of this context are not resident (several batches, or no alignment pass yet): use sr_align_all");
    int r = sr_ctx_sync(c);
    if (r) return r;
    const size_t np = c->pair_q.size();
    AlnAcc acc;
    acc.cnt.assign(np + 1, 0); acc.score.assign(np + 1, 0); acc.isrev.assign(np + 1, 0);
    if ((r = collect_batch(c, 0, acc))) return r;
    *out = make_alignments(c, acc);
    return SR_OK;
}

extern "C" int sr_ctx_pair_results(sr_ctx *c, int32_t *score, uint8_t *is_reverse, uint32_t *cigar_ops) {
    if (!c || !c->loaded || c->from_paf) return fail(SR_ERR_INVALID, "context holds no device alignments");
    int r = sr_ctx_sync(c);
    if (r) return r;
// ... 1206 lines not shown
```

### seqrush_amd/csrc/sr_internal.h

```cpp
#pragma once
#include <stdint.h>
#include <stddef.h>

#define SR_NULL_OFF (-8192)
#define SR_MAX_SCOPE 127
#define SR_STACK_DEPTH 64
#define SR_WG 256
#define SR_BFS_MAXSEG 4096
#define SR_BFS_SEGREC 16
#define SR_BFS_MAXACT 32
#define SR_BFS_BTCAP 1024
#define SR_NULL_ROWS 10
#define SR_BLK_MAK_SLOTS 80

enum { SR_C_M = 0, SR_C_I1 = 1, SR_C_I2 = 2, SR_C_D1 = 3, SR_C_D2 = 4 };
enum { SR_OP_M = 0, SR_OP_X = 1, SR_OP_I = 2 , SR_OP_D = 3  };

enum {
    SR_DEV_ERR_SCORE_BOUND = 1,
    SR_DEV_ERR_BASE_OVERFLOW = 2,
    SR_DEV_ERR_BACKTRACE = 4,
    SR_DEV_ERR_STACK = 8,
    SR_DEV_ERR_CIGAR_OVERFLOW = 16,
    SR_DEV_ERR_UF_SPIN = 32,
    SR_DEV_ERR_BREAKPOINT = 64,
    SR_DEV_ERR_GRAPH = 128,
    SR_DEV_ERR_ADDRESS = 256
};

struct SrPen {
    int x, o1, e1, o2, e2;
    int two;
    int scope;
};

struct SrAlignArgs {
    const uint32_t *seqwords;
    const uint64_t *word_off_fwd;
    const uint64_t *word_off_rc;
    const uint64_t *word_off_rev;
    const uint64_t *word_off_cmp;
    int symbits;
    const uint32_t *order;
    const uint32_t *seqlen;
    uint32_t max_words;
    const uint32_t *pair_q, *pair_t;
    uint32_t npairs;
    uint32_t *queue_head;
    SrPen pen, ori;
    int mem_mode;
    int ring_scope;
    int ring_hot;
    int hist_w, hist_levels;
    int impl;
    int kdepth;
    int kdepth2;
    int kblock;
    void *bring;
    uint64_t bring_wg_stride;
    int brow;
    void *bhist;
    uint64_t bhist_wg_stride;
    uint64_t hist_cap;
    uint32_t hist_stride;
    uint32_t hist_nul_w;
    int bbase_jobs;
    int *bseg;
    uint32_t *bbt;
    uint32_t *bcl;
    uint64_t bcl_wg_stride;
    void *oring;
    uint64_t oring_wg_stride;
    int orow;
    uint32_t *oqueue;
    const uint32_t *kbits;
    int pre_oriented;
    int lazy_id;
    int profile_ticks;
    int ori_levels;
    int ring_u16;
    int *bmak;
    int test_base_levels;
    int fuse_unite;
    unsigned long long *uf_nodes;
    const uint64_t *seq_goff;
    const int32_t *max_score;
    uint64_t min_match_len;
    const uint32_t *mirror;
    uint32_t *tail_list;
    uint32_t *tail_count;
    uint32_t *tail_head;
    uint32_t *tail_deferred;
    int tail_mode;
    int *brec;
    unsigned long long *timeline;
    uint8_t *is_reverse;
    int32_t *score;
    int32_t *ori_fwd, *ori_rev;
    uint32_t *cigar_ops;
    const uint64_t *cigar_base;
    uint32_t *cigar_cnt;
    unsigned long long *counters;
    int *error_flag;
};
#define SR_NCOUNTERS 52
enum { SR_TAIL_MAIN = 0,
       SR_TAIL_RUN = 1,
       SR_TAIL_DEFER_ALL = 2 };

struct SrUniteArgs {
    const uint32_t *pair_q, *pair_t;
    uint32_t npairs;
    const uint32_t *seqlen;
    const uint64_t *seq_goff;
    const uint32_t *q_start, *t_start;
    const uint8_t *is_reverse;
    const int32_t *score;
    const int32_t *max_score;
    const uint32_t *cigar_ops;
    const uint64_t *cigar_base;
    const uint32_t *cigar_cnt;
    uint64_t min_match_len;
    unsigned long long *nodes;
    uint64_t uf_size;
    unsigned long long *counters;
    int *error_flag;
};

struct SrInvJob;
struct SrInvJobJ;
struct SrInvScanArgs {
    const uint32_t *cigar_ops;
    const uint64_t *cigar_base;
    const uint32_t *cigar_cnt;
    const int32_t *score;
    const int32_t *max_score;
    uint32_t npairs;
    uint32_t pair0;
    unsigned long long min_size;
    uint32_t *count;
    const uint32_t *offset;
    struct SrInvJob *jobs;
    uint64_t job_cap;
    unsigned long long *stats;
    uint32_t join_below;
    struct SrInvJobJ *jobs_j;
    int32_t pen[6];
};

#ifdef __cplusplus
extern "C" {
#endif
int srk_inv_scan(const struct SrInvScanArgs *a, int emit, void *stream);
int srk_inv_offsets(const uint32_t *count, uint32_t n, uint32_t *off, void *stream);
int srk_align(const SrAlignArgs *a, int nwg, size_t lds_bytes, int off16, int nthreads, void *stream);
int srk_unite(const SrUniteArgs *a, int nwg, void *stream);
int srk_uf_init(unsigned long long *nodes, uint64_t total_len, uint64_t uf_size, void *stream);
int srk_labels(unsigned long long *nodes, uint64_t uf_size, unsigned long long *minarr,
               unsigned long long *labels, int *error_flag, void *stream);
int srk_merge(unsigned long long *nodes, uint64_t uf_size, const unsigned long long *labels,
              uint32_t count, int *error_flag, void *stream);
int srk_align_max_lds(void);
int srk_orient(const SrAlignArgs *a, int nwg, size_t lds_bytes, int off16, void *stream);
int srk_kmer_bits(const SrAlignArgs *a, uint32_t nseq, uint32_t *kbits, void *stream);
size_t srk_order_temp_bytes(uint32_t n);
int srk_order(const SrAlignArgs *a, uint64_t *keys_in, uint64_t *keys_out, uint32_t *vals_in, void *temp, size_t temp_bytes,
              uint32_t *order_out, void *stream);
int srk_graph_induce(const unsigned long long *labels, const uint8_t *bases, const uint8_t *islast,
                     uint64_t N, uint64_t uf_size, unsigned long long *first, uint32_t *flag, uint32_t *nid,
                     uint32_t *steps, uint8_t *node_base, unsigned long long *hkeys, uint32_t *hvals,
                     uint64_t hcap, uint32_t *eslot, unsigned long long *edges, uint32_t *tile_sum,
                     uint32_t *counts, int *error_flag, void *stream);
int srk_scan_u32(const uint32_t *in, uint64_t n, uint32_t *out, uint32_t *tile_sum, uint32_t *grand, void *stream);
const char *srk_source_digest(void);
const char *srk_align_blk_build_tag(void);
int srk_align_blk_max_levels(void);
int srk_align_blk_supports(const SrPen *pen, const SrPen *ori);
int srk_labels32(unsigned long long *nodes, uint64_t uf_size, unsigned long long *minarr, uint32_t *labels, int *error_flag,
                 void *stream);
int srk_merge32(unsigned long long *nodes, uint64_t uf_size, const uint32_t *labels, uint32_t count, int *error_flag, void *stream);
int srk_sketch(const uint8_t *bases, const uint64_t *goff, const uint32_t *len, uint32_t n, int k, int s_max,
               unsigned long long *scratch, uint64_t stride, const uint32_t *npad, unsigned long long *sketch, uint32_t *sk_n,
               void *stream);
int srk_jaccard(const unsigned long long *sketch, const uint32_t *sk_n, uint32_t n, int s_max, uint32_t *shared, uint32_t *denom,
                void *stream);
int srk_knn_select(const uint32_t *shared, const uint32_t *denom, uint32_t n, int kn, int kf, uint8_t *sel, void *stream);
struct SrIterState;
int srk_iter_unite(const SrUniteArgs *a, int nwg, const struct SrIterState *st, void *stream);
int srk_count_roots(const unsigned long long *nodes, uint64_t nbases, unsigned long long *count, const struct SrIterState *st,
                    void *stream);
int srk_iter_decide(struct SrIterState *st, const unsigned long long *counts, uint32_t k, uint32_t check, void *stream);
#ifdef __cplusplus
}
#endif
```

### seqrush_amd/seqrush.py

```python
import ctypes as C
import dataclasses
from typing import List, Optional, Sequence as Seq

import numpy as np

from . import _lib
from ._lib import (ParamsC, SeqSetC, AlignmentsC, SortParamsC, IterStatsC, InvParamsC, InvStatsC, InvJobC, InvSiteC, GraphStatsC,
                   LayoutParamsC, BinParamsC, PathBinsC, VizParamsC, GrowthParamsC, GrowthC, VariantParamsC, VariantsC, check, SeqRushError)

SR_MEM_HIGH, SR_MEM_ULTRALOW = 0, 3


@dataclasses.dataclass
class Args:
    sequences: str = ""
    output: str = "output.gfa"
    min_match_length: int = 0
    threads: int = 4
    scores: str = "0,5,8,2,24,1"
    orientation_scores: str = "0,1,1,1"
    max_divergence: Optional[float] = None
    sparsification: str = "none"
    paf: Optional[str] = None
    output_alignments: Optional[str] = None
# ... 258 lines not shown
    def run(self):
        check(self.L.sr_ctx_run(self._h))

    def align_all(self, unite: bool = False) -> "Alignments":
        p = C.POINTER(AlignmentsC)()
        check(self.L.sr_ctx_align_all(self._h, 1 if unite else 0, C.byref(p)))
        return Alignments(p)

    def orientation_scores(self):
        n = self.num_pairs
        fw = np.zeros(max(n, 1), dtype=np.int32); rv = np.zeros(max(n, 1), dtype=np.int32)
        check(self.L.sr_ctx_orientation_scores(self._h, fw.ctypes.data_as(C.POINTER(C.c_int32)), rv.ctypes.data_as(C.POINTER(C.c_int32))))
        return fw[:n], rv[:n]

    def pair_results(self):
        n = self.num_pairs
        sc = np.zeros(max(n, 1), dtype=np.int32); rv = np.zeros(max(n, 1), dtype=np.uint8); co = np.zeros(max(n, 1), dtype=np.uint32)
        check(self.L.sr_ctx_pair_results(self._h, sc.ctypes.data_as(C.POINTER(C.c_int32)),
                                         rv.ctypes.data_as(C.POINTER(C.c_uint8)), co.ctypes.data_as(C.POINTER(C.c_uint32))))
        return sc[:n], rv[:n], co[:n]

    def load_iterative(self, seqset: SeqSet, params: Params, keep_alignments: bool = False):
        self.seqset = seqset
        check(self.L.sr_ctx_load_iterative(self._h, C.byref(seqset.c), C.byref(params.c), 1 if keep_alignments else 0))

    def run_iterative(self):
        check(self.L.sr_ctx_run_iterative(self._h))

    def iterative_stats(self):
        st = IterStatsC()
        check(self.L.sr_ctx_iterative_stats(self._h, C.byref(st), None, 0))
        cc = np.zeros(max(int(st.checks), 1), dtype=np.uint64)
        check(self.L.sr_ctx_iterative_stats(self._h, C.byref(st), cc.ctypes.data_as(C.POINTER(C.c_uint64)), int(st.checks)))
        d = {f: getattr(st, f) for f, _ in IterStatsC._fields_ if f != "reserved"}
        d["stabilized"], d["tree_defaulted"] = bool(d["stabilized"]), bool(d["tree_defaulted"])
        d["check_counts"] = [int(x) for x in cc[:int(st.checks)]]
        return d

    def iterative_alignments(self) -> "Alignments":
        p = C.POINTER(AlignmentsC)()
        check(self.L.sr_ctx_iterative_alignments(self._h, C.byref(p)))
        return Alignments(p)

    def enable_inversions(self, min_size: int = 0, keep_alignments: bool = False, on: bool = True, join_below: int = 0):
        if not on:
            check(self.L.sr_ctx_enable_inversions(self._h, None))
            return
        if not 0 <= int(join_below) < 2 ** 32:
            raise SeqRushError(-1, f"inversion join length out of range: {join_below}")
        ip = InvParamsC(int(min_size), 1 if keep_alignments else 0, int(join_below))
        check(self.L.sr_ctx_enable_inversions(self._h, C.byref(ip)))

    def inversion_stats(self):
        st = InvStatsC()
        check(self.L.sr_ctx_inversion_stats(self._h, C.byref(st)))
        return {f: getattr(st, f) for f, _ in InvStatsC._fields_}

    def inversion_join_stats(self):
        out = (C.c_uint64 * 4)()
        check(self.L.sr_ctx_inversion_join_stats(self._h, out))
        return dict(islands_absorbed=int(out[0]), rejected_site_cost=int(out[1]), host_us=int(out[2]))

    def inversion_jobs(self):
        p = C.POINTER(InvJobC)(); cnt = C.c_uint64()
        check(self.L.sr_ctx_inversion_jobs(self._h, C.byref(p), C.byref(cnt)))
        out = [{f: int(getattr(p[i], f)) for f, _ in InvJobC._fields_ if f != "reserved"} for i in range(cnt.value)]
        self.L.sr_free(C.cast(p, C.c_void_p))
        return out

    def inversion_alignments(self) -> "Alignments":
        p = C.POINTER(AlignmentsC)()
        check(self.L.sr_ctx_inversion_alignments(self._h, C.byref(p)))
        return Alignments(p)

    def load_paf(self, seqset: SeqSet, params: Params, paf_path: str):
        self.seqset = seqset
        check(self.L.sr_ctx_load_paf(self._h, C.byref(seqset.c), C.byref(params.c), paf_path.encode()))

    def build_gfa(self, compact: bool = False, sort: "Optional[SortParams]" = None, compact_on: str = "host"):
        mode = compact_mode(compact, compact_on)
        out = C.c_void_p(); nn = C.c_uint64(); ne = C.c_uint64()
        if sort is None:
            check(self.L.sr_ctx_build_gfa_opts(self._h, C.byref(self.seqset.c), mode, C.byref(out),
                                               C.byref(nn), C.byref(ne)))
        else:
            check(self.L.sr_ctx_build_gfa_sorted(self._h, C.byref(self.seqset.c), mode, C.byref(sort.c),
                                                 C.byref(out), C.byref(nn), C.byref(ne)))
        text = C.cast(out, C.c_char_p).value.decode()
        self.L.sr_free(out)
        return text, int(nn.value), int(ne.value)

    def reset_uf(self):
        check(self.L.sr_ctx_reset_uf(self._h))

    def align(self):
        check(self.L.sr_ctx_align(self._h))

    def unite(self):
        check(self.L.sr_ctx_unite(self._h))

    def sync(self):
        check(self.L.sr_ctx_sync(self._h))

    def alignments(self) -> Alignments:
        p = C.POINTER(AlignmentsC)()
        check(self.L.sr_ctx_alignments(self._h, C.byref(p)))
        return Alignments(p)

    @property
    def uf_size(self):
        return int(self.L.sr_ctx_uf_size(self._h))

    @property
    def num_pairs(self):
        return int(self.L.sr_ctx_num_pairs(self._h))

    @property
    def dp_cells(self):
        return int(self.L.sr_ctx_dp_cells(self._h))

    def download_uf(self) -> np.ndarray:
        out = np.zeros(self.uf_size, dtype=np.uint64)
        check(self.L.sr_ctx_download_uf(self._h, out.ctypes.data_as(C.POINTER(C.c_uint64))))
        return out

    def download_labels(self) -> np.ndarray:
        out = np.zeros(self.uf_size, dtype=np.uint64)
        check(self.L.sr_ctx_download_labels(self._h, out.ctypes.data_as(C.POINTER(C.c_uint64))))
        return out

    def labels_device(self, dev_ptr: int):
        check(self.L.sr_ctx_labels_device(self._h, C.c_void_p(dev_ptr)))

    def merge_labels(self, dev_ptr: int, count: int):
        check(self.L.sr_ctx_merge_labels(self._h, C.c_void_p(dev_ptr), count))

    def labels_device_u32(self, dev_ptr: int):
        check(self.L.sr_ctx_labels_device_u32(self._h, C.c_void_p(dev_ptr)))

    def merge_labels_u32(self, dev_ptr: int, count: int):
        check(self.L.sr_ctx_merge_labels_u32(self._h, C.c_void_p(dev_ptr), count))

    @property
    def align_kernel(self) -> str:
        n = self.L.sr_ctx_align_kernel(self._h)
        return n.decode() if n else ""

    def kernel_ms(self, which: int) -> float:
        ms = C.c_float()
        check(self.L.sr_ctx_kernel_ms(self._h, which, C.byref(ms)))
        return float(ms.value)

    def counters(self):
        out = (C.c_uint64 * 52)()
        n = self.L.sr_ctx_counters_all(self._h, out, 52)
        if n < 0:
            check(n)
        return dict(row_bytes_loaded=int(out[16]), row_bytes_stored=int(out[17]), tk_recompute=int(out[18]),
                    wf_cells=int(out[0]), wf_steps=int(out[1]), base_segments=int(out[2]),
                    breakpoint_searches=int(out[3]), united_bases=int(out[4]), match_runs=int(out[5]),
                    ticks_orientation=int(out[6]), ticks_breakpoint=int(out[7]), ticks_base=int(out[8]),
                    bp_passes=int(out[9]), ticks_pair=int(out[10]), tk_pass=int(out[11]),
                    tk_barrier=int(out[12]), tk_setup_first=int(out[13]), tk_phase2=int(out[14]),
                    tk_tail=int(out[15]), bp_filter_units=int(out[19]), bp_candidates=int(out[20]),
                    bp_exact_units=int(out[21]), bp_rounds=int(out[22]), tk_backtrace=int(out[23]), tk_emit=int(out[24]),
                    tk_ctl_section=int(out[25]), tk_ctl_mak=int(out[26]), tk_ctl_segments=int(out[27]), tk_p2_list=int(out[28]),
                    tk_p2_filter=int(out[29]), tk_p2_exact=int(out[30]), tk_p2_replay=int(out[31]),
                    st_wait_cycles=int(out[32]), st_body_cycles=int(out[33]), st_tiles=int(out[34]), st_ext_iters=int(out[35]),
                    lds_row_bytes=int(out[36]), base_requeues=int(out[37]),
                    mirror_pairs=int(out[38]), mirror_ties=int(out[39]),
                    bounds_first=[int(out[40]), int(out[41]), int(out[42]), int(out[43])],
                    experiment=[int(out[44]), int(out[45]), int(out[46]), int(out[47])],
                    hist_bytes_loaded=int(out[44]), hist_bytes_stored=int(out[45]), base_tiles=int(out[46]),
                    base_level_diagonals=int(out[47]),
                    mirror_tie_top=int(out[48]), mirror_tie_base_only=int(out[49]), mirror_replays=int(out[50]),
                    replay_cached_searches=int(out[51]))

    def tail_deferred(self) -> int:
        v = C.c_uint64()
        check(self.L.sr_ctx_tail_deferred(self._h, C.byref(v)))
        return int(v.value)

    def tail_timeline(self):
        cap = int(self.workspace_report().get("workgroups", 0))
        out = np.zeros((max(cap, 1), 4), dtype=np.uint64)
        n = self.L.sr_ctx_tail_timeline(self._h, out.ctypes.data_as(C.POINTER(C.c_uint64)), cap)
        if n < 0:
            check(n)
        return out[:n]

    def close(self):
        if self._h:
            self.L.sr_ctx_destroy(self._h)
            self._h = C.c_void_p()

    def __del__(self):
        try:
            self.close()
        except Exception:
            pass


class SortParams:

    HOST_TWIN, SEQUENTIAL = -1, -2

    def __init__(self, **kw):
        self.c = SortParamsC()
        _lib.load().sr_sort_params_default(C.byref(self.c))
        for k, v in kw.items():
            if not hasattr(self.c, k):
                raise AttributeError(k)
            setattr(self.c, k, int(v) if isinstance(v, bool) else v)

    @staticmethod
    def from_args(args: Args) -> "SortParams":
        return SortParams(seed=args.sort_seed, iter_max=args.sgd_iter_max, skip_sgd=args.skip_sgd,
                          skip_groom=args.skip_groom, skip_topo=args.skip_topo, device=args.device)

    def as_dict(self):
        return {f: getattr(self.c, f) for f, _ in SortParamsC._fields_}


def _sort_params(params) -> SortParams:
    return params if isinstance(params, SortParams) else SortParams(**params)


def sort_gfa(text: str, **params) -> str:
    L = _lib.load()
    sp = _sort_params(params)
    out = C.c_void_p(); nn = C.c_uint64(); ne = C.c_uint64()
    check(L.sr_sort_gfa(text.encode(), C.byref(sp.c), C.byref(out), C.byref(nn), C.byref(ne)))
    res = C.cast(out, C.c_char_p).value.decode()
    L.sr_free(out)
    return res


COMPACT_STATS = ("rounds", "host_rounds", "chains", "longest_list", "jumps", "compact_us", "copy_us", "reserved")


def compact_mode(compact: bool, compact_on: str) -> int:
    if compact_on not in ("host", "device"):
        raise SeqRushError(-1, f"compact_on must be 'host' or 'device', not {compact_on!r}")
    if compact_on == "device" and not compact:
        raise SeqRushError(-1, "--compact-on device and --no-compact exclude each other")
    return 0 if not compact else (2 if compact_on == "device" else 1)


def compact_gfa(text: str, device: int = -1, stats: Optional[dict] = None) -> str:
    L = _lib.load()
    out = C.c_void_p(); nn = C.c_uint64(); ne = C.c_uint64()
    st = (C.c_uint64 * 8)()
    check(L.sr_compact_gfa(text.encode(), device, C.byref(out), C.byref(nn), C.byref(ne), st))
    res = C.cast(out, C.c_char_p).value.decode()
    L.sr_free(out)
    if stats is not None:
        stats.update(zip(COMPACT_STATS, (int(v) for v in st)))
    return res


def compact_stats() -> dict:
    st = (C.c_uint64 * 8)()
    check(_lib.load().sr_compact_stats(st))
    return dict(zip(COMPACT_STATS, (int(v) for v in st)))


SR_STATS_DEVICE_HOST = -1
STATS_KERNELS = ("steps", "nodes", "similarity", "layout", "topology")


class _GraphStats:

    def __init__(self, text: str, device: int):
        self.L = _lib.load()
        self.p = C.POINTER(GraphStatsC)()
        check(self.L.sr_graph_stats_gfa(text.encode(), int(device), C.byref(self.p)))

    def close(self):
        if self.p:
            self.L.sr_graph_stats_free(self.p)
            self.p = None

    def __enter__(self):
        return self

    def __exit__(self, *exc):
        self.close()

    def as_dict(self) -> dict:
        s = self.p.contents
        V, P = int(s.nodes), int(s.paths)

        def arr(ptr, n, dt):
            return np.ctypeslib.as_array(ptr, shape=(max(n, 1),))[:n].astype(dt, copy=True)

        def sq(parts):
            return (int(parts[0]) << 32) + (int(parts[1]) << 17) + int(parts[2])
        d = {k: int(getattr(s, k)) for k in ("length", "nodes", "edges", "paths", "steps", "rev_steps", "depth_bp", "self_loops",
                                             "tips", "components", "total_pairs", "total_abs", "total_len", "stats_us")}
        d["depth"], d["paths_on"] = arr(s.depth, V, np.uint32), arr(s.paths_on, V, np.uint32)
        d["bp_by_paths"], d["nodes_by_paths"] = arr(s.bp_by_paths, P + 1, np.uint64), arr(s.nodes_by_paths, P + 1, np.uint64)
        d["shared"] = arr(s.shared, P * P, np.uint64).reshape(P, P)
        d["path_pairs"], d["path_abs"], d["path_len"] = (arr(q, P, np.uint64) for q in (s.path_pairs, s.path_abs, s.path_len))
        d["path_sq_parts"] = arr(s.path_sq, 3 * P, np.uint64).reshape(P, 3)
        d["path_sq"] = [sq(row) for row in d["path_sq_parts"]]
        d["total_sq_parts"] = [int(v) for v in s.total_sq]
        d["total_sq"] = sq(s.total_sq)
        d["kernel_us"] = dict(zip(STATS_KERNELS, (int(v) for v in s.kernel_us)))
        return d

    def report(self, names) -> str:
        arr = (C.c_char_p * max(1, len(names)))(*[n.encode() for n in names])
        out = C.c_void_p()
        check(self.L.sr_graph_stats_report(self.p, C.cast(arr, C.POINTER(C.c_char_p)), C.byref(out)))
        res = C.cast(out, C.c_char_p).value.decode()
        self.L.sr_free(out)
        return res


def _path_names(text: str):
    names = []
    for line in text.split("\n"):
        f = line.rstrip("\r").split("\t")
        if f[0][:1] == "P" and len(f) >= 3:
            names.append(f[1])
    return names


def graph_stats(text: str, device: int = 0) -> dict:
    with _GraphStats(text, device) as gs:
        return gs.as_dict()


def _graph_stats_report(text: str, device: int):
    with _GraphStats(text, device) as gs:
        s = gs.p.contents
        return gs.report(_path_names(text)), dict(stats_us=int(s.stats_us))


# ... 965 lines not shown
```

Measured before the change: 102,300 pairs/s.

## Rotate wave priority among co-resident workgroups per CU by clock epoch

Each workgroup takes a per-CU arrival rank through an atomic counter indexed by the XCC and CU hardware registers. During tile passes its low-priority setting becomes a role (0-3) that rotates with a realtime clock epoch, so the workgroups sharing a CU take turns at high s_setprio instead of all sitting at priority 0. The aim is to stagger co-resident workgroups and cut contention and tail imbalance on the shared CU. In exchange it adds an atomic and a memset per launch, a clock read per pass, and a risk of starving some workgroups. It is turned off for large batches and for the tail launch.

```diff
diff --git a/include/seqrush_amd.h b/include/seqrush_amd.h
--- a/include/seqrush_amd.h
+++ b/include/seqrush_amd.h
@@ -131,6 +131,9 @@
 const char *sr_knobs_doc(void);
 int sr_ctx_tail_deferred(sr_ctx *c, uint64_t *out);
 int sr_ctx_tail_timeline(sr_ctx *c, uint64_t *out, uint32_t cap_wg);
+int sr_ctx_prio_timeline(sr_ctx *c, uint64_t *out, uint32_t cap_wg);
+int sr_tile_prio_role_host(uint32_t rank, uint32_t epoch, uint32_t wg_per_cu);
+int sr_tile_prio_epoch_shift(void);
 int sr_tail_shape(int impl, int block_levels, int wave_build, int off16, int ring_u16, int symbol_bits, int two_piece,
                   int main_threads, uint32_t max_words, int forced);
 
diff --git a/seqrush_amd/_lib.py b/seqrush_amd/_lib.py
--- a/seqrush_amd/_lib.py
+++ b/seqrush_amd/_lib.py
@@ -39,6 +39,7 @@
     "sr_variant_params_default", "sr_variants_gfa", "sr_variants_free", "sr_variants_vcf",
     "sr_ctx_tail_deferred", "sr_ctx_tail_timeline", "sr_tail_shape",
     "sr_replay_record_ints", "sr_replay_transpose_host", "sr_replay_match_host",
+    "sr_ctx_prio_timeline", "sr_tile_prio_role_host", "sr_tile_prio_epoch_shift",
 ]
 
 
@@ -234,6 +235,9 @@
     L.sr_knobs_doc.restype = C.c_char_p
     L.sr_ctx_tail_deferred.argtypes = [vp, C.POINTER(u64)]
     L.sr_ctx_tail_timeline.argtypes = [vp, C.POINTER(u64), C.c_uint32]
+    L.sr_ctx_prio_timeline.argtypes = [vp, C.POINTER(u64), C.c_uint32]
+    L.sr_tile_prio_role_host.argtypes = [C.c_uint32, C.c_uint32, C.c_uint32]
+    L.sr_tile_prio_epoch_shift.argtypes = []
     L.sr_tail_shape.argtypes = [i32] * 8 + [C.c_uint32, i32]
     L.sr_ctx_load_pairs.argtypes = [vp, PS, PP, C.POINTER(C.c_uint32), C.POINTER(C.c_uint32), u64]
     L.sr_ctx_pairs.argtypes = [vp, C.POINTER(C.POINTER(C.c_uint32)), C.POINTER(C.POINTER(C.c_uint32)), C.POINTER(u64)]
diff --git a/seqrush_amd/csrc/sr_align_blk.inc b/seqrush_amd/csrc/sr_align_blk.inc
--- a/seqrush_amd/csrc/sr_align_blk.inc
+++ b/seqrush_amd/csrc/sr_align_blk.inc
@@ -32,7 +32,7 @@
     unsigned long long t_ori = 0, t_bp = 0, t_base = 0, t_all = 0, tb_bt = 0, tb_emit = 0;
     unsigned long long tq_pass = 0, tq_bar = 0, tq_ctl = 0, tq_ph2 = 0, tq_tail = 0, tq_rec = 0;
     unsigned row_ld = 0, row_st = 0;
-    unsigned long long tl_first = 0, tl_last = 0, tl_n = 0, tl_mir = 0;
+    unsigned long long tl_first = 0, tl_last = 0, tl_n = 0, tl_mir = 0, tl_end1 = 0;
     const int depth = a.kdepth;
     const int depth2 = a.kdepth2;
     const unsigned nrows = (unsigned)depth + 4u * (unsigned)depth2 + (unsigned)SR_NULL_ROWS + 2u;
@@ -64,6 +64,22 @@
             b_sh.geom.brow = a.brow; b_sh.geom.ring_scope = a.ring_scope; b_sh.geom.ring_hot = a.ring_hot;
             b_sh.geom.bbase_jobs = a.bbase_jobs; b_sh.geom.hist_w = a.hist_w; b_sh.geom.hist_levels = a.hist_levels;
             b_sh.geom.urow = urow;
+            unsigned p_rank = 0, p_idx = 0, p_arr = 0;
+            if (a.cu_arrivals) {
+                const unsigned xcc = (unsigned)__builtin_amdgcn_s_getreg(20 | (0 << 6) | (3 << 11));
+                const unsigned cu = (unsigned)__builtin_amdgcn_s_getreg(4 | (8 << 6) | (7 << 11));
+                p_idx = sr_prio_table_index(xcc, cu);
+                p_arr = atomicAdd(&a.cu_arrivals[p_idx], 1u);
+                p_rank = p_arr % (unsigned)max(a.prio_wg, 1);
+                atomicAdd(&a.counters[52], 1ull);
+                atomicMax(&a.counters[53], (unsigned long long)p_arr + 1ull);
+            }
+            k_sh.prio_rank = (int)p_rank; k_sh.prio_role = 0;
+            k_sh.prio_wg = (a.tile_prio && a.cu_arrivals && a.prio_wg > 1) ? a.prio_wg : 0;
+            if (PROF && a.prio_timeline) {
+                unsigned long long *tp = a.prio_timeline + 4ull * blockIdx.x;
+                tp[0] = 0ull; tp[1] = p_rank; tp[2] = p_idx; tp[3] = p_arr;
+            }
         }
         __syncthreads();
     }
@@ -95,6 +111,7 @@
             if (PROF) {
                 const unsigned long long now = KTICK();
                 if (tl_n == 0) tl_first = now;
+                if (tl_n == 1 && tl_end1 == 0) tl_end1 = now;
                 if (pr < (int)a.npairs) { tl_last = now; tl_n++; tl_mir = from_mir ? 1ull : 0ull; }
             }
             k_sh.rp_on = (from_mir && k_sh.rp_ready) ? 1 : 0;
@@ -697,6 +714,7 @@
             unsigned long long *tl = a.timeline + 4ull * blockIdx.x;
             tl[0] = tl_first; tl[1] = tl_last; tl[2] = KTICK(); tl[3] = tl_n | (tl_mir << 32);
         }
+        if (PROF && a.prio_timeline) a.prio_timeline[4ull * blockIdx.x] = tl_end1;
         if (PROF) {
             if (!a.pre_oriented) atomicAdd(&a.counters[6], t_ori);
             atomicAdd(&a.counters[7], t_bp);
diff --git a/seqrush_amd/csrc/sr_blk_pass.inc b/seqrush_amd/csrc/sr_blk_pass.inc
--- a/seqrush_amd/csrc/sr_blk_pass.inc
+++ b/seqrush_amd/csrc/sr_blk_pass.inc
@@ -1,4 +1,5 @@
 #include "sr_base_cone.h"
+#include "sr_prio_rule.h"
 template <bool TWO, int E1, int E2>
 __device__ __forceinline__ int kreach(const SrPen &p, int s, int begin) {
     int r;
@@ -21,8 +22,23 @@
 }
 
 #define KTICK() (PROF ? __builtin_amdgcn_s_memrealtime() : 0ull)
+__device__ __forceinline__ void kprio_role() {
+    switch (RFL(k_sh.prio_role)) {
+    case 1: __builtin_amdgcn_s_setprio(1); break;
+    case 2: __builtin_amdgcn_s_setprio(2); break;
+    case 3: __builtin_amdgcn_s_setprio(3); break;
+    default: __builtin_amdgcn_s_setprio(0); break;
+    }
+}
+__device__ __forceinline__ void kprio_epoch() {
+    const int wg = RFL(k_sh.prio_wg);
+    if (wg > 1) {
+        const unsigned epoch = (unsigned)(__builtin_amdgcn_s_memrealtime() >> SR_PRIO_EPOCH_SHIFT);
+        if (threadIdx.x == 0) k_sh.prio_role = sr_tile_prio_role((unsigned)k_sh.prio_rank, epoch, (unsigned)wg);
+    }
+}
 #define KPRIO_HI() __builtin_amdgcn_s_setprio(3)
-#define KPRIO_LO() __builtin_amdgcn_s_setprio(0)
+#define KPRIO_LO() kprio_role()
 #ifndef SR_BASE_CONE
 #define SR_BASE_CONE 1
 #endif
@@ -77,6 +93,7 @@
     if (tid == 0) k_sh.jtstart[0] = 0;
     if (tid == 63) { k_sh.nband = hincl; k_sh.total_tiles = incl + hincl; k_sh.next_tile = NT / 64; if (BASE) k_sh.base_tiles += (unsigned long long)incl; }
     k_sh.cells_l[tid] += (unsigned long long)cells;
+    kprio_epoch();
 }
 
 template <typename OT, bool TWO, int NT, int B, int E1, int E2, bool PROF, int X = 0, int OE1 = 0, typename ST = OT, bool RING = false, bool BASE = false>
@@ -89,6 +106,7 @@
         __syncthreads();
         if (PROF && threadIdx.x == 0) k_sh.t_setup += KTICK() - tsu0;
     }
+    kprio_role();
     const int total = RFL(k_sh.total_tiles);
     const int slot0 = kslots(R, s0);
     const int nband = RFL(k_sh.nband);
diff --git a/seqrush_amd/csrc/sr_blk_rows.inc b/seqrush_amd/csrc/sr_blk_rows.inc
--- a/seqrush_amd/csrc/sr_blk_rows.inc
+++ b/seqrush_amd/csrc/sr_blk_rows.inc
@@ -16,6 +16,7 @@
     int jgplo[BJ_MAX + 2], jgphi[BJ_MAX + 2];
     int total_tiles;
     int next_tile;
+    int prio_role, prio_rank, prio_wg;
     int p2n, p2seg[K_P2];
     unsigned p2mask_lo, p2mask_hi;
     int pc_n[K_P2], pc_s1[K_P2][2 * KB_MAX];
diff --git a/seqrush_amd/csrc/sr_host.cpp b/seqrush_amd/csrc/sr_host.cpp
--- a/seqrush_amd/csrc/sr_host.cpp
+++ b/seqrush_amd/csrc/sr_host.cpp
@@ -21,6 +21,7 @@
 #include "sr_inv_rule.h"
 #include "sr_base_cone.h"
 #include "sr_mirror_rule.h"
+#include "sr_prio_rule.h"
 
 static thread_local std::string g_err;
 static int fail(int code, const std::string &msg) { g_err = msg; return code; }
@@ -50,6 +51,7 @@
     {"SR_PROFILE_TICKS", "0", "1 = launch the instrumented instance (100 MHz tick counters, per-workgroup timeline)"},
     {"SR_TAIL", "on", "0 = no tail launch: a tied secondary is always aligned by its primary's workgroup (A/B runs); all = every such secondary is deferred to the tail launch (tests)"},
     {"SR_TAIL_THREADS", "widest instance wider than the main launch", "threads per workgroup of the tail launch among the existing instances: 256 | 512 | 1024 (tests)"},
+    {"SR_TILE_PRIO", "1", "0 = no rotating tile priority among the workgroups of a CU: all tile code at priority 0, no clock read (A/B runs, tests)"},
     {"SR_TAIL_ROUNDS", "8", "a batch defers only when its alignments are at most this many times the launch's workgroups"},
     {"SR_FORCE_INT32", "off", "tests: 32-bit offsets (and the 16-bit ring of 32-bit searches) whatever the sequence length"},
     {"SR_TEST_BASE_LEVELS", "off", "tests: cap on the levels a base case is given at first (forces the re-queue path)"},
@@ -266,6 +268,9 @@
     std::vector<uint32_t> batch_partners;
     uint32_t *d_tail_list = nullptr, *d_tail_deferred = nullptr;
     unsigned long long *d_timeline = nullptr;
+    int prio_rounds = SR_TAIL_ROUNDS_DEFAULT;
+    uint32_t *d_cu_arrivals = nullptr;
+    unsigned long long *d_prio_timeline = nullptr;
     std::vector<std::pair<hipEvent_t, hipEvent_t>> ev[5];
     int ev_used[5] = {0, 0, 0, 0, 0};
     bool loaded = false;
@@ -318,6 +323,7 @@
     c->d_error = nullptr; c->d_queue = nullptr; c->d_oqueue = nullptr; c->d_order = nullptr; c->d_cbase = nullptr;
     c->d_bases = nullptr; c->d_max_score = nullptr; c->d_mirror = nullptr; c->mirror_partners = 0; c->onwg = 0;
     c->tail_threads = 0; c->tail_all = false; c->batch_partners.clear(); c->d_tail_list = c->d_tail_deferred = nullptr; c->d_timeline = nullptr;
+    c->d_cu_arrivals = nullptr; c->d_prio_timeline = nullptr;
     c->d_okeys = c->d_okeys2 = nullptr; c->d_ovals = nullptr; c->d_otemp = nullptr; c->otemp_bytes = 0;
     c->loaded = false; c->from_paf = false; c->aligned_batch_valid = false;
     for (int k = 0; k < 5; k++) c->ev_used[k] = 0;
@@ -1078,6 +1084,17 @@
     if (impl == 2 && knob("SR_PROFILE_TICKS") && atoi(knob("SR_PROFILE_TICKS")) != 0) {
         if ((r = dev_alloc(c, &d, (size_t)nwg * 4 * 8))) return r; c->d_timeline = (unsigned long long *)d;
         HIPCHK(hipMemsetAsync(c->d_timeline, 0, (size_t)nwg * 4 * 8, c->stream));
+        if ((r = dev_alloc(c, &d, (size_t)nwg * 4 * 8))) return r; c->d_prio_timeline = (unsigned long long *)d;
+        HIPCHK(hipMemsetAsync(c->d_prio_timeline, 0, (size_t)nwg * 4 * 8, c->stream));
+    }
+    if (impl == 2) {
+        if ((r = dev_alloc(c, &d, SR_PRIO_TABLE * sizeof(uint32_t)))) return r; c->d_cu_arrivals = (uint32_t *)d;
+        HIPCHK(hipMemsetAsync(c->d_cu_arrivals, 0, SR_PRIO_TABLE * sizeof(uint32_t), c->stream));
+        const char *tp = knob("SR_TILE_PRIO");
+        a.prio_wg = std::max(1, std::min(pl.wg_per_cu, 1024 / std::max(64, c->nthreads)));
+        a.tile_prio = (a.prio_wg > 1 && !(tp && atoi(tp) == 0)) ? 1 : 0;
+        const char *trk = knob("SR_TAIL_ROUNDS");
+        c->prio_rounds = trk ? std::max(0, atoi(trk)) : SR_TAIL_ROUNDS_DEFAULT;
     }
     if ((r = dev_alloc(c, &d, (uint64_t)nwg * pl.bring_wg * rsz))) return r; a.bring = d;
     if ((r = dev_alloc(c, &d, (uint64_t)nwg * pl.bhist_wg * osz))) return r; a.bhist = d;
@@ -1170,6 +1187,7 @@
     a.fuse_unite = 0; a.uf_nodes = c->d_nodes; a.seq_goff = sd.goff; a.max_score = c->d_max_score; a.min_match_len = p->min_match_len;
     a.mirror = c->d_mirror;
     a.tail_count = c->d_queue + 1; a.tail_head = c->d_queue + 2; a.tail_deferred = c->d_tail_deferred; a.timeline = c->d_timeline;
+    a.cu_arrivals = c->d_cu_arrivals; a.prio_timeline = c->d_prio_timeline;
     c->fuse_unite = impl == 2 && !knob("SR_NO_FUSED_UNITE");
     u.is_reverse = a.is_reverse; u.score = a.score; u.max_score = c->d_max_score;
     u.cigar_ops = a.cigar_ops; u.cigar_base = c->d_cbase; u.cigar_cnt = a.cigar_cnt;
@@ -1180,7 +1198,7 @@
 
 static void write_report(sr_ctx *c, const PackedSeqs &pk, const SrPen &pen, const Plan &pl) {
     const uint32_t np = (uint32_t)c->pair_q.size();
-    char buf[2048];
+    char buf[3072];
     const SrPen &ori = c->aa.ori;
     const char *oroute = c->onwg == 0 ? "in-kernel"
                          : (!ori.two && ori.x == 1 && ori.o1 == 1 && ori.e1 == 1 && !knob("SR_ORIENT_LEVELS")) ? "orient-blk" : "orient-levels";
@@ -1191,14 +1209,15 @@
              "\"base_history_bytes_per_workgroup\": %llu, \"workspace_bytes\": %llu, \"cigar_arena_bytes\": %llu, "
              "\"orientation_ring_bytes\": %llu, \"union_find_bytes\": %llu, \"device_free_bytes_at_load\": %zu, \"kernel_build\": \"%s\", "
              "\"ring_depth_m\": %d, \"ring_depth_id\": %d, \"fused_unite\": %d, \"wave_build\": %d, \"level_kernel_wide\": %d, "
-             "\"profile_ticks\": %d, \"orientation_route\": \"%s\", \"source_digest\": \"%s\", \"mirror_partners\": %llu, \"tail_threads\": %d, \"mirror_replay\": %d, \"replay_record_bytes\": %llu, \"knobs\": ",
+             "\"profile_ticks\": %d, \"orientation_route\": \"%s\", \"source_digest\": \"%s\", \"mirror_partners\": %llu, \"tail_threads\": %d, \"mirror_replay\": %d, \"replay_record_bytes\": %llu, \"tile_prio\": %d, \"prio_epoch_shift\": %d, \"prio_workgroups_per_cu\": %d, \"knobs\": ",
              np, pl.nbatch, pk.sm.bits, pl.osz, pl.impl == 2 ? pl.rsz : pl.osz, pl.impl, pl.impl == 2 ? pl.kblock : 1, pen.two ? 1 : 0, pl.lazy_id,
              pl.nwg, c->nthreads, pl.wg_per_cu, c->lds_bytes,
              (unsigned long long)(pl.bring_wg * pl.rsz), (unsigned long long)(pl.bhist_wg * pl.osz),
              (unsigned long long)((uint64_t)pl.nwg * pl.per_wg_bytes), (unsigned long long)(pl.arena_ops * 4), (unsigned long long)pl.oring_bytes,
              (unsigned long long)(3ULL * c->uf_size * 8), pl.free_b, srk_align_blk_build_tag(), pl.kdepth, pl.kdepth2, c->fuse_unite ? 1 : 0,
              pl.wave_wg ? 1 : 0, (pl.impl == 1 && pl.ring_scope + 1 > 32) ? 1 : 0, c->aa.profile_ticks, oroute, srk_source_digest(),
-             (unsigned long long)c->mirror_partners, c->tail_threads, pl.brec_bytes ? 1 : 0, (unsigned long long)pl.brec_bytes);
+             (unsigned long long)c->mirror_partners, c->tail_threads, pl.brec_bytes ? 1 : 0, (unsigned long long)pl.brec_bytes,
+             c->aa.tile_prio, SR_PRIO_EPOCH_SHIFT, c->aa.prio_wg);
     c->workspace_report = std::string(buf) + knobs_json() + "}";
 }
 
@@ -1300,6 +1319,8 @@
     const bool defer = partners > 0 && (c->tail_all || (uint64_t)(a.npairs - partners) <= (uint64_t)c->tail_rounds * (uint64_t)main_wg);
     a.tail_list = defer ? c->d_tail_list : nullptr;
     a.tail_mode = defer && c->tail_all ? SR_TAIL_DEFER_ALL : SR_TAIL_MAIN;
+    const uint32_t secondaries = b < c->batch_partners.size() ? std::min<uint32_t>(c->batch_partners[b], a.npairs) : 0;
+    if ((uint64_t)(a.npairs - secondaries) > (uint64_t)c->prio_rounds * (uint64_t)main_wg) a.tile_prio = 0;
     HIPCHK(hipMemsetAsync(c->d_queue, 0, (c->tail_threads ? 3 : 1) * sizeof(uint32_t), c->stream));
     hipEvent_t *e0, *e1;
     int r;
@@ -1319,11 +1340,13 @@
     if ((r = ev_get(c, 0, c->ev_used[0], &e0, &e1))) return r;
     HIPCHK(hipEventRecord(*e0, c->stream));
     if (a.npairs > 0) {
+        if (a.cu_arrivals) HIPCHK(hipMemsetAsync(a.cu_arrivals, 0, SR_PRIO_TABLE * sizeof(uint32_t), c->stream));
         r = srk_align(&a, main_wg, c->lds_bytes, c->off16, c->nthreads, c->stream);
         if (r) return fail(SR_ERR_HIP, std::string("align kernel launch failed: ") + hipGetErrorString((hipError_t)r));
         if (defer) {
             const int grid = (int)std::min<uint64_t>({(uint64_t)c->tail_cus * (uint64_t)c->tail_wg_per_cu, (uint64_t)c->nwg, (uint64_t)partners});
             a.tail_mode = SR_TAIL_RUN; a.timeline = nullptr;
+            a.cu_arrivals = nullptr; a.prio_timeline = nullptr; a.tile_prio = 0;
             r = srk_align(&a, grid, c->lds_bytes, c->off16, c->tail_threads, c->stream);
             if (r) return fail(SR_ERR_HIP, std::string("align kernel tail launch failed: ") + hipGetErrorString((hipError_t)r));
         }
@@ -1510,6 +1533,18 @@
     HIPCHK(hipMemcpy(out, c->d_timeline, (size_t)n * 4 * sizeof(uint64_t), hipMemcpyDeviceToHost));
     return (int)n;
 }
+
+extern "C" int sr_ctx_prio_timeline(sr_ctx *c, uint64_t *out, uint32_t cap_wg) {
+    if (!c || !c->loaded || !out) return fail(SR_ERR_INVALID, "context not loaded");
+    if (!c->d_prio_timeline) return 0;
+    HIPCHK(hipSetDevice(c->device));
+    HIPCHK(hipStreamSynchronize(c->stream));
+    const uint32_t n = std::min<uint32_t>(cap_wg, (uint32_t)c->nwg);
+    HIPCHK(hipMemcpy(out, c->d_prio_timeline, (size_t)n * 4 * sizeof(uint64_t), hipMemcpyDeviceToHost));
+    return (int)n;
+}
+extern "C" int sr_tile_prio_role_host(uint32_t rank, uint32_t epoch, uint32_t wg_per_cu) { return sr_tile_prio_role(rank, epoch, wg_per_cu); }
+extern "C" int sr_tile_prio_epoch_shift(void) { return SR_PRIO_EPOCH_SHIFT; }
 
 extern "C" int sr_ctx_download_uf(sr_ctx *c, uint64_t *parent_out) {
     if (!c || !c->loaded) return fail(SR_ERR_INVALID, "context not loaded");
diff --git a/seqrush_amd/csrc/sr_internal.h b/seqrush_amd/csrc/sr_internal.h
--- a/seqrush_amd/csrc/sr_internal.h
+++ b/seqrush_amd/csrc/sr_internal.h
@@ -94,6 +94,10 @@
     int tail_mode;
     int *brec;
     unsigned long long *timeline;
+    uint32_t *cu_arrivals;
+    int prio_wg;
+    int tile_prio;
+    unsigned long long *prio_timeline;
     uint8_t *is_reverse;
     int32_t *score;
     int32_t *ori_fwd, *ori_rev;
@@ -103,7 +107,7 @@
     unsigned long long *counters;
     int *error_flag;
 };
-#define SR_NCOUNTERS 52
+#define SR_NCOUNTERS 54
 enum { SR_TAIL_MAIN = 0,
        SR_TAIL_RUN = 1,
        SR_TAIL_DEFER_ALL = 2 };
diff --git a/seqrush_amd/csrc/sr_prio_rule.h b/seqrush_amd/csrc/sr_prio_rule.h
--- /dev/null
+++ b/seqrush_amd/csrc/sr_prio_rule.h
@@ -0,0 +1,17 @@
+#pragma once
+
+#if defined(__HIPCC__) || defined(__CUDACC__)
+#define SR_PRIO_HD __host__ __device__
+#else
+#define SR_PRIO_HD
+#endif
+
+#define SR_PRIO_EPOCH_SHIFT 11
+#define SR_PRIO_TABLE 4096
+SR_PRIO_HD inline unsigned sr_prio_table_index(unsigned xcc_id, unsigned se_sh_cu) { return ((xcc_id & 15u) << 8 | (se_sh_cu & 255u)) & (SR_PRIO_TABLE - 1u); }
+
+SR_PRIO_HD inline int sr_tile_prio_role(unsigned rank, unsigned epoch, unsigned wg_per_cu) {
+    if (wg_per_cu <= 1u) return 0;
+    const unsigned pos = (rank % wg_per_cu + epoch % wg_per_cu) % wg_per_cu;
+    return (int)(pos * 4u / wg_per_cu);
+}
diff --git a/seqrush_amd/seqrush.py b/seqrush_amd/seqrush.py
--- a/seqrush_amd/seqrush.py
+++ b/seqrush_amd/seqrush.py
@@ -434,8 +434,8 @@
         return float(ms.value)
 
     def counters(self):
-        out = (C.c_uint64 * 52)()
-        n = self.L.sr_ctx_counters_all(self._h, out, 52)
+        out = (C.c_uint64 * 54)()
+        n = self.L.sr_ctx_counters_all(self._h, out, 54)
         if n < 0:
             check(n)
         return dict(row_bytes_loaded=int(out[16]), row_bytes_stored=int(out[17]), tk_recompute=int(out[18]),
@@ -456,7 +456,8 @@
                     hist_bytes_loaded=int(out[44]), hist_bytes_stored=int(out[45]), base_tiles=int(out[46]),
                     base_level_diagonals=int(out[47]),
                     mirror_tie_top=int(out[48]), mirror_tie_base_only=int(out[49]), mirror_replays=int(out[50]),
-                    replay_cached_searches=int(out[51]))
+                    replay_cached_searches=int(out[51]),
+                    prio_ranks_taken=int(out[52]), prio_max_cu_arrivals=int(out[53]))
 
     def tail_deferred(self) -> int:
         v = C.c_uint64()
@@ -467,6 +468,14 @@
         cap = int(self.workspace_report().get("workgroups", 0))
         out = np.zeros((max(cap, 1), 4), dtype=np.uint64)
         n = self.L.sr_ctx_tail_timeline(self._h, out.ctypes.data_as(C.POINTER(C.c_uint64)), cap)
+        if n < 0:
+            check(n)
+        return out[:n]
+
+    def prio_timeline(self):
+        cap = int(self.workspace_report().get("workgroups", 0))
+        out = np.zeros((max(cap, 1), 4), dtype=np.uint64)
+        n = self.L.sr_ctx_prio_timeline(self._h, out.ctypes.data_as(C.POINTER(C.c_uint64)), cap)
         if n < 0:
             check(n)
         return out[:n]
```

Result: faster. 108,900 pairs/s (median of 6 runs) (+6.5%).
